# zhenyuw16/Uni3DETR

Hardware: AMD Instinct MI355X
Metric: scenes/sec (fwd+bwd) SUN-RGB-D 20k pts, 300 queries (higher is better)
Workload: dtype bf16

## Files before the change

### include/u3d_hip.h

```cpp
#ifndef U3D_HIP_H_
#define U3D_HIP_H_

#include <stddef.h>
#include <stdint.h>

#ifdef __cplusplus
extern "C" {
#endif

typedef struct ihipStream_t* u3d_stream;

enum {
  U3D_OK = 0,
  U3D_ERR_ARG = -1,
  U3D_ERR_UNSUPPORTED = -2,
  U3D_ERR_LAUNCH = -3,
  U3D_ERR_WORKSPACE = -4
};

enum { U3D_F32 = 0, U3D_BF16 = 1 };

int32_t u3d_version(void);
const char* u3d_strerror(int32_t code);

// ... 388 lines not shown
  U3D_DL_IOU0, U3D_DL_IOU1, U3D_DL_IOU2,
  U3D_DL_NLIN
};
enum { U3D_DLN_1, U3D_DLN_2, U3D_DLN_3, U3D_DLN_PE0, U3D_DLN_PE1, U3D_DLN_C1, U3D_DLN_C2, U3D_DL_NLN };
typedef struct u3d_declayer_params {
  const void* w[U3D_DL_NLIN];
  const void* wt[U3D_DL_NLIN];
  const float* b[U3D_DL_NLIN];
  const float* ln_g[U3D_DL_NLN];
  const float* ln_b[U3D_DL_NLN];
  const float* attw_w; const float* attw_b;
  const float* pe0_w;  const float* pe0_b;
  const float* dim_t;
} u3d_declayer_params;
typedef struct u3d_declayer_dims {
  int32_t m;
  int32_t nq;
  int32_t qps;
  int32_t batch, dz, dy, dx;
  int32_t ncls, code;
  int32_t has_qs;
  int32_t need_dref;
  int32_t layer;
  float p_attn, p_drop;
  float ln_eps;
  int32_t dtype;
  int32_t reserved;
} u3d_declayer_dims;
enum {
  U3D_DS_SINE, U3D_DS_RPH1, U3D_DS_RPH2, U3D_DS_RAW, U3D_DS_QS1, U3D_DS_QS2, U3D_DS_QS, U3D_DS_POS, U3D_DS_QKIN,
  U3D_DS_QK, U3D_DS_V, U3D_DS_LSE, U3D_DS_O, U3D_DS_U1, U3D_DS_MR, U3D_DS_QP, U3D_DS_SAMP, U3D_DS_GATED, U3D_DS_PEH0,
  U3D_DS_UPE1, U3D_DS_U2, U3D_DS_X2C, U3D_DS_FFH, U3D_DS_U3, U3D_DS_R1, U3D_DS_R2, U3D_DS_I1, U3D_DS_I2, U3D_DS_UC1,
  U3D_DS_C1, U3D_DS_UC2, U3D_DS_C2,
  U3D_DS_AMASK,
  U3D_DS_COUNT
};
enum {
  U3D_DG_CLSO, U3D_DG_C2U, U3D_DG_C1U, U3D_DG_IOUO, U3D_DG_I2, U3D_DG_I1, U3D_DG_REGO, U3D_DG_R2, U3D_DG_R1, U3D_DG_F,
  U3D_DG_FFH, U3D_DG_OUT, U3D_DG_UPE1, U3D_DG_P0, U3D_DG_WL, U3D_DG_O2, U3D_DG_DO, U3D_DG_DQK, U3D_DG_DV, U3D_DG_QS,
  U3D_DG_QS2, U3D_DG_QS1, U3D_DG_RAW, U3D_DG_RPH2, U3D_DG_RPH1, U3D_DG_LNP, U3D_DG_DU1, U3D_DG_DPOSA, U3D_DG_SINE,
  U3D_DG_COUNT
};
int32_t u3d_decoder_layer_slots(int32_t m, int32_t ncls, int32_t code, int64_t* save_off, int64_t* grad_off);
int32_t u3d_decoder_layer_slots_dt(int32_t m, int32_t ncls, int32_t code, int32_t dtype, int64_t* save_off, int64_t* grad_off);
int32_t u3d_decoder_layer_blocks(int32_t m);
int32_t u3d_decoder_layer_blocks_dt(int32_t m, int32_t dtype);
int32_t u3d_decoder_layer_fwd(const u3d_declayer_params* p, const u3d_declayer_dims* d, const float* x, const void* xc,
                              const float* ref, const void* value, const uint64_t* rng, float* x_out, void* xc_out,
                              float* reg_out, float* cls_out, float* iou_out, void* save, int64_t save_bytes, u3d_stream s);
int32_t u3d_decoder_layer_bwd(const u3d_declayer_params* p, const u3d_declayer_dims* d, const float* x, const void* xc,
                              const float* ref, const void* value, const uint64_t* rng, const void* xc_out, const void* save,
                              const float* dx_out, const float* dreg, const float* dcls, const float* diou, float* dx,
                              void* vrec, float* dref, void* grad, int64_t grad_bytes, u3d_stream s);
int64_t u3d_value_records_bytes(int32_t m);
int64_t u3d_value_scatter_workspace(int32_t n_cells);
int32_t u3d_value_scatter(const void* records, int32_t m, int32_t n_cells, void* dvalue, int32_t dvalue_bf16, void* work,
                          int64_t work_bytes, u3d_stream s);
int32_t u3d_mha_fwd(const void* qk, const void* v, int32_t m, int32_t nq, float p_attn, int32_t layer, const uint64_t* rng, void* o,
                    float* lse, u3d_stream s);
int32_t u3d_mha_bwd(const void* qk, const void* v, const void* o, const void* d_o, const float* lse, int32_t m, int32_t nq,
                    float p_attn, int32_t layer, const uint64_t* rng, void* dqk, void* dv, u3d_stream s);
int32_t u3d_mha_fwd_dt(const void* qk, const void* v, int32_t m, int32_t nq, float p_attn, int32_t layer, const uint64_t* rng, void* o,
                       float* lse, int32_t dtype, u3d_stream s);
int32_t u3d_mha_bwd_dt(const void* qk, const void* v, const void* o, const void* d_o, const float* lse, int32_t m, int32_t nq,
                       float p_attn, int32_t layer, const uint64_t* rng, void* dqk, void* dv, int32_t dtype, u3d_stream s);
typedef struct u3d_wpack_desc {
  const float* src; void* dst; void* dst_t;
  int32_t n, k, n_pad, n_pad_t;
  int32_t t_plain;
  int32_t reserved;
} u3d_wpack_desc;
int32_t u3d_wpack_bf16(const u3d_wpack_desc* descs_dev, int32_t count, int32_t max_elems, u3d_stream s);
int32_t u3d_wpack(const u3d_wpack_desc* descs_dev, int32_t count, int32_t max_elems, int32_t dtype, u3d_stream s);
int32_t u3d_dropout_mask(const uint64_t* rng, int32_t layer, int32_t site, int64_t n, float p, int32_t cols, uint8_t* keep, u3d_stream s);

#define U3D_AUG_NPARAM 9
int32_t u3d_points_augment(float* points, const int32_t* scene_off, int32_t batch, int32_t n_total, int32_t feat, const float* params,
                           int32_t coord, int32_t height_dim, u3d_stream s);
int32_t u3d_boxes_augment(float* boxes, const int32_t* gt_off, int32_t batch, int32_t n, int32_t box_dim, const float* params, int32_t coord,
                          u3d_stream s);
int32_t u3d_points_range_filter(const float* points, const int32_t* scene_off, int32_t batch, int32_t feat, const float* range6, float* out,
                                int32_t* count, u3d_stream s);
int32_t u3d_point_sample(const float* points, const int32_t* scene_off, const int32_t* count, int32_t batch, int32_t feat, int32_t num_points,
                         const uint64_t* seed, float* out, int32_t* idx_out, u3d_stream s);

int32_t u3d_boxes_range_filter(float* boxes, int32_t* labels, const int32_t* gt_off, int32_t batch, int32_t box_dim,
                               const float* bev_range4, int32_t* count, u3d_stream s);
int32_t u3d_point_shuffle(const float* points, const int32_t* scene_off, const int32_t* count, int32_t batch, int32_t n_total, int32_t feat,
                          const uint64_t* seed, float* out, u3d_stream s);
int32_t u3d_boxes_label_filter(float* boxes, int32_t* labels, const int32_t* gt_off, const int32_t* gt_count, int32_t batch, int32_t box_dim,
                               int32_t num_classes, int32_t* count, u3d_stream s);

int32_t u3d_batch_ingest(const float* points, int32_t n_src, int32_t feat, const int32_t* scene_off, const int32_t* count, int32_t batch,
                         int32_t point_cap, const float* gt, int32_t g_src, int32_t box_dim, const int32_t* gt_labels, const int32_t* gt_off,
                         const int32_t* gt_count, int32_t gt_cap, int32_t gt_dim, float* cat, int32_t* dst_off, float* gt_out,
                         int32_t* labels_out, int32_t* gt_off_out, float* flag, int32_t* overflow, u3d_stream s);

int32_t u3d_objaug_stats(const int32_t* scene_off, const int32_t* count, const int32_t* gt_off, const int32_t* gt_count,
                         const int32_t* labels, int32_t batch, int32_t ncls, int32_t* stats, u3d_stream s);
int32_t u3d_objaug_accept(const float* gt, const int32_t* gt_off, const int32_t* g_live, int32_t box_dim, const float* db_boxes,
                          const int32_t* cand_ids, const int32_t* cand_off, const int32_t* cand_grp, int32_t batch, int32_t words,
                          int32_t* hit_ws, uint32_t* cc_ws, int32_t* acc, u3d_stream s);
int32_t u3d_points_in_boxes(const float* points, const int32_t* scene_off, const int32_t* n_live, int32_t batch, int32_t feat,
                            int32_t tiles, const float* boxes, const int32_t* box_off, const int32_t* box_live, const int32_t* box_active,
                            int32_t box_dim, int32_t words, int32_t* first, uint32_t* bits, int32_t* tile_free, u3d_stream s);
int32_t u3d_objaug_paste(const float* points, const int32_t* scene_off, const int32_t* n_live, int32_t feat, const int32_t* first,
// ... 42 lines not shown
```

### uni3detr_amd/csrc/decoder.hip

```cpp
#include "decoder_common.h"

#ifdef DC_PHASE_TIMING
__device__ unsigned long long dc_dbg_fwd[64];
#define DC_MARK(id) do { if (blockIdx.x == 7 && threadIdx.x == 0) dc_dbg_fwd[id] = __builtin_readcyclecounter(); } while (0)
extern "C" int32_t u3d_debug_fwd_times(uint64_t* out) { return hipMemcpyFromSymbol(out, HIP_SYMBOL(dc_dbg_fwd), 64 * 8) == hipSuccess ? 0 : -1; }
#define MP_MARK(id) do { if (blockIdx.x == 7 && threadIdx.x == 0) dc_dbg_fwd[32 + (id)] = __builtin_readcyclecounter(); } while (0)
#else
#define DC_MARK(id)
#define MP_MARK(id)
#endif

template <typename E>
struct DcPtrs {
  typedef typename E::T T;
  T *sine, *rph1, *rph2, *raw, *qs1, *qs2, *qs, *pos, *qkin, *qk, *v;
  float* lse;
  T* o;
  float *u1, *mr;
  T *qp, *samp, *gated, *peh0, *upe1;
  float* u2;
  T *x2c, *ffh;
  float* u3;
  T *r1, *r2, *i1, *i2, *uc1, *c1, *uc2, *c2;
  unsigned* amask;
// ... 80 lines not shown
  for (int i = blockIdx.x * 256 + threadIdx.x; i < total; i += gridDim.x * 256) {
    const int e = i % E::CH, l = (i / E::CH) & 63, blk = i / WBLK, ks = blk % KS, tile = blk / KS;
    const int n = tile * 16 + (l & 15), k = ks * E::KSTEP + (l >> 4) * E::CH + e;
    ((T*)d.dst)[i] = n < d.n ? E::from_f(d.src[(size_t)n * d.k + k]) : E::from_f(0.f);
  }
  if (d.dst_t) {
    const int tt = d.k * d.n_pad_t;
    if (d.t_plain) {
      for (int i = blockIdx.x * 256 + threadIdx.x; i < tt; i += gridDim.x * 256) {
        const int k = i / d.n_pad_t, n = i % d.n_pad_t;
        ((T*)d.dst_t)[i] = n < d.n ? E::from_f(d.src[(size_t)n * d.k + k]) : E::from_f(0.f);
      }
    } else {
      const int KST = d.n_pad_t / E::KSTEP;
      for (int i = blockIdx.x * 256 + threadIdx.x; i < tt; i += gridDim.x * 256) {
        const int e = i % E::CH, l = (i / E::CH) & 63, blk = i / WBLK, ks = blk % KST, tile = blk / KST;
        const int k = tile * 16 + (l & 15), n = ks * E::KSTEP + (l >> 4) * E::CH + e;
        ((T*)d.dst_t)[i] = n < d.n ? E::from_f(d.src[(size_t)n * d.k + k]) : E::from_f(0.f);
      }
    }
  }
}
extern "C" int32_t u3d_wpack(const u3d_wpack_desc* descs_dev, int32_t count, int32_t max_elems, int32_t dtype, u3d_stream s) {
  U3D_REQUIRE(descs_dev && count >= 0 && max_elems > 0 && (dtype == U3D_BF16 || dtype == U3D_F32), U3D_ERR_ARG);
  if (count == 0) return U3D_OK;
  int gx = u3d_cdiv(max_elems, 256 * 4);
  if (gx > 64) gx = 64;
  if (dtype == U3D_BF16) hipLaunchKernelGGL(k_wpack<EB>, dim3(gx, count), dim3(256), 0, s, descs_dev);
  else hipLaunchKernelGGL(k_wpack<EF>, dim3(gx, count), dim3(256), 0, s, descs_dev);
  U3D_CHECK_LAUNCH();
  return U3D_OK;
}
extern "C" int32_t u3d_wpack_bf16(const u3d_wpack_desc* descs_dev, int32_t count, int32_t max_elems, u3d_stream s) {
  return u3d_wpack(descs_dev, count, max_elems, U3D_BF16, s);
}

__global__ void k_dropout_mask(const unsigned long long* rng, int layer, int site, long long n, unsigned thresh, int cols, unsigned char* keep) {
  const long long i = (long long)blockIdx.x * blockDim.x + threadIdx.x;
  if (i >= n) return;
  const unsigned idx = cols > 0 ? dc_att_idx((unsigned)(i / cols), (unsigned)(i % cols), (unsigned)(cols + 1) & ~1u) : (unsigned)i;
  keep[i] = thresh == 0u ? 1 : (dc_keep(dc_rng_load(rng), dc_site_key(layer, site), idx, thresh) ? 1 : 0);
}
extern "C" int32_t u3d_dropout_mask(const uint64_t* rng, int32_t layer, int32_t site, int64_t n, float p, int32_t cols, uint8_t* keep,
                                    u3d_stream s) {
  U3D_REQUIRE(rng && keep && n >= 0 && p >= 0.f && p < 1.f && cols >= 0, U3D_ERR_ARG);
  if (n == 0) return U3D_OK;
  hipLaunchKernelGGL(k_dropout_mask, dim3((unsigned)((n + 255) / 256)), dim3(256), 0, s, (const unsigned long long*)rng, layer, site,
                     (long long)n, dc_thresh(p), (int)cols, keep);
  U3D_CHECK_LAUNCH();
  return U3D_OK;
}

template <typename E>
__global__ __launch_bounds__(DC_THREADS) void k_dec_pre(u3d_declayer_params P, u3d_declayer_dims dm, const typename E::T* __restrict__ xc,
                                                        const float* __restrict__ ref, DcPtrs<E> S, int skip_inproj) {
  typedef typename E::T T;
  typedef typename E::V4 V4;
  typedef typename E::VC VC;
  typedef DcLds<E> L;
  constexpr int BM = E::BM;
  extern __shared__ __attribute__((aligned(16))) unsigned char lds[];
  T* A0 = (T*)(lds + L::A0);
  T* A1 = (T*)(lds + L::A1);
  T* A2 = (T*)(lds + L::A2);
  const int tid = threadIdx.x, lane = tid & 63, wave = dc_wave_id();
  const int wv = (wave + (int)(blockIdx.x >> 3)) & 3;
  const int row0 = blockIdx.x * BM, M = dm.m;
  dc_poison_lds<E>(lds, tid);
  constexpr int SCH = 384 / E::CH;
  DC_FOR_TID(c, BM * SCH) {
    const int row = c / SCH, ch = c % SCH, col0 = ch * E::CH, coord = col0 >> 7, f0 = col0 & 127;
    const float pos = E::sigmoid(ref[(size_t)min(row0 + row, M - 1) * 3 + coord]);
    VC v;
#pragma unroll
    for (int e = 0; e < E::CH; ++e) {
      const float sarg = pos * 6.283185307179586f / P.dim_t[f0 + e];
      v[e] = E::from_f((e & 1) ? cosf(sarg) : sinf(sarg));
    }
    *(VC*)(A0 + dc_aoff<E>(row, col0, 384)) = v;
    *(VC*)(S.sine + (size_t)(row0 + row) * 384 + col0) = v;
  }
  __syncthreads();
  auto relu_to = [&](T* dst, const float* bias) {
    return [=](int row, int col, f32x4 v) {
      *(V4*)(dst + dc_aoff<E>(row, col, DC_C)) = E::pack4(dc_relu4(v + dc_bias4(bias, col)));
    };
  };
  auto lin_to = [&](T* dst, const float* bias) {
    return [=](int row, int col, f32x4 v) { *(V4*)(dst + dc_aoff<E>(row, col, DC_C)) = E::pack4(v + dc_bias4(bias, col)); };
  };
  T* A1b = A1 + BM * DC_C;
  dc_linear<E, 384, 4>(A0, (const T*)P.w[U3D_DL_RPH0], wv * 64, lane, relu_to(A1, P.b[U3D_DL_RPH0]));
  __syncthreads();
  dc_store_a<E, 256>(A1, S.rph1, DC_C, row0, tid);
  dc_linear<E, 256, 4>(A1, (const T*)P.w[U3D_DL_RPH1], wv * 64, lane, relu_to(A0, P.b[U3D_DL_RPH1]));
  __syncthreads();
  dc_store_a<E, 256>(A0, S.rph2, DC_C, row0, tid);
  dc_linear<E, 256, 4>(A0, (const T*)P.w[U3D_DL_RPH2], wv * 64, lane, lin_to(A2, P.b[U3D_DL_RPH2]));
  __syncthreads();
  dc_store_a<E, 256>(A2, dm.has_qs ? S.raw : S.pos, DC_C, row0, tid);
  dc_load_a<E, 256, true>(A0, xc, DC_C, row0, M, tid);
  __syncthreads();
  if (dm.has_qs) {
    dc_linear<E, 256, 4>(A0, (const T*)P.w[U3D_DL_QS0], wv * 64, lane, relu_to(A1, P.b[U3D_DL_QS0]));
    __syncthreads();
    dc_store_a<E, 256>(A1, S.qs1, DC_C, row0, tid);
    dc_linear<E, 256, 4>(A1, (const T*)P.w[U3D_DL_QS1], wv * 64, lane, relu_to(A1b, P.b[U3D_DL_QS1]));
    __syncthreads();
    dc_store_a<E, 256>(A1b, S.qs2, DC_C, row0, tid);
    const float* bias = P.b[U3D_DL_QS2];
    dc_linear<E, 256, 4>(A1b, (const T*)P.w[U3D_DL_QS2], wv * 64, lane, [=](int row, int col, f32x4 v) {
      const V4 q = E::pack4(v + dc_bias4(bias, col));
      const int ao = dc_aoff<E>(row, col, DC_C);
      const f32x4 raw = E::unpack4(*(const V4*)(A2 + ao));
      *(V4*)(A2 + ao) = E::pack4(E::unpack4(q) * raw);
      *(V4*)(A1 + ao) = q;
    });
    __syncthreads();
    dc_store_a<E, 256>(A1, S.qs, DC_C, row0, tid);
    dc_store_a<E, 256>(A2, S.pos, DC_C, row0, tid);
  }
  DC_FOR_TID(c, BM * (DC_C / E::CH)) {
    const int off = c * E::CH;
    const VC a = *(const VC*)(A0 + off), p = *(const VC*)(A2 + off);
    VC r;
#pragma unroll
    for (int e = 0; e < E::CH; ++e) r[e] = E::from_f(E::to_f(a[e]) + E::to_f(p[e]));
    *(VC*)(A1b + off) = r;
  }
  __syncthreads();
  dc_store_a<E, 256>(A1b, S.qkin, DC_C, row0, tid);
  if (skip_inproj) return;
  dc_linear<E, 256, 4>(A1b, (const T*)P.w[U3D_DL_INQK], wv * 64, lane, lin_to(A1, P.b[U3D_DL_INQK]));
  {
    const float* bias = P.b[U3D_DL_INQK];
    dc_linear<E, 256, 4>(A1b, (const T*)P.w[U3D_DL_INQK], 256 + wv * 64, lane, [=](int row, int col, f32x4 v) {
      *(V4*)(A2 + dc_aoff<E>(row, col - 256, DC_C)) = E::pack4(v + dc_bias4(bias, col));
    });
  }
  __syncthreads();
  dc_store_a<E, 256>(A1, S.qk, 512, row0, tid);
  dc_store_a<E, 256>(A2, S.qk + 256, 512, row0, tid);
  dc_linear<E, 256, 4>(A0, (const T*)P.w[U3D_DL_INV], wv * 64, lane, lin_to(A1b, P.b[U3D_DL_INV]));
  __syncthreads();
  dc_store_a<E, 256>(A1b, S.v, DC_C, row0, tid);
}

template <typename E>
__device__ __forceinline__ void mha_chunk(const typename E::T* Ks, const typename E::T* Vs, const typename E::T* Vt, int kc0, int nkeys,
                                          const typename Mha<E>::RowFrag& qf, unsigned row, unsigned nq_pad, DcRng rg, unsigned key_site,
                                          unsigned thresh, float inv_keep, float scale_log2, int r16, int kq, float& m_run, float& l_run,
                                          f32x4 (&oacc)[2], const unsigned* __restrict__ keep_bits = nullptr) {
  typedef Mha<E> H;
  constexpr int KC = H::KC;
  const int ntile = (nkeys + 15) >> 4;
  f32x4 s[KC / 16];
  float mx = -INFINITY;
#pragma unroll
  for (int t = 0; t < KC / 16; ++t) {
    s[t] = (f32x4){-INFINITY, -INFINITY, -INFINITY, -INFINITY};
    if (t < ntile) {
      f32x4 a = H::scores(Ks, t * 16, r16, kq, qf);
      if (t == ntile - 1) {
#pragma unroll
        for (int r = 0; r < 4; ++r) a[r] = t * 16 + kq * 4 + r < nkeys ? a[r] : -INFINITY;
      }
      mx = fmaxf(fmaxf(mx, fmaxf(a[0], a[1])), fmaxf(a[2], a[3]));
      s[t] = a;
    }
  }
  mx = fmaxf(mx, __shfl_xor(mx, 16, 64));
  mx = fmaxf(mx, __shfl_xor(mx, 32, 64));
  const float m_new = fmaxf(m_run, mx);
  const float corr = E::exp2((m_run - m_new) * scale_log2);
  const float neg_m = -m_new * scale_log2;
  l_run *= corr;
  oacc[0] *= corr; oacc[1] *= corr;
  m_run = m_new;
#pragma unroll
  for (int tp = 0; tp < KC / 32; ++tp) {
    if (tp * 2 < ntile) {
      f32x4 p0, p1;
#pragma unroll
      for (int r = 0; r < 4; ++r) {
        p0[r] = E::exp2(fmaf(s[2 * tp][r], scale_log2, neg_m));
        p1[r] = E::exp2(fmaf(s[2 * tp + 1][r], scale_log2, neg_m));
        l_run += p0[r] + p1[r];
      }
      if (thresh && keep_bits) {
        const int w = (int)keep_bits[tp];
#pragma unroll
        for (int r = 0; r < 4; ++r) {
          p0[r] = __int_as_float(__float_as_int(p0[r] * inv_keep) & __builtin_amdgcn_sbfe(w, kq * 4 + r, 1));
          p1[r] = __int_as_float(__float_as_int(p1[r] * inv_keep) & __builtin_amdgcn_sbfe(w, 16 + kq * 4 + r, 1));
        }
      } else if (thresh) {
// ... 200 lines not shown
        *(V4*)(img + row * RS + (t & 1) * 16 + kq * 4) = valid ? pk : (V4){0, 0, 0, 0};
      }
    }
  }
  MP_MARK(3);
  __syncthreads();
  MP_MARK(4);
  {
    const int per = nq * 4, total = 3 * per, iters = (total + MHA_PROJ_THREADS - 1) / MHA_PROJ_THREADS;
    for (int it = 0; it < iters; ++it) {
      const int c = it * MHA_PROJ_THREADS + tid;
      if (c < total) {
        const int which = c / per, rem = c - which * per, row = rem >> 2, part = rem & 3;
        const VC v = *(const VC*)((which == 0 ? Qs : (which == 1 ? Ks : Vs)) + row * RS + part * 8);
        u16* dst = which == 2 ? v_out + (base + row) * DC_C + h * DC_HD + part * 8
                              : qk_out + (base + row) * 512 + which * 256 + h * DC_HD + part * 8;
        *(VC*)dst = v;
      }
    }
    if (thresh) {
      const int words = nq * MhaProjLds::MW, wit = (words + MHA_PROJ_THREADS - 1) / MHA_PROJ_THREADS;
      for (int it = 0; it < wit; ++it) {
        const int wd = it * MHA_PROJ_THREADS + tid;
        if (wd < words) amask[(size_t)bh * words + wd] = Ms[wd];
      }
    }
  }
  MP_MARK(5);
  for (int qb = wave; qb < nrb; qb += NW) {
    const int q = qb * 16 + r16;
    H::RowFrag qf;
    qf.c[0] = *(const VC*)(Qs + q * RS + kq * 8);
    f32x4 oacc[2] = {{0.f, 0.f, 0.f, 0.f}, {0.f, 0.f, 0.f, 0.f}};
    float m_run = -INFINITY, l_run = 0.f;
    const unsigned row = (unsigned)(bh * nq + q);
    unsigned kb[MhaProjLds::MW];
#pragma unroll
    for (int j = 0; j < MhaProjLds::MW; ++j) kb[j] = Ms[q * MhaProjLds::MW + j];
    mha_chunk<EB>(Ks, Vs, nullptr, 0, nq, qf, row, nq_pad, rg, key_site, thresh, inv_keep, scale_log2, r16, kq, m_run, l_run, oacc, kb);
    l_run += __shfl_xor(l_run, 16, 64);
    l_run += __shfl_xor(l_run, 32, 64);
    if (q < nq) {
      const float inv = 1.f / l_run;
#pragma unroll
      for (int dt = 0; dt < 2; ++dt) *(V4*)(o + (base + q) * DC_C + h * DC_HD + dt * 16 + kq * 4) = EB::pack4(oacc[dt] * inv);
      if (kq == 0) lse[(base + q) * DC_NHEAD + h] = m_run * scale_log2 + log2f(l_run);
    }
    MP_MARK(6 + (qb >> 3));
  }
  MP_MARK(9);
}

template <typename E>
__global__ __launch_bounds__(DC_THREADS) void k_dec_post(u3d_declayer_params P, u3d_declayer_dims dm, const float* __restrict__ x,
                                                         const float* __restrict__ ref, const typename E::T* __restrict__ value,
                                                         const unsigned long long* __restrict__ rng, DcPtrs<E> S, float* __restrict__ x_out,
                                                         typename E::T* __restrict__ xc_out, float* __restrict__ reg_out,
                                                         float* __restrict__ cls_out, float* __restrict__ iou_out) {
  typedef typename E::T T;
  typedef typename E::V4 V4;
  typedef DcLds<E> L;
  constexpr int BM = E::BM, RPW = E::BM / 4;
  extern __shared__ __attribute__((aligned(16))) unsigned char lds[];
  T* A0 = (T*)(lds + L::A0);
  T* A1 = (T*)(lds + L::A1);
  T* A2 = (T*)(lds + L::A2);
  float* F = (float*)(lds + L::F);
  float* G = (float*)(lds + L::G);
  float* misc = (float*)(lds + L::MISC);
  const int tid = threadIdx.x, lane = tid & 63, wave = dc_wave_id();
  const int wv = (wave + (int)(blockIdx.x >> 3)) & 3;
  const int row0 = blockIdx.x * BM, M = dm.m;
  dc_poison_lds<E>(lds, tid);
  DcDrop drop = {dc_rng_load(rng), dc_thresh(dm.p_drop), dc_inv_keep(dm.p_drop), dm.layer};

  DC_MARK(0);
  dc_load_a<E, 256, true>(A0, S.o, DC_C, row0, M, tid);
  dc_load_f<E, false>(F, x, row0, M, tid);
  dc_load_a<E, 256, false>(A2, S.pos, DC_C, row0, M, tid);
  {
    const int row = (tid >> 3) & (BM - 1), j = tid & 7;
    misc[row * DC_MISC_LD + j] = ref[(size_t)min(row0 + row, M - 1) * 3 + min(j, 2)];
  }
  __syncthreads();
  auto add_to_F = [&](const float* bias, int site) {
    return [=](int row, int col, f32x4 v) {
      v = E::round4(v + dc_bias4(bias, col));
      v = drop.apply(v, site, (unsigned)((row0 + row) * DC_C + col));
      float* fp = F + row * DC_TS + col;
      *(f32x4*)fp = *(const f32x4*)fp + v;
    };
  };
  DC_MARK(1);
  dc_linear<E, 256, 4>(A0, (const T*)P.w[U3D_DL_OUTP], wv * 64, lane, add_to_F(P.b[U3D_DL_OUTP], 0));
  __syncthreads();
  DC_MARK(2);
  {
    DcLnOut<E> o = {F, A0, DC_C, nullptr, nullptr, S.mr, U3D_DLN_1, false, S.u1, nullptr};
    dc_layernorm<E>(F, P.ln_g[U3D_DLN_1], P.ln_b[U3D_DLN_1], dm.ln_eps, false, o, row0, wave, lane);
  }
  __syncthreads();
  DC_MARK(3);
  {
    const f32x4 aw = *(const f32x4*)(P.attw_w + lane * 4);
    const float ab = P.attw_b[0];
    constexpr int GRP = 4;
    static_assert(RPW % GRP == 0, "rows per wave must split into gather groups");
#pragma unroll 1
    for (int r0g = 0; r0g < RPW; r0g += GRP) {
      V4 cv[GRP][8];
      float cw[GRP][8];
#ifndef DC_ABL_NOGATHER
#pragma unroll
      for (int g = 0; g < GRP; ++g) {
        const int row = wave * RPW + r0g + g;
        DcCorners tc;
        dc_corners<E>(misc + row * DC_MISC_LD, min(row0 + row, M - 1) / dm.qps, dm.dz, dm.dy, dm.dx, tc);
#pragma unroll
        for (int c = 0; c < 8; ++c) {
          const int vr = max(tc.row[c], 0);
          cw[g][c] = tc.row[c] >= 0 ? tc.w[c] : 0.f;
          cv[g][c] = *(const V4*)(value + (size_t)vr * DC_C + lane * 4);
        }
      }
#endif
#pragma unroll
      for (int g = 0; g < GRP; ++g) {
        const int row = wave * RPW + r0g + g;
        const size_t gr = (size_t)(row0 + row);
        const int ao = dc_aoff<E>(row, lane * 4, DC_C);
        const f32x4 x1 = E::unpack4(*(const V4*)(A0 + ao)), pp = E::unpack4(*(const V4*)(A2 + ao));
        const V4 qpb = E::pack4(x1 + pp);
        const f32x4 qp = E::unpack4(qpb);
        *(V4*)(S.qp + gr * DC_C + lane * 4) = qpb;
        const float wl = E::round(dc_wave_sum(qp[0] * aw[0] + qp[1] * aw[1] + qp[2] * aw[2] + qp[3] * aw[3]) + ab);
        const float gate = E::round(E::sigmoid(wl));
        S.mr[gr * 16 + 14] = wl;
        f32x4 acc = {0.f, 0.f, 0.f, 0.f};
#ifndef DC_ABL_NOGATHER
#pragma unroll
        for (int c = 0; c < 8; ++c) acc += cw[g][c] * E::unpack4(cv[g][c]);
#endif
        const V4 sb = E::pack4(acc);
        const V4 gb = E::pack4(E::unpack4(sb) * gate);
        *(V4*)(A1 + ao) = gb;
        *(V4*)(S.samp + gr * DC_C + lane * 4) = sb;
        *(V4*)(S.gated + gr * DC_C + lane * 4) = gb;
      }
    }
  }
  DC_MARK(4);
  {
    const int col = tid;
    const float w0 = E::round(P.pe0_w[col * 3 + 0]), w1 = E::round(P.pe0_w[col * 3 + 1]), w2 = E::round(P.pe0_w[col * 3 + 2]);
    const float b = P.pe0_b[col];
    for (int row = 0; row < BM; ++row) {
      const float* r3 = misc + row * DC_MISC_LD;
      G[row * DC_TS + col] = E::round(E::round(r3[0]) * w0 + E::round(r3[1]) * w1 + E::round(r3[2]) * w2 + b);
    }
  }
  __syncthreads();
  DC_MARK(5);
  dc_linear<E, 256, 4>(A1, (const T*)P.w[U3D_DL_OPROJ], wv * 64, lane, add_to_F(P.b[U3D_DL_OPROJ], 1));
  {
    DcLnOut<E> o = {nullptr, A0, DC_C, nullptr, S.peh0, S.mr, U3D_DLN_PE0, false, nullptr, nullptr};
    dc_layernorm<E>(G, P.ln_g[U3D_DLN_PE0], P.ln_b[U3D_DLN_PE0], dm.ln_eps, true, o, row0, wave, lane);
  }
  __syncthreads();
  DC_MARK(6);
  {
    const float* bias = P.b[U3D_DL_PE1];
    dc_linear<E, 256, 4>(A0, (const T*)P.w[U3D_DL_PE1], wv * 64, lane, [=](int row, int col, f32x4 v) {
      *(f32x4*)(G + row * DC_TS + col) = E::round4(v + dc_bias4(bias, col));
    });
  }
  __syncthreads();
  DC_MARK(7);
  {
    DcLnOut<E> o = {G, nullptr, 0, nullptr, nullptr, S.mr, U3D_DLN_PE1, true, nullptr, S.upe1};
    dc_layernorm<E>(G, P.ln_g[U3D_DLN_PE1], P.ln_b[U3D_DLN_PE1], dm.ln_eps, true, o, row0, wave, lane);
  }
  __syncthreads();
  DC_FOR_TID(c, BM * 64) {
    const int o = (c >> 6) * DC_TS + (c & 63) * 4;
    *(f32x4*)(F + o) = *(const f32x4*)(F + o) + *(const f32x4*)(G + o);
  }
  __syncthreads();
  DC_MARK(8);
  {
    DcLnOut<E> o = {F, A0, DC_C, nullptr, S.x2c, S.mr, U3D_DLN_2, false, S.u2, nullptr};
    dc_layernorm<E>(F, P.ln_g[U3D_DLN_2], P.ln_b[U3D_DLN_2], dm.ln_eps, false, o, row0, wave, lane);
  }
  __syncthreads();
  DC_MARK(9);
  {
    const float* bias = P.b[U3D_DL_FFN0];
    auto ffh = [=](int row, int col, f32x4 v) {
      v = E::round4(dc_relu4(v + dc_bias4(bias, col)));
      const V4 hb = E::pack4(drop.apply(v, 2, (unsigned)((row0 + row) * DC_FF + col)));
      *(V4*)(A1 + dc_aoff<E>(row, col, DC_FF)) = hb;
    };
    dc_linear<E, 256, 4>(A0, (const T*)P.w[U3D_DL_FFN0], wv * 64, lane, ffh);
    dc_linear<E, 256, 4>(A0, (const T*)P.w[U3D_DL_FFN0], 256 + wv * 64, lane, ffh);
  }
  __syncthreads();
  DC_MARK(10);
  dc_store_a<E, 512>(A1, S.ffh, DC_FF, row0, tid);
  dc_linear<E, 512, 4>(A1, (const T*)P.w[U3D_DL_FFN1], wv * 64, lane, add_to_F(P.b[U3D_DL_FFN1], 3));
  __syncthreads();
  DC_MARK(11);
  {
    DcLnOut<E> o = {nullptr, A2, DC_C, x_out, xc_out, S.mr, U3D_DLN_3, false, S.u3, nullptr};
    dc_layernorm<E>(F, P.ln_g[U3D_DLN_3], P.ln_b[U3D_DLN_3], dm.ln_eps, false, o, row0, wave, lane);
  }
  __syncthreads();
  DC_MARK(12);
  auto relu_to = [&](T* dst, const float* bias) {
    return [=](int row, int col, f32x4 v) {
      *(V4*)(dst + dc_aoff<E>(row, col, DC_C)) = E::pack4(dc_relu4(v + dc_bias4(bias, col)));
    };
  };
  auto narrow_out = [&](float* dst, int n, const float* bias) {
    return [=](int row, int col, f32x4 v) {
#pragma unroll
      for (int r = 0; r < 4; ++r)
        if (col + r < n) dst[(size_t)(row0 + row) * n + col + r] = E::round(v[r] + bias[col + r]);
    };
  };
  T* A1b = A1 + BM * DC_C;
#ifdef DC_PHASE_TIMING
  {
    DC_MARK(20);
    f32x4 acc[E::MT][4];
#pragma unroll
    for (int mt = 0; mt < E::MT; ++mt)
#pragma unroll
      for (int nt = 0; nt < 4; ++nt) acc[mt][nt] = (f32x4){0.f, 0.f, 0.f, 0.f};
    dc_gemm<E, 256, 4>(A2, (const T*)P.w[U3D_DL_REG0] + (size_t)(wv * 64) * 256, acc, lane);
    __builtin_amdgcn_sched_barrier(0);
    DC_MARK(21);
    auto epi = relu_to(A0, P.b[U3D_DL_REG0]);
#pragma unroll
    for (int mt = 0; mt < E::MT; ++mt)
#pragma unroll
      for (int nt = 0; nt < 4; ++nt) epi(mt * 16 + (lane & 15), wv * 64 + nt * 16 + (lane >> 4) * 4, acc[mt][nt]);
    __builtin_amdgcn_sched_barrier(0);
    DC_MARK(22);
    __syncthreads();
    DC_MARK(23);
  }
#else
  dc_linear<E, 256, 4>(A2, (const T*)P.w[U3D_DL_REG0], wv * 64, lane, relu_to(A0, P.b[U3D_DL_REG0]));
  __syncthreads();
#endif
  dc_store_a<E, 256>(A0, S.r1, DC_C, row0, tid);
  dc_linear<E, 256, 4>(A0, (const T*)P.w[U3D_DL_REG1], wv * 64, lane, relu_to(A1, P.b[U3D_DL_REG1]));
  __syncthreads();
  dc_store_a<E, 256>(A1, S.r2, DC_C, row0, tid);
  dc_linear<E, 256, 1>(A1, (const T*)P.w[U3D_DL_REG2], wv * 16, lane, narrow_out(reg_out, dm.code, P.b[U3D_DL_REG2]));
  dc_linear<E, 256, 4>(A2, (const T*)P.w[U3D_DL_IOU0], wv * 64, lane, relu_to(A0, P.b[U3D_DL_IOU0]));
  __syncthreads();
  dc_store_a<E, 256>(A0, S.i1, DC_C, row0, tid);
  dc_linear<E, 256, 4>(A0, (const T*)P.w[U3D_DL_IOU1], wv * 64, lane, relu_to(A1b, P.b[U3D_DL_IOU1]));
  __syncthreads();
  dc_store_a<E, 256>(A1b, S.i2, DC_C, row0, tid);
  dc_linear<E, 256, 1>(A1b, (const T*)P.w[U3D_DL_IOU2], wv * 16, lane, narrow_out(iou_out, 1, P.b[U3D_DL_IOU2]));
  auto to_G = [&](const float* bias) {
    return [=](int row, int col, f32x4 v) { *(f32x4*)(G + row * DC_TS + col) = E::round4(v + dc_bias4(bias, col)); };
  };
  dc_linear<E, 256, 4>(A2, (const T*)P.w[U3D_DL_CLS0], wv * 64, lane, to_G(P.b[U3D_DL_CLS0]));
  __syncthreads();
  {
    DcLnOut<E> o = {nullptr, A0, DC_C, nullptr, S.c1, S.mr, U3D_DLN_C1, false, nullptr, S.uc1};
    dc_layernorm<E>(G, P.ln_g[U3D_DLN_C1], P.ln_b[U3D_DLN_C1], dm.ln_eps, true, o, row0, wave, lane);
  }
  __syncthreads();
  dc_linear<E, 256, 4>(A0, (const T*)P.w[U3D_DL_CLS1], wv * 64, lane, to_G(P.b[U3D_DL_CLS1]));
  __syncthreads();
  {
    DcLnOut<E> o = {nullptr, A1, DC_C, nullptr, S.c2, S.mr, U3D_DLN_C2, false, nullptr, S.uc2};
    dc_layernorm<E>(G, P.ln_g[U3D_DLN_C2], P.ln_b[U3D_DLN_C2], dm.ln_eps, true, o, row0, wave, lane);
  }
  __syncthreads();
  dc_linear<E, 256, 1>(A1, (const T*)P.w[U3D_DL_CLS2], wv * 16, lane, narrow_out(cls_out, dm.ncls, P.b[U3D_DL_CLS2]));
  DC_MARK(14);
}

static int32_t dc_check(const u3d_declayer_params* p, const u3d_declayer_dims* d) {
  U3D_REQUIRE(p && d, U3D_ERR_ARG);
  U3D_REQUIRE(d->m > 0 && d->nq > 0 && d->qps > 0 && d->qps % d->nq == 0 && d->m % d->qps == 0 && d->batch == d->m / d->qps, U3D_ERR_ARG);
  U3D_REQUIRE(d->ncls > 0 && d->ncls <= 32 && d->code > 0 && d->code <= 32, U3D_ERR_UNSUPPORTED);
  U3D_REQUIRE(d->p_attn >= 0.f && d->p_attn < 1.f && d->p_drop >= 0.f && d->p_drop < 1.f, U3D_ERR_ARG);
  U3D_REQUIRE(d->dtype == U3D_BF16 || d->dtype == U3D_F32, U3D_ERR_ARG);
  U3D_REQUIRE((long long)d->m * DC_FF < (1ll << 32), U3D_ERR_UNSUPPORTED);
  for (int i = 0; i < U3D_DL_NLIN; ++i) {
    if (!d->has_qs && (i == U3D_DL_QS0 || i == U3D_DL_QS1 || i == U3D_DL_QS2)) continue;
    U3D_REQUIRE(p->w[i] && p->b[i], U3D_ERR_ARG);
  }
  for (int i = 0; i < U3D_DL_NLN; ++i) U3D_REQUIRE(p->ln_g[i] && p->ln_b[i], U3D_ERR_ARG);
  U3D_REQUIRE(p->attw_w && p->attw_b && p->pe0_w && p->pe0_b && p->dim_t, U3D_ERR_ARG);
  return U3D_OK;
}

template <typename E>
static int32_t dc_layer_fwd(const u3d_declayer_params* p, const u3d_declayer_dims* d, const float* x, const void* xc, const float* ref,
                            const void* value, const uint64_t* rng, float* x_out, void* xc_out, float* reg_out, float* cls_out,
                            float* iou_out, void* save, u3d_stream s) {
  typedef typename E::T T;
  const DcPtrs<E> S = dc_resolve<E>(save, d->m);
  const int nb = u3d_decoder_layer_blocks_dt(d->m, E::DT);
  U3D_ALLOW_LDS(k_dec_pre<E>, DcLds<E>::BYTES);
  U3D_ALLOW_LDS(k_dec_post<E>, DcLds<E>::BYTES);
  const bool fused = mha_fused_inproj(E::DT, d->nq);
  hipLaunchKernelGGL(k_dec_pre<E>, dim3(nb), dim3(DC_THREADS), DcLds<E>::BYTES, s, *p, *d, (const T*)xc, ref, S, fused ? 1 : 0);
  if (fused) {
    U3D_ALLOW_LDS(k_mha_proj_fwd, MhaProjLds::BYTES);
    const float scale_log2 = 1.4426950408889634f / sqrtf((float)DC_HD);
    hipLaunchKernelGGL(k_mha_proj_fwd, dim3((d->m / d->nq) * DC_NHEAD), dim3(MHA_PROJ_THREADS), MhaProjLds::BYTES, s, (const u16*)S.qkin,
                       (const u16*)xc, (const u16*)p->w[U3D_DL_INQK], p->b[U3D_DL_INQK], (const u16*)p->w[U3D_DL_INV], p->b[U3D_DL_INV],
                       d->nq, scale_log2, dc_thresh(d->p_attn), dc_inv_keep(d->p_attn), d->layer, (const unsigned long long*)rng,
                       (u16*)S.qk, (u16*)S.v, (u16*)S.o, S.lse, S.amask);
  } else {
    int32_t rc = u3d_mha_fwd_dt(S.qk, S.v, d->m, d->nq, d->p_attn, d->layer, rng, S.o, S.lse, E::DT, s);
    if (rc != U3D_OK) return rc;
  }
  hipLaunchKernelGGL(k_dec_post<E>, dim3(nb), dim3(DC_THREADS), DcLds<E>::BYTES, s, *p, *d, x, ref, (const T*)value,
                     (const unsigned long long*)rng, S, x_out, (T*)xc_out, reg_out, cls_out, iou_out);
  U3D_CHECK_LAUNCH();
  return U3D_OK;
}

extern "C" int32_t u3d_decoder_layer_fwd(const u3d_declayer_params* p, const u3d_declayer_dims* d, const float* x, const void* xc,
                                         const float* ref, const void* value, const uint64_t* rng, float* x_out, void* xc_out,
                                         float* reg_out, float* cls_out, float* iou_out, void* save, int64_t save_bytes, u3d_stream s) {
  int32_t rc = dc_check(p, d);
  if (rc != U3D_OK) return rc;
  U3D_REQUIRE(x && xc && ref && value && x_out && xc_out && reg_out && cls_out && iou_out && save, U3D_ERR_ARG);
  U3D_REQUIRE((d->p_attn == 0.f && d->p_drop == 0.f) || rng, U3D_ERR_ARG);
  int64_t off[U3D_DS_COUNT + 1];
  u3d_decoder_layer_slots_dt(d->m, d->ncls, d->code, d->dtype, off, nullptr);
  U3D_REQUIRE(save_bytes >= off[U3D_DS_COUNT], U3D_ERR_WORKSPACE);
  if (d->dtype == U3D_BF16) return dc_layer_fwd<EB>(p, d, x, xc, ref, value, rng, x_out, xc_out, reg_out, cls_out, iou_out, save, s);
  return dc_layer_fwd<EF>(p, d, x, xc, ref, value, rng, x_out, xc_out, reg_out, cls_out, iou_out, save, s);
}
```

### uni3detr_amd/csrc/decoder_bwd.hip

```cpp
#define DC_PF 4
#include "decoder_common.h"

#ifdef DC_PHASE_TIMING
__device__ unsigned long long dc_dbg_bwd[64];
#define DC_MARK(id) do { if (blockIdx.x == 7 && threadIdx.x == 0) dc_dbg_bwd[id] = __builtin_readcyclecounter(); } while (0)
extern "C" int32_t u3d_debug_bwd_times(uint64_t* out) { return hipMemcpyFromSymbol(out, HIP_SYMBOL(dc_dbg_bwd), 64 * 8) == hipSuccess ? 0 : -1; }
#else
#define DC_MARK(id)
#endif

template <typename E>
struct DcSave {
  typedef typename E::T T;
  const T *sine, *rph1, *rph2, *raw, *qs1, *qs2, *qs, *pos, *qkin, *qk, *v;
  const float* lse;
  const T* o;
  const float *u1, *mr;
  const T *qp, *samp, *gated, *peh0, *upe1;
  const float* u2;
  const T *x2c, *ffh;
  const float* u3;
  const T *r1, *r2, *i1, *i2, *uc1, *c1, *uc2, *c2;
  const unsigned* amask;
};
// ... 11 lines not shown
extern "C" int32_t u3d_decoder_layer_blocks_dt(int32_t m, int32_t dtype);

template <typename E>
static DcSave<E> dcb_resolve_save(const void* save, int m) {
  typedef typename E::T T;
  int64_t off[U3D_DS_COUNT + 1];
  u3d_decoder_layer_slots_dt(m, 1, 1, E::DT, off, nullptr);
  const char* b = (const char*)save;
  DcSave<E> p;
  p.sine = (const T*)(b + off[U3D_DS_SINE]); p.rph1 = (const T*)(b + off[U3D_DS_RPH1]); p.rph2 = (const T*)(b + off[U3D_DS_RPH2]);
  p.raw = (const T*)(b + off[U3D_DS_RAW]); p.qs1 = (const T*)(b + off[U3D_DS_QS1]); p.qs2 = (const T*)(b + off[U3D_DS_QS2]);
  p.qs = (const T*)(b + off[U3D_DS_QS]); p.pos = (const T*)(b + off[U3D_DS_POS]); p.qkin = (const T*)(b + off[U3D_DS_QKIN]);
  p.qk = (const T*)(b + off[U3D_DS_QK]); p.v = (const T*)(b + off[U3D_DS_V]); p.lse = (const float*)(b + off[U3D_DS_LSE]);
  p.o = (const T*)(b + off[U3D_DS_O]); p.u1 = (const float*)(b + off[U3D_DS_U1]); p.mr = (const float*)(b + off[U3D_DS_MR]);
  p.qp = (const T*)(b + off[U3D_DS_QP]); p.samp = (const T*)(b + off[U3D_DS_SAMP]); p.gated = (const T*)(b + off[U3D_DS_GATED]);
  p.peh0 = (const T*)(b + off[U3D_DS_PEH0]); p.upe1 = (const T*)(b + off[U3D_DS_UPE1]); p.u2 = (const float*)(b + off[U3D_DS_U2]);
  p.x2c = (const T*)(b + off[U3D_DS_X2C]); p.ffh = (const T*)(b + off[U3D_DS_FFH]); p.u3 = (const float*)(b + off[U3D_DS_U3]);
  p.r1 = (const T*)(b + off[U3D_DS_R1]); p.r2 = (const T*)(b + off[U3D_DS_R2]); p.i1 = (const T*)(b + off[U3D_DS_I1]);
  p.i2 = (const T*)(b + off[U3D_DS_I2]); p.uc1 = (const T*)(b + off[U3D_DS_UC1]); p.c1 = (const T*)(b + off[U3D_DS_C1]);
  p.uc2 = (const T*)(b + off[U3D_DS_UC2]); p.c2 = (const T*)(b + off[U3D_DS_C2]);
  p.amask = (const unsigned*)(b + off[U3D_DS_AMASK]);
  return p;
}
template <typename E>
static DcGrad<E> dcb_resolve_grad(void* grad, int m, int ncls, int code, int64_t* total) {
  typedef typename E::T T;
  int64_t off[U3D_DG_COUNT + 1];
  u3d_decoder_layer_slots_dt(m, ncls, code, E::DT, nullptr, off);
  char* b = (char*)grad;
  DcGrad<E> g;
  g.clso = (T*)(b + off[U3D_DG_CLSO]); g.c2u = (T*)(b + off[U3D_DG_C2U]); g.c1u = (T*)(b + off[U3D_DG_C1U]);
  g.iouo = (T*)(b + off[U3D_DG_IOUO]); g.i2 = (T*)(b + off[U3D_DG_I2]); g.i1 = (T*)(b + off[U3D_DG_I1]);
  g.rego = (T*)(b + off[U3D_DG_REGO]); g.r2 = (T*)(b + off[U3D_DG_R2]); g.r1 = (T*)(b + off[U3D_DG_R1]);
  g.f = (T*)(b + off[U3D_DG_F]); g.ffh = (T*)(b + off[U3D_DG_FFH]); g.out = (T*)(b + off[U3D_DG_OUT]);
  g.upe1 = (T*)(b + off[U3D_DG_UPE1]); g.p0 = (T*)(b + off[U3D_DG_P0]); g.wl = (T*)(b + off[U3D_DG_WL]);
  g.o2 = (T*)(b + off[U3D_DG_O2]); g.d_o = (T*)(b + off[U3D_DG_DO]); g.dqk = (T*)(b + off[U3D_DG_DQK]);
  g.dv = (T*)(b + off[U3D_DG_DV]); g.qs = (T*)(b + off[U3D_DG_QS]); g.qs2 = (T*)(b + off[U3D_DG_QS2]);
  g.qs1 = (T*)(b + off[U3D_DG_QS1]); g.raw = (T*)(b + off[U3D_DG_RAW]); g.rph2 = (T*)(b + off[U3D_DG_RPH2]);
  g.rph1 = (T*)(b + off[U3D_DG_RPH1]); g.lnp = (float*)(b + off[U3D_DG_LNP]); g.du1 = (float*)(b + off[U3D_DG_DU1]);
  g.dposa = (T*)(b + off[U3D_DG_DPOSA]); g.sine = (T*)(b + off[U3D_DG_SINE]);
  g.nb = u3d_decoder_layer_blocks_dt(m, E::DT);
  if (total) *total = off[U3D_DG_COUNT];
  return g;
}

template <typename E>
struct DcLnBwdOut { float* tile; typename E::T* a; typename E::T* g16; };
template <typename E, typename LoadU>
__device__ __forceinline__ void dc_layernorm_bwd(const float* T, LoadU load_u, const float* __restrict__ mr, int mr_idx,
                                                 const float* __restrict__ gamma, const float* __restrict__ beta, bool relu,
                                                 const DcLnBwdOut<E>& o, float* __restrict__ lnp, int ln, int nb, float* red ,
                                                 int row0, int wave, int lane, int tid) {
  typedef typename E::V4 V4;
  constexpr int RPW = E::BM / 4;
  const f32x4 ga = *(const f32x4*)(gamma + lane * 4), be = *(const f32x4*)(beta + lane * 4);
  f32x4 dg = {0.f, 0.f, 0.f, 0.f}, db = {0.f, 0.f, 0.f, 0.f};
#pragma unroll 2
  for (int rr = 0; rr < RPW; ++rr) {
    const int row = wave * RPW + rr;
    const int gr = row0 + row;
    const float mu = mr[(size_t)gr * 16 + 2 * mr_idx], rs = mr[(size_t)gr * 16 + 2 * mr_idx + 1];
    const f32x4 u = load_u(row, gr);
    f32x4 dy = *(const f32x4*)(T + row * DC_TS + lane * 4);
    f32x4 xh, dxh;
    float s1 = 0.f, s2 = 0.f;
#pragma unroll
    for (int j = 0; j < 4; ++j) {
      xh[j] = (u[j] - mu) * rs;
      if (relu && !(xh[j] * ga[j] + be[j] > 0.f)) dy[j] = 0.f;
      dxh[j] = dy[j] * ga[j];
      s1 += dxh[j];
      s2 += dxh[j] * xh[j];
      dg[j] += dy[j] * xh[j];
      db[j] += dy[j];
    }
    s1 = dc_wave_sum(s1) * (1.f / DC_C);
    s2 = dc_wave_sum(s2) * (1.f / DC_C);
    f32x4 du;
#pragma unroll
    for (int j = 0; j < 4; ++j) du[j] = rs * (dxh[j] - s1 - xh[j] * s2);
    if (o.tile) *(f32x4*)(o.tile + row * DC_TS + lane * 4) = du;
    const V4 dub = E::pack4(du);
    if (o.a) *(V4*)(o.a + dc_aoff<E>(row, lane * 4, DC_C)) = dub;
    if (o.g16) *(V4*)(o.g16 + (size_t)gr * DC_C + lane * 4) = dub;
  }
  *(f32x4*)(red + (wave * 2 + 0) * DC_C + lane * 4) = dg;
  *(f32x4*)(red + (wave * 2 + 1) * DC_C + lane * 4) = db;
  __syncthreads();
  DC_FOR_TID(i, 2 * DC_C) {
    const int which = i >> 8, col = i & 255;
    const float v = red[(0 * 2 + which) * DC_C + col] + red[(1 * 2 + which) * DC_C + col] + red[(2 * 2 + which) * DC_C + col] +
                    red[(3 * 2 + which) * DC_C + col];
    lnp[((size_t)(ln * 2 + which) * nb + blockIdx.x) * DC_C + col] = v;
  }
  __syncthreads();
}

template <typename E>
__global__ __launch_bounds__(DC_THREADS) void k_dec_post_bwd(u3d_declayer_params P, u3d_declayer_dims dm, const float* __restrict__ ref,
                                                             const typename E::T* __restrict__ value,
                                                             const unsigned long long* __restrict__ rng, DcSave<E> S, DcGrad<E> Gd,
                                                             const float* __restrict__ dx_out, const float* __restrict__ dreg,
                                                             const float* __restrict__ dcls, const float* __restrict__ diou,
                                                             void* __restrict__ vrec, float* __restrict__ dref) {
  float* const rec_ds = (float*)vrec;
  int* const rec_cell = (int*)(rec_ds + (size_t)dm.m * DC_C);
  float* const rec_w = (float*)(rec_cell + (size_t)dm.m * 8);
  typedef typename E::T T;
  typedef typename E::V4 V4;
  typedef DcLds<E> L;
  constexpr int BM = E::BM, RPW = E::BM / 4;
  extern __shared__ __attribute__((aligned(16))) unsigned char lds[];
  T* A0 = (T*)(lds + L::A0);
  T* A1 = (T*)(lds + L::A1);
  T* A2 = (T*)(lds + L::A2);
  float* F = (float*)(lds + L::F);
  float* G = (float*)(lds + L::G);
  float* misc = (float*)(lds + L::MISC);
  float* red = (float*)(A1 + BM * DC_C);
  static_assert(BM * DC_C * sizeof(T) >= 4 * 2 * DC_C * 4, "LayerNorm reduce scratch must fit the second half of A1");
  constexpr int NLD = 40;
  T* Dn = A2;
  static_assert(BM * NLD <= BM * DC_C, "narrow-gradient tile must fit the A2 region");
  const int tid = threadIdx.x, lane = tid & 63, wave = dc_wave_id();
  const int wv = (wave + (int)(blockIdx.x >> 3)) & 3;
  const int row0 = blockIdx.x * BM, M = dm.m, nb = Gd.nb;
  dc_poison_lds<E>(lds, tid);
  DcDrop drop = {dc_rng_load(rng), dc_thresh(dm.p_drop), dc_inv_keep(dm.p_drop), dm.layer};

  DC_MARK(0);
  dc_load_f<E, true>(F, dx_out, row0, M, tid);
  {
    const int row = (tid >> 3) & (BM - 1), j = tid & 7;
    misc[row * DC_MISC_LD + j] = ref[(size_t)min(row0 + row, M - 1) * 3 + min(j, 2)];
  }
  auto load_narrow = [&](const float* src, int n, T* gcopy) {
    DC_FOR_TID(i, BM * 32) {
      const int row = i >> 5, j = i & 31;
      const float raw = src[(size_t)min(row0 + row, M - 1) * n + min(j, n - 1)];
      const float vr = row0 + row < M ? raw : 0.f;
      gcopy[(size_t)(row0 + row) * n + min(j, n - 1)] = E::from_f(vr);
      Dn[row * NLD + j] = E::from_f(j < n ? vr : 0.f);
    }
  };
  auto narrow_dgrad = [&](const T* wt, const T* mask_src, T* dst) {
    typedef typename E::VC VC;
    constexpr int KSN = 32 / E::KSTEP, WBLK = 64 * E::CH;
    const int r16 = lane & 15, kq = lane >> 4;
    f32x4 acc[E::MT][4];
#pragma unroll
    for (int mt = 0; mt < E::MT; ++mt)
#pragma unroll
      for (int nt = 0; nt < 4; ++nt) acc[mt][nt] = (f32x4){0.f, 0.f, 0.f, 0.f};
#pragma unroll
    for (int ks = 0; ks < KSN; ++ks) {
      VC a[E::MT];
#pragma unroll
      for (int mt = 0; mt < E::MT; ++mt) a[mt] = *(const VC*)(Dn + (mt * 16 + r16) * NLD + (ks * 4 + kq) * E::CH);
#pragma unroll
      for (int nt = 0; nt < 4; ++nt) {
        const VC wf = *(const VC*)(wt + (size_t)((wv * 4 + nt) * KSN + ks) * WBLK + lane * E::CH);
#pragma unroll
        for (int mt = 0; mt < E::MT; ++mt) E::mma(wf, a[mt], acc[mt][nt]);
      }
    }
#pragma unroll
    for (int mt = 0; mt < E::MT; ++mt)
#pragma unroll
      for (int nt = 0; nt < 4; ++nt) {
        const int row = mt * 16 + r16, col = wv * 64 + nt * 16 + kq * 4;
        f32x4 v = acc[mt][nt];
        if (mask_src) {
          const V4 y = *(const V4*)(mask_src + (size_t)(row0 + row) * DC_C + col);
#pragma unroll
          for (int r = 0; r < 4; ++r) v[r] = E::to_f(y[r]) > 0.f ? v[r] : 0.f;
        }
        if (dst) *(V4*)(dst + dc_aoff<E>(row, col, DC_C)) = E::pack4(v);
        else *(f32x4*)(G + row * DC_TS + col) = E::round4(v);
      }
  };
  auto masked_to = [&](T* dst, const T* mask_src) {
    return [=](int row, int col, f32x4 v) {
      const V4 y = *(const V4*)(mask_src + (size_t)(row0 + row) * DC_C + col);
#pragma unroll
      for (int r = 0; r < 4; ++r) v[r] = E::to_f(y[r]) > 0.f ? v[r] : 0.f;
      *(V4*)(dst + dc_aoff<E>(row, col, DC_C)) = E::pack4(v);
    };
  };
  auto acc_to_F = [&]() {
    return [=](int row, int col, f32x4 v) {
      float* fp = F + row * DC_TS + col;
      *(f32x4*)fp = *(const f32x4*)fp + E::round4(v);
    };
  };
  auto to_G = [&]() {
    return [=](int row, int col, f32x4 v) { *(f32x4*)(G + row * DC_TS + col) = E::round4(v); };
  };
  auto u_elem = [&](const T* src) {
    return [=](int row, int gr) { return E::unpack4(*(const V4*)(src + (size_t)gr * DC_C + lane * 4)); };
  };
  auto u_f32 = [&](const float* src) {
    return [=](int row, int gr) { return *(const f32x4*)(src + (size_t)gr * DC_C + lane * 4); };
  };

  DC_MARK(1);
  load_narrow(dcls, dm.ncls, Gd.clso);
  __syncthreads();
  narrow_dgrad((const T*)P.wt[U3D_DL_CLS2], nullptr, nullptr);
  __syncthreads();
  {
    DcLnBwdOut<E> o = {nullptr, A0, Gd.c2u};
    dc_layernorm_bwd<E>(G, u_elem(S.uc2), S.mr, U3D_DLN_C2, P.ln_g[U3D_DLN_C2], P.ln_b[U3D_DLN_C2], true, o, Gd.lnp, U3D_DLN_C2, nb, red, row0,
                        wave, lane, tid);
  }
  dc_linear<E, 256, 4>(A0, (const T*)P.wt[U3D_DL_CLS1], wv * 64, lane, to_G());
  __syncthreads();
  {
    DcLnBwdOut<E> o = {nullptr, A0, Gd.c1u};
    dc_layernorm_bwd<E>(G, u_elem(S.uc1), S.mr, U3D_DLN_C1, P.ln_g[U3D_DLN_C1], P.ln_b[U3D_DLN_C1], true, o, Gd.lnp, U3D_DLN_C1, nb, red, row0,
                        wave, lane, tid);
  }
  dc_linear<E, 256, 4>(A0, (const T*)P.wt[U3D_DL_CLS0], wv * 64, lane, acc_to_F());
  __syncthreads();
  DC_MARK(2);
  load_narrow(diou, 1, Gd.iouo);
  __syncthreads();
  narrow_dgrad((const T*)P.wt[U3D_DL_IOU2], S.i2, A0);
  __syncthreads();
  dc_store_a<E, 256>(A0, Gd.i2, DC_C, row0, tid);
  dc_linear<E, 256, 4>(A0, (const T*)P.wt[U3D_DL_IOU1], wv * 64, lane, masked_to(A1, S.i1));
  __syncthreads();
  dc_store_a<E, 256>(A1, Gd.i1, DC_C, row0, tid);
  dc_linear<E, 256, 4>(A1, (const T*)P.wt[U3D_DL_IOU0], wv * 64, lane, acc_to_F());
  __syncthreads();
  DC_MARK(3);
  load_narrow(dreg, dm.code, Gd.rego);
  __syncthreads();
  narrow_dgrad((const T*)P.wt[U3D_DL_REG2], S.r2, A0);
  __syncthreads();
  dc_store_a<E, 256>(A0, Gd.r2, DC_C, row0, tid);
  dc_linear<E, 256, 4>(A0, (const T*)P.wt[U3D_DL_REG1], wv * 64, lane, masked_to(A1, S.r1));
  __syncthreads();
  dc_store_a<E, 256>(A1, Gd.r1, DC_C, row0, tid);
  dc_linear<E, 256, 4>(A1, (const T*)P.wt[U3D_DL_REG0], wv * 64, lane, acc_to_F());
  __syncthreads();
  DC_MARK(4);
  {
    DcLnBwdOut<E> o = {F, nullptr, nullptr};
    dc_layernorm_bwd<E>(F, u_f32(S.u3), S.mr, U3D_DLN_3, P.ln_g[U3D_DLN_3], P.ln_b[U3D_DLN_3], false, o, Gd.lnp, U3D_DLN_3, nb, red, row0,
                        wave, lane, tid);
  }
  DC_MARK(5);
  auto branch_grad = [&](int site, T* dst, T* gslot) {
    DC_FOR_TID(c, BM * 64) {
      const int row = c >> 6, col = (c & 63) * 4;
      f32x4 v = *(const f32x4*)(F + row * DC_TS + col);
      v = drop.apply(v, site, (unsigned)((row0 + row) * DC_C + col));
      const V4 o = E::pack4(v);
      *(V4*)(dst + dc_aoff<E>(row, col, DC_C)) = o;
      *(V4*)(gslot + (size_t)(row0 + row) * DC_C + col) = o;
    }
  };
  branch_grad(3, A0, Gd.f);
  __syncthreads();
  {
    const float ik = drop.inv_keep;
    auto dh = [=](int row, int col, f32x4 v) {
      const V4 y = *(const V4*)(S.ffh + (size_t)(row0 + row) * DC_FF + col);
#pragma unroll
      for (int r = 0; r < 4; ++r) v[r] = E::to_f(y[r]) > 0.f ? E::round(v[r]) * ik : 0.f;
      const V4 o = E::pack4(v);
      *(V4*)(A1 + dc_aoff<E>(row, col, DC_FF)) = o;
    };
    dc_linear<E, 256, 4>(A0, (const T*)P.wt[U3D_DL_FFN1], wv * 64, lane, dh);
    dc_linear<E, 256, 4>(A0, (const T*)P.wt[U3D_DL_FFN1], 256 + wv * 64, lane, dh);
  }
  __syncthreads();
  dc_store_a<E, 512>(A1, Gd.ffh, DC_FF, row0, tid);
  dc_linear<E, 512, 4>(A1, (const T*)P.wt[U3D_DL_FFN0], wv * 64, lane, acc_to_F());
  __syncthreads();
  DC_MARK(6);
  {
    DcLnBwdOut<E> o = {F, nullptr, nullptr};
    dc_layernorm_bwd<E>(F, u_f32(S.u2), S.mr, U3D_DLN_2, P.ln_g[U3D_DLN_2], P.ln_b[U3D_DLN_2], false, o, Gd.lnp, U3D_DLN_2, nb, red, row0,
                        wave, lane, tid);
  }
  DC_MARK(7);
  DC_FOR_TID(c, BM * 64) {
    const int o = (c >> 6) * DC_TS + (c & 63) * 4;
    *(f32x4*)(G + o) = E::round4(*(const f32x4*)(F + o));
  }
  __syncthreads();
  {
    DcLnBwdOut<E> o = {nullptr, A0, Gd.upe1};
    dc_layernorm_bwd<E>(G, u_elem(S.upe1), S.mr, U3D_DLN_PE1, P.ln_g[U3D_DLN_PE1], P.ln_b[U3D_DLN_PE1], true, o, Gd.lnp, U3D_DLN_PE1, nb, red,
                        row0, wave, lane, tid);
  }
  dc_linear<E, 256, 4>(A0, (const T*)P.wt[U3D_DL_PE1], wv * 64, lane, to_G());
  __syncthreads();
  {
    const f32x4 b4 = *(const f32x4*)(P.pe0_b + lane * 4);
    float w[4][3];
#pragma unroll
    for (int j = 0; j < 4; ++j)
#pragma unroll
      for (int k = 0; k < 3; ++k) w[j][k] = E::round(P.pe0_w[(lane * 4 + j) * 3 + k]);
    auto u_pe0 = [=](int row, int gr) {
      const float* r3 = misc + row * DC_MISC_LD;
      const float a = E::round(r3[0]), b = E::round(r3[1]), c = E::round(r3[2]);
      f32x4 u;
#pragma unroll
      for (int j = 0; j < 4; ++j) u[j] = E::round(a * w[j][0] + b * w[j][1] + c * w[j][2] + b4[j]);
      return u;
    };
    DcLnBwdOut<E> o = {G, nullptr, Gd.p0};
    dc_layernorm_bwd<E>(G, u_pe0, S.mr, U3D_DLN_PE0, P.ln_g[U3D_DLN_PE0], P.ln_b[U3D_DLN_PE0], true, o, Gd.lnp, U3D_DLN_PE0, nb, red, row0,
                        wave, lane, tid);
    if (dm.need_dref) {
      for (int rr = 0; rr < RPW; ++rr) {
        const int row = wave * RPW + rr;
        const f32x4 d = E::round4(*(const f32x4*)(G + row * DC_TS + lane * 4));
        float g3[3];
#pragma unroll
        for (int k = 0; k < 3; ++k) g3[k] = dc_wave_sum(d[0] * w[0][k] + d[1] * w[1][k] + d[2] * w[2][k] + d[3] * w[3][k]);
        misc[row * DC_MISC_LD + 8 + (lane & 3)] = (lane & 3) == 0 ? g3[0] : ((lane & 3) == 1 ? g3[1] : g3[2]);
      }
    }
  }
  __syncthreads();
  DC_MARK(8);
  branch_grad(1, A0, Gd.out);
  __syncthreads();
  dc_linear<E, 256, 4>(A0, (const T*)P.wt[U3D_DL_OPROJ], wv * 64, lane, to_G());
  __syncthreads();
  DC_MARK(9);
  {
    const f32x4 aw = *(const f32x4*)(P.attw_w + lane * 4);
#pragma unroll 2
    for (int rr = 0; rr < RPW; ++rr) {
      const int row = wave * RPW + rr, gr = row0 + row;
      const bool ok = gr < M;
      const f32x4 dgt = *(const f32x4*)(G + row * DC_TS + lane * 4);
      const f32x4 samp = E::unpack4(*(const V4*)(S.samp + (size_t)gr * DC_C + lane * 4));
      const float wl = S.mr[(size_t)gr * 16 + 14];
      const float gate = E::round(E::sigmoid(wl));
      float dw = dc_wave_sum(dgt[0] * samp[0] + dgt[1] * samp[1] + dgt[2] * samp[2] + dgt[3] * samp[3]);
      const float sg = E::sigmoid(wl);
      const float dwl = E::round(E::round(dw) * sg * (1.f - sg));
      Gd.wl[gr] = E::from_f(dwl);
      f32x4 dqp;
#pragma unroll
      for (int j = 0; j < 4; ++j) dqp[j] = E::round(dwl * E::round(aw[j]));
      float* fp = F + row * DC_TS + lane * 4;
      *(f32x4*)fp = *(const f32x4*)fp + dqp;
      *(V4*)(Gd.dposa + (size_t)gr * DC_C + lane * 4) = E::pack4(dqp);
      f32x4 ds;
#pragma unroll
      for (int j = 0; j < 4; ++j) ds[j] = E::round(dgt[j] * gate);
      float dsc[4];
#pragma unroll
      for (int j = 0; j < 4; ++j) dsc[j] = E::round(G[row * DC_TS + j * 64 + lane] * gate);
      DcCorners tc;
      dc_corners<E>(misc + row * DC_MISC_LD, min(gr, M - 1) / dm.qps, dm.dz, dm.dy, dm.dx, tc);
      if (ok) {
        float* rds = rec_ds + (size_t)gr * DC_C + lane;
#pragma unroll
        for (int j = 0; j < 4; ++j) rds[j * 64] = dsc[j];
        if (lane == 0) {
#pragma unroll
          for (int c = 0; c < 8; ++c) { rec_cell[(size_t)gr * 8 + c] = tc.row[c]; rec_w[(size_t)gr * 8 + c] = tc.w[c]; }
        }
      }
      float gx = 0.f, gy = 0.f, gz = 0.f;
#ifndef DC_ABL_NOGATHER
      if (ok && dm.need_dref) {
#pragma unroll
        for (int c = 0; c < 8; ++c)
          if (tc.row[c] >= 0) {
            const f32x4 val = E::unpack4(*(const V4*)(value + (size_t)tc.row[c] * DC_C + lane * 4));
            const float dot = val[0] * ds[0] + val[1] * ds[1] + val[2] * ds[2] + val[3] * ds[3];
            gx += tc.dwx[c] * dot; gy += tc.dwy[c] * dot; gz += tc.dwz[c] * dot;
          }
      }
#endif
      if (dm.need_dref) {
        gx = dc_wave_sum(gx); gy = dc_wave_sum(gy); gz = dc_wave_sum(gz);
        {
          const float* r3 = misc + row * DC_MISC_LD;
          const int k = lane % 3;
          const float gk = k == 0 ? gx * dm.dx * 0.5f : (k == 1 ? gy * dm.dy * 0.5f : gz * dm.dz * 0.5f);
          const float sk = E::sigmoid(r3[k]);
          dref[(size_t)gr * 3 + k] = r3[8 + k] + gk * 2.f * sk * (1.f - sk);
        }
      }
    }
  }
  __syncthreads();
  DC_MARK(10);
  {
    DcLnBwdOut<E> o = {F, nullptr, nullptr};
    dc_layernorm_bwd<E>(F, u_f32(S.u1), S.mr, U3D_DLN_1, P.ln_g[U3D_DLN_1], P.ln_b[U3D_DLN_1], false, o, Gd.lnp, U3D_DLN_1, nb, red, row0,
                        wave, lane, tid);
  }
  dc_store_f<E>(F, Gd.du1, row0, tid);
  branch_grad(0, A0, Gd.o2);
  __syncthreads();
  dc_linear<E, 256, 4>(A0, (const T*)P.wt[U3D_DL_OUTP], wv * 64, lane, [=](int row, int col, f32x4 v) {
    *(V4*)(A1 + dc_aoff<E>(row, col, DC_C)) = E::pack4(v);
  });
  __syncthreads();
  dc_store_a<E, 256>(A1, Gd.d_o, DC_C, row0, tid);
  DC_MARK(11);
}

template <typename E>
__global__ __launch_bounds__(256, 2) void k_mha_bwd_dq(const typename E::T* __restrict__ qk, const typename E::T* __restrict__ vv,
                                                       const typename E::T* __restrict__ o, const typename E::T* __restrict__ d_o,
                                                       const float* __restrict__ lse, int nq, int qt_per_wg, float scale_log2, float scale,
                                                       unsigned thresh, float inv_keep, int layer, const unsigned long long* __restrict__ rng,
                                                       typename E::T* __restrict__ dqk, const unsigned* __restrict__ amask) {
  typedef typename E::T T;
  typedef typename E::V4 V4;
  typedef Mha<E> H;
  constexpr int KC = H::KC, MW = KC / 32;
  __shared__ __attribute__((aligned(16))) T Ks[H::RM_ELEMS];
  __shared__ __attribute__((aligned(16))) T Vs[H::RM_ELEMS];
  __shared__ __attribute__((aligned(16))) T Kt[H::TP_ELEMS];
  const int tid = threadIdx.x, lane = tid & 63, wave = tid >> 6, r16 = lane & 15, kq = lane >> 4;
  const int bh = blockIdx.y, g = bh >> 3, h = bh & 7;
  const long long base = (long long)g * nq;
  const unsigned nq_pad = (unsigned)(nq + 1) & ~1u;
  const DcRng rg = dc_rng_load(rng);
  const unsigned key_site = dc_site_key(layer, 4);
  const bool one_chunk = nq <= KC;
  for (int qt = 0; qt < qt_per_wg; ++qt) {
    const int q0 = (blockIdx.x * qt_per_wg + qt) * 64;
    if (q0 >= nq) break;
    const int q = q0 + wave * 16 + r16;
    const bool qok = q < nq;
    typename H::RowFrag qf = H::zero_frag(), dof = H::zero_frag();
    float Dq = 0.f, lq = INFINITY;
    if (qok) {
      qf = H::load_frag(qk + (base + q) * 512 + h * DC_HD, kq);
      dof = H::load_frag(d_o + (base + q) * DC_C + h * DC_HD, kq);
      Dq = H::dot(dof, H::load_frag(o + (base + q) * DC_C + h * DC_HD, kq));
      lq = lse[(base + q) * DC_NHEAD + h];
    }
    Dq += __shfl_xor(Dq, 16, 64);
    Dq += __shfl_xor(Dq, 32, 64);
    f32x4 dq[2] = {{0.f, 0.f, 0.f, 0.f}, {0.f, 0.f, 0.f, 0.f}};
    const unsigned row = (unsigned)(bh * nq + q);
    unsigned kb[MW];
#pragma unroll
    for (int j = 0; j < MW; ++j) kb[j] = (amask && qok) ? amask[(size_t)row * MW + j] : 0u;
    for (int kc0 = 0; kc0 < nq; kc0 += KC) {
      if (qt == 0 || !one_chunk) {
        __syncthreads();
        H::stage(qk + 256 + h * DC_HD, 512, base, kc0, nq, Ks, Kt, tid);
        H::stage(vv + h * DC_HD, 256, base, kc0, nq, Vs, nullptr, tid);
        __syncthreads();
// ... 31 lines not shown
          }
          H::pv(Ks, Kt, tp, r16, kq, dsv[0], dsv[1], dq);
        }
      }
    }
    if (qok) {
#pragma unroll
      for (int dt = 0; dt < 2; ++dt) *(V4*)(dqk + (base + q) * 512 + h * DC_HD + dt * 16 + kq * 4) = E::pack4(dq[dt]);
    }
  }
}

template <typename E>
__global__ __launch_bounds__(256, 2) void k_mha_bwd_dkv(const typename E::T* __restrict__ qk, const typename E::T* __restrict__ vv,
                                                        const typename E::T* __restrict__ o, const typename E::T* __restrict__ d_o,
                                                        const float* __restrict__ lse, int nq, int kt_per_wg, float scale_log2, float scale,
                                                        unsigned thresh, float inv_keep, int layer, const unsigned long long* __restrict__ rng,
                                                        typename E::T* __restrict__ dqk, typename E::T* __restrict__ dv,
                                                        const unsigned* __restrict__ amask) {
  typedef typename E::T T;
  typedef typename E::V4 V4;
  typedef typename E::VC VC;
  typedef Mha<E> H;
  constexpr int KC = H::KC, NP = H::NP, MW = KC / 32;
  __shared__ unsigned Ms[H::TR ? KC * MW : 4];
  __shared__ __attribute__((aligned(16))) T Qs[H::RM_ELEMS];
  __shared__ __attribute__((aligned(16))) T Os[H::RM_ELEMS];
  __shared__ __attribute__((aligned(16))) T Qt[H::TP_ELEMS];
  __shared__ __attribute__((aligned(16))) T Ot[H::TP_ELEMS];
  __shared__ float lse_s[KC], D_s[KC];
  const int tid = threadIdx.x, lane = tid & 63, wave = tid >> 6, r16 = lane & 15, kq = lane >> 4;
  const int bh = blockIdx.y, g = bh >> 3, h = bh & 7;
  const long long base = (long long)g * nq;
  const unsigned nq_pad = (unsigned)(nq + 1) & ~1u;
  const DcRng rg = dc_rng_load(rng);
  const unsigned key_site = dc_site_key(layer, 4);
  const bool one_chunk = nq <= KC;
  for (int kt = 0; kt < kt_per_wg; ++kt) {
    const int k0 = (blockIdx.x * kt_per_wg + kt) * 64;
    if (k0 >= nq) break;
    const int key = k0 + wave * 16 + r16;
    const bool kok = key < nq;
    typename H::RowFrag kf = H::zero_frag(), vf = H::zero_frag();
    if (kok) {
      kf = H::load_frag(qk + (base + key) * 512 + 256 + h * DC_HD, kq);
      vf = H::load_frag(vv + (base + key) * DC_C + h * DC_HD, kq);
    }
    f32x4 dk[2] = {{0.f, 0.f, 0.f, 0.f}, {0.f, 0.f, 0.f, 0.f}}, dvv[2] = {{0.f, 0.f, 0.f, 0.f}, {0.f, 0.f, 0.f, 0.f}};
    for (int qc0 = 0; qc0 < nq; qc0 += KC) {
      if (kt == 0 || !one_chunk) {
        __syncthreads();
        H::stage(qk + h * DC_HD, 512, base, qc0, nq, Qs, Qt, tid);
        H::stage(d_o + h * DC_HD, 256, base, qc0, nq, Os, Ot, tid);
        DC_FOR_TID(c, KC * NP) {
          const int qq = c / NP, part = c % NP;
          float d = 0.f;
          if (qc0 + qq < nq) {
            const VC a = *(const VC*)(d_o + (base + qc0 + qq) * DC_C + h * DC_HD + part * E::CH);
            const VC b = *(const VC*)(o + (base + qc0 + qq) * DC_C + h * DC_HD + part * E::CH);
#pragma unroll
            for (int e = 0; e < E::CH; ++e) d += E::chunk_elem(a, e) * E::chunk_elem(b, e);
          }
#pragma unroll
          for (int sh = 1; sh < NP; sh <<= 1) d += __shfl_xor(d, sh, 64);
          if (part == 0) {
            D_s[qq] = d;
            lse_s[qq] = qc0 + qq < nq ? lse[(base + qc0 + qq) * DC_NHEAD + h] : INFINITY;
          }
        }
        if constexpr (H::TR) {
          if (amask) {
            DC_FOR_TID(c, KC * MW) Ms[c] = c < nq * MW ? amask[(size_t)bh * nq * MW + c] : 0u;
          }
        }
        __syncthreads();
      }
      const int nqs = min(KC, nq - qc0);
      const int ntile = (nqs + 15) >> 4;
#pragma unroll 2
      for (int tp = 0; tp < KC / 32; ++tp) {
        if (tp * 2 < ntile) {
          f32x4 pd[2], dsv[2];
#pragma unroll
          for (int u = 0; u < 2; ++u) {
            const int t = tp * 2 + u;
            const f32x4 s = H::scores(Qs, t * 16, r16, kq, kf);
            const f32x4 dp = H::scores(Os, t * 16, r16, kq, vf);
            const f32x4 l4 = *(const f32x4*)(lse_s + t * 16 + kq * 4), D4 = *(const f32x4*)(D_s + t * 16 + kq * 4);
#pragma unroll
            for (int r = 0; r < 4; ++r) {
              const float p = E::exp2(fmaf(s[r], scale_log2, -l4[r]));
              float keepf = 1.f;
              if (H::TR && thresh && amask)
                keepf = __int_as_float(__float_as_int(inv_keep) & __builtin_amdgcn_sbfe((int)Ms[(t * 16 + kq * 4 + r) * MW + (key >> 5)], key & 31, 1));
              else if (thresh) keepf = dc_keep(rg, key_site, dc_att_idx((unsigned)(bh * nq + qc0 + t * 16 + kq * 4 + r), (unsigned)key, nq_pad), thresh) ? inv_keep : 0.f;
              pd[u][r] = p * keepf;
              dsv[u][r] = p * (dp[r] * keepf - D4[r]) * scale;
            }
          }
          H::pv(Os, Ot, tp, r16, kq, pd[0], pd[1], dvv);
          H::pv(Qs, Qt, tp, r16, kq, dsv[0], dsv[1], dk);
        }
      }
    }
    if (kok) {
#pragma unroll
      for (int dt = 0; dt < 2; ++dt) {
        *(V4*)(dqk + (base + key) * 512 + 256 + h * DC_HD + dt * 16 + kq * 4) = E::pack4(dk[dt]);
        *(V4*)(dv + (base + key) * DC_C + h * DC_HD + dt * 16 + kq * 4) = E::pack4(dvv[dt]);
      }
    }
  }
}

template <typename E>
static void mha_bwd_launch(const void* qk, const void* v, const void* o, const void* d_o, const float* lse, int32_t m, int32_t nq,
                           float p_attn, int32_t layer, const uint64_t* rng, void* dqk, void* dv, u3d_stream s, const unsigned* amask = nullptr) {
  typedef typename E::T T;
  if (nq > Mha<E>::KC || E::DT != U3D_BF16) amask = nullptr;
  const float scale = 1.f / sqrtf((float)DC_HD), scale_log2 = 1.4426950408889634f * scale;
  const int qt = mha_tiles_per_wg<E>(nq);
  const dim3 grid(u3d_cdiv(nq, 64 * qt), (m / nq) * DC_NHEAD);
  hipLaunchKernelGGL(k_mha_bwd_dq<E>, grid, dim3(256), 0, s, (const T*)qk, (const T*)v, (const T*)o, (const T*)d_o, lse, nq, qt, scale_log2,
                     scale, dc_thresh(p_attn), dc_inv_keep(p_attn), layer, (const unsigned long long*)rng, (T*)dqk, amask);
  hipLaunchKernelGGL(k_mha_bwd_dkv<E>, grid, dim3(256), 0, s, (const T*)qk, (const T*)v, (const T*)o, (const T*)d_o, lse, nq, qt, scale_log2,
                     scale, dc_thresh(p_attn), dc_inv_keep(p_attn), layer, (const unsigned long long*)rng, (T*)dqk, (T*)dv, amask);
}
extern "C" int32_t u3d_mha_bwd_dt(const void* qk, const void* v, const void* o, const void* d_o, const float* lse, int32_t m, int32_t nq,
                                  float p_attn, int32_t layer, const uint64_t* rng, void* dqk, void* dv, int32_t dtype, u3d_stream s) {
  U3D_REQUIRE(qk && v && o && d_o && lse && dqk && dv && m > 0 && nq > 0 && m % nq == 0 && p_attn >= 0.f && p_attn < 1.f, U3D_ERR_ARG);
  U3D_REQUIRE(p_attn == 0.f || rng, U3D_ERR_ARG);
  U3D_REQUIRE(dtype == U3D_BF16 || dtype == U3D_F32, U3D_ERR_ARG);
  U3D_REQUIRE((long long)(m / nq) * DC_NHEAD * nq * (nq + 1) < (1ll << 32), U3D_ERR_UNSUPPORTED);
  if (dtype == U3D_BF16) mha_bwd_launch<EB>(qk, v, o, d_o, lse, m, nq, p_attn, layer, rng, dqk, dv, s);
  else mha_bwd_launch<EF>(qk, v, o, d_o, lse, m, nq, p_attn, layer, rng, dqk, dv, s);
  U3D_CHECK_LAUNCH();
  return U3D_OK;
}
extern "C" int32_t u3d_mha_bwd(const void* qk, const void* v, const void* o, const void* d_o, const float* lse, int32_t m, int32_t nq,
                               float p_attn, int32_t layer, const uint64_t* rng, void* dqk, void* dv, u3d_stream s) {
  return u3d_mha_bwd_dt(qk, v, o, d_o, lse, m, nq, p_attn, layer, rng, dqk, dv, U3D_BF16, s);
}

template <typename E>
__global__ __launch_bounds__(DC_THREADS) void k_dec_pre_bwd(u3d_declayer_params P, u3d_declayer_dims dm, DcSave<E> S, DcGrad<E> Gd,
                                                            float* __restrict__ dx) {
  typedef typename E::T T;
  typedef typename E::V4 V4;
  typedef DcLds<E> L;
  constexpr int BM = E::BM;
  extern __shared__ __attribute__((aligned(16))) unsigned char lds[];
  T* A0 = (T*)(lds + L::A0);
  T* A1 = (T*)(lds + L::A1);
  T* A2 = (T*)(lds + L::A2);
  float* F = (float*)(lds + L::F);
  float* G = (float*)(lds + L::G);
  const int tid = threadIdx.x, lane = tid & 63, wave = dc_wave_id();
  const int wv = (wave + (int)(blockIdx.x >> 3)) & 3;
  const int row0 = blockIdx.x * BM, M = dm.m;
  dc_poison_lds<E>(lds, tid);

  dc_load_a<E, 512, true>(A1, Gd.dqk, 512, row0, M, tid);
  dc_load_a<E, 256, true>(A0, Gd.dv, DC_C, row0, M, tid);
  dc_load_f_rows<E>(F, Gd.du1, row0, tid);
  __syncthreads();
  auto acc_to_F = [&]() {
    return [=](int row, int col, f32x4 v) {
      float* fp = F + row * DC_TS + col;
      *(f32x4*)fp = *(const f32x4*)fp + E::round4(v);
    };
  };
  auto masked_to = [&](T* dst, const T* mask_src) {
    return [=](int row, int col, f32x4 v) {
      const V4 y = *(const V4*)(mask_src + (size_t)(row0 + row) * DC_C + col);
#pragma unroll
      for (int r = 0; r < 4; ++r) v[r] = E::to_f(y[r]) > 0.f ? v[r] : 0.f;
      *(V4*)(dst + dc_aoff<E>(row, col, DC_C)) = E::pack4(v);
    };
  };
  dc_linear<E, 512, 4>(A1, (const T*)P.wt[U3D_DL_INQK], wv * 64, lane,
                       [=](int row, int col, f32x4 v) { *(f32x4*)(G + row * DC_TS + col) = E::round4(v); });
  dc_linear<E, 256, 4>(A0, (const T*)P.wt[U3D_DL_INV], wv * 64, lane, acc_to_F());
  __syncthreads();
  DC_FOR_TID(c, BM * 64) {
    const int row = c >> 6, col = (c & 63) * 4;
    const size_t go = (size_t)(row0 + row) * DC_C + col;
    const f32x4 dqk = *(const f32x4*)(G + row * DC_TS + col);
    float* fp = F + row * DC_TS + col;
    *(f32x4*)fp = *(const f32x4*)fp + dqk;
    const f32x4 dpos = E::round4(dqk + E::unpack4(*(const V4*)(Gd.dposa + go)));
    const int ao = dc_aoff<E>(row, col, DC_C);
    if (dm.has_qs) {
      const f32x4 raw = E::unpack4(*(const V4*)(S.raw + go)), qs = E::unpack4(*(const V4*)(S.qs + go));
      const V4 dqs = E::pack4(dpos * raw), draw = E::pack4(dpos * qs);
      *(V4*)(A0 + ao) = dqs;
      *(V4*)(A2 + ao) = draw;
      *(V4*)(Gd.qs + go) = dqs;
      *(V4*)(Gd.raw + go) = draw;
    } else {
      const V4 draw = E::pack4(dpos);
      *(V4*)(A2 + ao) = draw;
      *(V4*)(Gd.raw + go) = draw;
    }
  }
  __syncthreads();
  T* A1b = A1 + BM * DC_C;
  if (dm.has_qs) {
    dc_linear<E, 256, 4>(A0, (const T*)P.wt[U3D_DL_QS2], wv * 64, lane, masked_to(A1, S.qs2));
    __syncthreads();
    dc_store_a<E, 256>(A1, Gd.qs2, DC_C, row0, tid);
    dc_linear<E, 256, 4>(A1, (const T*)P.wt[U3D_DL_QS1], wv * 64, lane, masked_to(A1b, S.qs1));
    __syncthreads();
    dc_store_a<E, 256>(A1b, Gd.qs1, DC_C, row0, tid);
    dc_linear<E, 256, 4>(A1b, (const T*)P.wt[U3D_DL_QS0], wv * 64, lane, acc_to_F());
    __syncthreads();
  }
  dc_linear<E, 256, 4>(A2, (const T*)P.wt[U3D_DL_RPH2], wv * 64, lane, masked_to(A0, S.rph2));
  __syncthreads();
  dc_store_a<E, 256>(A0, Gd.rph2, DC_C, row0, tid);
  dc_linear<E, 256, 4>(A0, (const T*)P.wt[U3D_DL_RPH1], wv * 64, lane, masked_to(A1, S.rph1));
  __syncthreads();
  dc_store_a<E, 256>(A1, Gd.rph1, DC_C, row0, tid);
  if (dm.need_dref) {
    auto to_sine = [=](int row, int col, f32x4 v) { *(V4*)(Gd.sine + (size_t)(row0 + row) * 384 + col) = E::pack4(v); };
    dc_linear<E, 256, 4>(A1, (const T*)P.wt[U3D_DL_RPH0], wv * 64, lane, to_sine);
    dc_linear<E, 256, 2>(A1, (const T*)P.wt[U3D_DL_RPH0], 256 + wv * 32, lane, to_sine);
  }
  dc_store_f<E>(F, dx, row0, tid);
}

static int32_t dcb_check(const u3d_declayer_params* p, const u3d_declayer_dims* d) {
  U3D_REQUIRE(p && d, U3D_ERR_ARG);
  U3D_REQUIRE(d->m > 0 && d->nq > 0 && d->qps > 0 && d->qps % d->nq == 0 && d->m % d->qps == 0 && d->batch == d->m / d->qps, U3D_ERR_ARG);
  U3D_REQUIRE(d->ncls > 0 && d->ncls <= 32 && d->code > 0 && d->code <= 32, U3D_ERR_UNSUPPORTED);
  U3D_REQUIRE(d->dtype == U3D_BF16 || d->dtype == U3D_F32, U3D_ERR_ARG);
  for (int i = 0; i < U3D_DL_NLIN; ++i) {
    if (!d->has_qs && (i == U3D_DL_QS0 || i == U3D_DL_QS1 || i == U3D_DL_QS2)) continue;
    U3D_REQUIRE(p->w[i], U3D_ERR_ARG);
    U3D_REQUIRE(p->wt[i], U3D_ERR_ARG);
  }
  for (int i = 0; i < U3D_DL_NLN; ++i) U3D_REQUIRE(p->ln_g[i] && p->ln_b[i], U3D_ERR_ARG);
  U3D_REQUIRE(p->attw_w && p->pe0_w && p->pe0_b && p->dim_t, U3D_ERR_ARG);
  return U3D_OK;
}

template <typename E>
static int32_t dcb_layer_bwd(const u3d_declayer_params* p, const u3d_declayer_dims* d, const float* ref, const void* value,
                             const uint64_t* rng, const void* save, const float* dx_out, const float* dreg, const float* dcls,
                             const float* diou, float* dx, void* dvalue, float* dref, void* grad, int64_t grad_bytes, u3d_stream s) {
  typedef typename E::T T;
  int64_t total = 0;
  const DcGrad<E> G = dcb_resolve_grad<E>(grad, d->m, d->ncls, d->code, &total);
  U3D_REQUIRE(grad_bytes >= total, U3D_ERR_WORKSPACE);
  const DcSave<E> S = dcb_resolve_save<E>(save, d->m);
  U3D_ALLOW_LDS(k_dec_post_bwd<E>, DcLds<E>::BYTES);
  U3D_ALLOW_LDS(k_dec_pre_bwd<E>, DcLds<E>::BYTES);
  hipLaunchKernelGGL(k_dec_post_bwd<E>, dim3(G.nb), dim3(DC_THREADS), DcLds<E>::BYTES, s, *p, *d, ref, (const T*)value,
                     (const unsigned long long*)rng, S, G, dx_out, dreg, dcls, diou, dvalue, dref);
  if (mha_fused_inproj(E::DT, d->nq) && d->p_attn > 0.f) {
    U3D_REQUIRE((long long)(d->m / d->nq) * DC_NHEAD * d->nq * (d->nq + 1) < (1ll << 32), U3D_ERR_UNSUPPORTED);
    mha_bwd_launch<E>(S.qk, S.v, S.o, G.d_o, S.lse, d->m, d->nq, d->p_attn, d->layer, rng, G.dqk, G.dv, s, S.amask);
  } else {
    int32_t rc = u3d_mha_bwd_dt(S.qk, S.v, S.o, G.d_o, S.lse, d->m, d->nq, d->p_attn, d->layer, rng, G.dqk, G.dv, E::DT, s);
    if (rc != U3D_OK) return rc;
  }
  hipLaunchKernelGGL(k_dec_pre_bwd<E>, dim3(G.nb), dim3(DC_THREADS), DcLds<E>::BYTES, s, *p, *d, S, G, dx);
  U3D_CHECK_LAUNCH();
  return U3D_OK;
}

extern "C" int32_t u3d_decoder_layer_bwd(const u3d_declayer_params* p, const u3d_declayer_dims* d, const float* x, const void* xc,
                                         const float* ref, const void* value, const uint64_t* rng, const void* xc_out, const void* save,
                                         const float* dx_out, const float* dreg, const float* dcls, const float* diou, float* dx,
                                         void* dvalue, float* dref, void* grad, int64_t grad_bytes, u3d_stream s) {
  (void)x; (void)xc; (void)xc_out;
  int32_t rc = dcb_check(p, d);
  if (rc != U3D_OK) return rc;
  U3D_REQUIRE(ref && value && save && dreg && dcls && diou && dx && dvalue && grad, U3D_ERR_ARG);
  U3D_REQUIRE(d->reserved == 0, U3D_ERR_ARG);
  U3D_REQUIRE(!d->need_dref || dref, U3D_ERR_ARG);
  U3D_REQUIRE((d->p_attn == 0.f && d->p_drop == 0.f) || rng, U3D_ERR_ARG);
  if (d->dtype == U3D_BF16)
    return dcb_layer_bwd<EB>(p, d, ref, value, rng, save, dx_out, dreg, dcls, diou, dx, dvalue, dref, grad, grad_bytes, s);
  return dcb_layer_bwd<EF>(p, d, ref, value, rng, save, dx_out, dreg, dcls, diou, dx, dvalue, dref, grad, grad_bytes, s);
}

#define VS_K 64
#define VS_NONE 0x7fffffff

__global__ void k_vs_init(int* __restrict__ cnt, int* __restrict__ owner, int n_cells) {
  const long long i = (long long)blockIdx.x * blockDim.x + threadIdx.x;
  if (i < n_cells) { cnt[i] = 0; owner[i] = VS_NONE; }
}

__global__ void k_vs_register(const int* __restrict__ cell, int n_entries, int n_cells, int* __restrict__ cnt, int* __restrict__ owner,
                              int* __restrict__ list) {
  const int e = blockIdx.x * blockDim.x + threadIdx.x;
  if (e >= n_entries) return;
  const int c = cell[e];
  if (c < 0 || c >= n_cells) return;
  atomicMin(&owner[c], e);
  const int slot = atomicAdd(&cnt[c], 1);
  if (slot < VS_K) list[(size_t)c * VS_K + slot] = e;
}

__device__ __forceinline__ unsigned short vs_bf16_rne(float f) {
  const unsigned int u = __float_as_uint(f);
  if ((u & 0x7fffffffu) > 0x7f800000u) return (unsigned short)((u >> 16) | 0x40u);
  return (unsigned short)((u + 0x7fffu + ((u >> 16) & 1u)) >> 16);
}

__device__ __forceinline__ void vs_add_entry(const float* __restrict__ ds, const float* __restrict__ w, int id, int lane, float* acc) {
  const float wt = w[id];
  const float* src = ds + (size_t)(id >> 3) * 256 + lane;
#pragma unroll
  for (int j = 0; j < 4; ++j) acc[j] += wt * src[j * 64];
}

__global__ __launch_bounds__(256) void k_vs_reduce(const float* __restrict__ ds, const int* __restrict__ cell, const float* __restrict__ w,
                                                   int n_entries, int n_cells, int* __restrict__ cnt, int* __restrict__ owner,
                                                   const int* __restrict__ list, void* __restrict__ dvalue, int dvalue_bf16) {
  const int lane = threadIdx.x & 63, wave = threadIdx.x >> 6;
  const int e = blockIdx.x * 4 + wave;
  if (e >= n_entries) return;
  const int c = cell[e];
  if (c < 0 || c >= n_cells || owner[c] != e) return;
  const int n = cnt[c];
  float acc[4] = {0.f, 0.f, 0.f, 0.f};
  if (n <= VS_K) {
    const int mine = lane < n ? list[(size_t)c * VS_K + lane] : VS_NONE;
    int rank = 0;
    for (int k = 0; k < n; ++k) rank += __shfl(mine, k) < mine;
    for (int k = 0; k < n; ++k)
      vs_add_entry(ds, w, __shfl(mine, __builtin_ctzll(__ballot(lane < n && rank == k))), lane, acc);
  } else {
    for (int base = 0; base < n_entries; base += 256) {
      int cc[4];
// ... 47 lines not shown
```

### uni3detr_amd/csrc/decoder_common.h

```cpp
#pragma once
#include "common.h"

typedef float f32x4 __attribute__((ext_vector_type(4)));
typedef __bf16 bf16x8 __attribute__((ext_vector_type(8)));
typedef __bf16 bf16x4 __attribute__((ext_vector_type(4)));
typedef unsigned short u16;
typedef unsigned short u16x4 __attribute__((ext_vector_type(4)));
typedef unsigned short u16x8 __attribute__((ext_vector_type(8)));

#define DC_THREADS 256
#define DC_C 256
#define DC_FF 512
#define DC_TS 260
#define DC_NHEAD 8
#define DC_HD 32
#define DC_MISC_LD 48

__device__ __forceinline__ float dc_bf2f(u16 v) { return __uint_as_float((unsigned)v << 16); }
__device__ __forceinline__ u16 dc_f2bf(float f) {
  __bf16 h = (__bf16)f;
  return __builtin_bit_cast(u16, h);
}
__device__ __forceinline__ float dc_sigmoid(float x) { return 1.f / (1.f + __expf(-x)); }

template <int CTRL, int ROW_MASK>
__device__ __forceinline__ float dc_dpp(float v) {
  return __builtin_bit_cast(float, __builtin_amdgcn_update_dpp(0, __builtin_bit_cast(int, v), CTRL, ROW_MASK, 0xF, true));
}
__device__ __forceinline__ float dc_wave_sum(float v) {
  v += dc_dpp<0xB1, 0xF>(v);
  v += dc_dpp<0x4E, 0xF>(v);
  v += dc_dpp<0x141, 0xF>(v);
  v += dc_dpp<0x140, 0xF>(v);
  v += dc_dpp<0x142, 0xA>(v);
  v += dc_dpp<0x143, 0xC>(v);
  return __builtin_bit_cast(float, __builtin_amdgcn_readlane(__builtin_bit_cast(int, v), 63));
}

struct EB {
  typedef u16 T;
  typedef u16x4 V4;
  typedef u16x8 VC;
  static constexpr int CH = 8;
  static constexpr int BM = 32;
  static constexpr int MT = 2;
  static constexpr int KSTEP = 32;
  static constexpr int DT = U3D_BF16;
  static constexpr int MHA_KC = 320;
  __device__ static __forceinline__ float to_f(T v) { return dc_bf2f(v); }
  __device__ static __forceinline__ T from_f(float f) { return dc_f2bf(f); }
  __device__ static __forceinline__ float round(float f) { return dc_bf2f(dc_f2bf(f)); }
  __device__ static __forceinline__ V4 pack4(f32x4 v) { return __builtin_bit_cast(u16x4, __builtin_convertvector(v, bf16x4)); }
  __device__ static __forceinline__ f32x4 unpack4(V4 v) {
    f32x4 r = {dc_bf2f(v[0]), dc_bf2f(v[1]), dc_bf2f(v[2]), dc_bf2f(v[3])};
    return r;
  }
  __device__ static __forceinline__ f32x4 round4(f32x4 v) { return unpack4(pack4(v)); }
  __device__ static __forceinline__ float exp2(float x) { return __builtin_amdgcn_exp2f(x); }
  __device__ static __forceinline__ float sigmoid(float x) { return 1.f / (1.f + __expf(-x)); }
  __device__ static __forceinline__ float rsqrt(float x) { return rsqrtf(x); }
  __device__ static __forceinline__ VC zero_chunk() { return (VC){0, 0, 0, 0, 0, 0, 0, 0}; }
  __device__ static __forceinline__ float chunk_elem(const VC& v, int e) { return dc_bf2f(v[e]); }
  __device__ static __forceinline__ void mma(const VC& w, const VC& a, f32x4& acc) {
    acc = __builtin_amdgcn_mfma_f32_16x16x32_bf16(__builtin_bit_cast(bf16x8, w), __builtin_bit_cast(bf16x8, a), acc, 0, 0, 0);
  }
};
struct EF {
  typedef float T;
  typedef f32x4 V4;
  typedef f32x4 VC;
  static constexpr int CH = 4;
  static constexpr int BM = 16;
  static constexpr int MT = 1;
  static constexpr int KSTEP = 16;
  static constexpr int DT = U3D_F32;
  static constexpr int MHA_KC = 64;
  __device__ static __forceinline__ float to_f(T v) { return v; }
  __device__ static __forceinline__ T from_f(float f) { return f; }
  __device__ static __forceinline__ float round(float f) { return f; }
  __device__ static __forceinline__ V4 pack4(f32x4 v) { return v; }
  __device__ static __forceinline__ f32x4 unpack4(V4 v) { return v; }
  __device__ static __forceinline__ f32x4 round4(f32x4 v) { return v; }
  __device__ static __forceinline__ float exp2(float x) { return exp2f(x); }
  __device__ static __forceinline__ float sigmoid(float x) { return 1.f / (1.f + expf(-x)); }
  __device__ static __forceinline__ float rsqrt(float x) { return 1.f / sqrtf(x); }
  __device__ static __forceinline__ VC zero_chunk() { return (VC){0.f, 0.f, 0.f, 0.f}; }
  __device__ static __forceinline__ float chunk_elem(const VC& v, int e) { return v[e]; }
  __device__ static __forceinline__ void mma(const VC& w, const VC& a, f32x4& acc) {
#pragma unroll
    for (int j = 0; j < 4; ++j) acc = __builtin_amdgcn_mfma_f32_16x16x4f32(w[j], a[j], acc, 0, 0, 0);
  }
};

template <typename E>
struct DcLds {
  static constexpr int ES = (int)sizeof(typename E::T);
  static constexpr int A0 = 0;
  static constexpr int A1 = A0 + E::BM * 512 * ES;
  static constexpr int A2 = A1 + E::BM * 512 * ES;
  static constexpr int F = A2 + E::BM * 256 * ES;
  static constexpr int G = F + E::BM * DC_TS * 4;
  static constexpr int MISC = G + E::BM * DC_TS * 4;
  static constexpr int BYTES = MISC + E::BM * DC_MISC_LD * 4;
};
static_assert(DcLds<EB>::BYTES <= 160 * 1024 && DcLds<EF>::BYTES <= 160 * 1024, "row-chain tiles must fit the CU's LDS");

template <typename E>
__device__ __forceinline__ int dc_aoff(int row, int col, int ldk) {
  return row * ldk + ((((col / E::CH) ^ (row & 15)) * E::CH) | (col % E::CH));
}

struct DcRng { unsigned lo, hi; };
__device__ __forceinline__ DcRng dc_rng_load(const unsigned long long* p) {
  const unsigned long long v = p ? *p : 0ull;
  DcRng r = {(unsigned)v, (unsigned)(v >> 32)};
  return r;
}
__device__ __forceinline__ unsigned dc_site_key(int layer, int site) { return (unsigned)(layer * 8 + site + 1) * 0x85EBCA77u; }
__device__ __forceinline__ unsigned dc_hash_pair(DcRng g, unsigned site_key, unsigned pair) {
  unsigned h = pair * 0x9E3779B1u + (g.lo ^ site_key);
  h ^= h >> 15; h *= 0x85EBCA77u; h ^= h >> 13; h ^= g.hi; h *= 0xC2B2AE3Du; h ^= h >> 16;
  return h;
}
__device__ __forceinline__ bool dc_keep_half(unsigned word, unsigned odd, unsigned thresh) { return ((word >> (odd * 16u)) & 0xFFFFu) >= thresh; }
__device__ __forceinline__ bool dc_keep(DcRng g, unsigned site_key, unsigned idx, unsigned thresh) {
  return dc_keep_half(dc_hash_pair(g, site_key, idx >> 1), idx & 1u, thresh);
}
__device__ __forceinline__ void dc_keep4(DcRng g, unsigned site_key, unsigned idx0, unsigned thresh, bool (&k)[4]) {
  const unsigned w0 = dc_hash_pair(g, site_key, idx0 >> 1), w1 = dc_hash_pair(g, site_key, (idx0 >> 1) + 1u);
  k[0] = dc_keep_half(w0, 0u, thresh); k[1] = dc_keep_half(w0, 1u, thresh);
  k[2] = dc_keep_half(w1, 0u, thresh); k[3] = dc_keep_half(w1, 1u, thresh);
}
__device__ __forceinline__ unsigned dc_att_idx(unsigned row, unsigned key, unsigned nq_pad) { return row * nq_pad + key; }
__host__ __device__ static inline unsigned dc_thresh(float p) { return p <= 0.f ? 0u : (unsigned)(p * 65536.0f); }
__host__ __device__ static inline float dc_inv_keep(float p) { return p <= 0.f ? 1.f : 1.f / (1.f - p); }

struct DcDrop {
  DcRng rng; unsigned thresh; float inv_keep; int layer;
  __device__ __forceinline__ f32x4 apply(f32x4 v, int site, unsigned idx0) const {
    if (thresh == 0u) return v;
    bool k[4];
    dc_keep4(rng, dc_site_key(layer, site), idx0, thresh, k);
#pragma unroll
    for (int r = 0; r < 4; ++r) v[r] = k[r] ? v[r] * inv_keep : 0.f;
    return v;
  }
};

#ifndef DC_PF
#define DC_PF 8
#endif
constexpr int dc_burst(int ks, int want) {
  int b = 1;
  for (int d = 1; d <= want && d <= ks; ++d)
    if (ks % d == 0) b = d;
  return b;
}
template <typename E, int K, int NT>
__device__ __forceinline__ void dc_gemm(const typename E::T* A, const typename E::T* __restrict__ W, f32x4 (&acc)[E::MT][NT], int lane) {
  typedef typename E::T T;
  typedef typename E::VC VC;
  constexpr int KS = K / E::KSTEP;
  constexpr int PF = dc_burst(KS, DC_PF);
  static_assert((K / E::CH) % 16 == 0, "the chunk swizzle permutes aligned groups of 16 chunks");
#ifdef DC_ABL_NOGEMM
  return;
#endif
  const int r16 = lane & 15, kq = lane >> 4;
  constexpr int WBLK = 64 * E::CH;
  const T* wp[NT];
#pragma unroll
  for (int nt = 0; nt < NT; ++nt) wp[nt] = W + (size_t)nt * KS * WBLK + lane * E::CH;
  const T* ap[E::MT];
#pragma unroll
  for (int mt = 0; mt < E::MT; ++mt) ap[mt] = A + (mt * 16 + r16) * K;
#ifndef DC_NO_KROT
  const int rot = (int)(blockIdx.x % KS);
#else
  const int rot = 0;
#endif
#pragma unroll
  for (int kb = 0; kb < KS; kb += PF) {
    VC wf[PF][NT];
    int kk[PF];
#pragma unroll
    for (int p = 0; p < PF; ++p) {
      kk[p] = kb + p + rot;
      kk[p] = kk[p] >= KS ? kk[p] - KS : kk[p];
    }
#pragma unroll
    for (int p = 0; p < PF; ++p)
#pragma unroll
      for (int nt = 0; nt < NT; ++nt) wf[p][nt] = *(const VC*)(wp[nt] + kk[p] * WBLK);
    __builtin_amdgcn_sched_barrier(0);
#pragma unroll
    for (int p = 0; p < PF; ++p) {
      const int ch = ((kk[p] * 4 + kq) ^ r16) * E::CH;
      VC a[E::MT];
#pragma unroll
      for (int mt = 0; mt < E::MT; ++mt) a[mt] = *(const VC*)(ap[mt] + ch);
#pragma unroll
      for (int nt = 0; nt < NT; ++nt)
#pragma unroll
        for (int mt = 0; mt < E::MT; ++mt) E::mma(wf[p][nt], a[mt], acc[mt][nt]);
    }
    __builtin_amdgcn_sched_barrier(0);
  }
}

template <typename E, int K, int NT, typename Epi>
__device__ __forceinline__ void dc_linear(const typename E::T* A, const typename E::T* __restrict__ W, int ncol0, int lane, Epi epi) {
  f32x4 acc[E::MT][NT];
#pragma unroll
  for (int mt = 0; mt < E::MT; ++mt)
#pragma unroll
    for (int nt = 0; nt < NT; ++nt) acc[mt][nt] = (f32x4){0.f, 0.f, 0.f, 0.f};
  dc_gemm<E, K, NT>(A, W + (size_t)ncol0 * K, acc, lane);
  const int r16 = lane & 15, kq = lane >> 4;
#pragma unroll
  for (int mt = 0; mt < E::MT; ++mt)
#pragma unroll
    for (int nt = 0; nt < NT; ++nt) epi(mt * 16 + r16, ncol0 + nt * 16 + kq * 4, acc[mt][nt]);
}

__device__ __forceinline__ f32x4 dc_ld4(const float* p) { return *(const f32x4*)p; }
__device__ __forceinline__ f32x4 dc_bias4(const float* b, int col) {
  return b ? *(const f32x4*)(b + col) : (f32x4){0.f, 0.f, 0.f, 0.f};
}
__device__ __forceinline__ f32x4 dc_relu4(f32x4 v) {
  f32x4 r = {fmaxf(v[0], 0.f), fmaxf(v[1], 0.f), fmaxf(v[2], 0.f), fmaxf(v[3], 0.f)};
  return r;
}

#define DC_FOR_TID(c, N) _Pragma("unroll") for (int it_ = 0, c = tid; it_ < (N) / DC_THREADS; ++it_, c += DC_THREADS)
__device__ __forceinline__ int dc_wave_id() { return __builtin_amdgcn_readfirstlane((int)(threadIdx.x >> 6)); }

template <typename E, int K, bool CLAMP>
__device__ __forceinline__ void dc_load_a(typename E::T* A, const typename E::T* __restrict__ src, int ld, int row0, int M, int tid) {
  typedef typename E::VC VC;
  constexpr int CPR = K / E::CH;
  static_assert((E::BM * CPR) % DC_THREADS == 0, "tile chunks must split evenly over the workgroup");
  DC_FOR_TID(c, E::BM * CPR) {
    const int row = c / CPR, ch = c % CPR;
    const int gr = CLAMP ? min(row0 + row, M - 1) : row0 + row;
    *(VC*)(A + dc_aoff<E>(row, ch * E::CH, K)) = *(const VC*)(src + (size_t)gr * ld + ch * E::CH);
  }
}
template <typename E, int K>
__device__ __forceinline__ void dc_store_a(const typename E::T* A, typename E::T* __restrict__ dst, int ld, int row0, int tid) {
  typedef typename E::VC VC;
  constexpr int CPR = K / E::CH;
  DC_FOR_TID(c, E::BM * CPR) {
    const int row = c / CPR, ch = c % CPR;
    *(VC*)(dst + (size_t)(row0 + row) * ld + ch * E::CH) = *(const VC*)(A + dc_aoff<E>(row, ch * E::CH, K));
  }
}
template <typename E, bool ZERO_TAIL>
__device__ __forceinline__ void dc_load_f(float* T, const float* __restrict__ src, int row0, int M, int tid) {
  if (src == nullptr) {
    DC_FOR_TID(c, E::BM * 64) *(f32x4*)(T + (c >> 6) * DC_TS + (c & 63) * 4) = (f32x4){0.f, 0.f, 0.f, 0.f};
    return;
  }
  DC_FOR_TID(c, E::BM * 64) {
    const int row = c >> 6, q = c & 63;
    f32x4 v = *(const f32x4*)(src + (size_t)min(row0 + row, M - 1) * DC_C + q * 4);
    if (ZERO_TAIL) {
      const float keep = row0 + row < M ? 1.f : 0.f;
      v *= keep;
    }
    *(f32x4*)(T + row * DC_TS + q * 4) = v;
  }
}
template <typename E>
__device__ __forceinline__ void dc_load_f_rows(float* T, const float* __restrict__ src, int row0, int tid) {
  DC_FOR_TID(c, E::BM * 64) *(f32x4*)(T + (c >> 6) * DC_TS + (c & 63) * 4) = *(const f32x4*)(src + (size_t)(row0 + (c >> 6)) * DC_C + (c & 63) * 4);
}
template <typename E>
__device__ __forceinline__ void dc_store_f(const float* T, float* __restrict__ dst, int row0, int tid) {
  DC_FOR_TID(c, E::BM * 64) *(f32x4*)(dst + (size_t)(row0 + (c >> 6)) * DC_C + (c & 63) * 4) = *(const f32x4*)(T + (c >> 6) * DC_TS + (c & 63) * 4);
}

template <typename E>
struct DcLnOut {
  float* tile;
  typename E::T* a; int a_ldk;
  float* g32;
  typename E::T* g16;
  float* mr;
  int mr_idx;
  bool round_out;
  float* gpre;
  typename E::T* gpre16;
};
template <typename E>
__device__ __forceinline__ void dc_layernorm(const float* T, const float* __restrict__ gamma, const float* __restrict__ beta, float eps,
                                             bool relu, const DcLnOut<E>& o, int row0, int wave, int lane) {
  typedef typename E::V4 V4;
  constexpr int RPW = E::BM / 4;
  const f32x4 ga = *(const f32x4*)(gamma + lane * 4), be = *(const f32x4*)(beta + lane * 4);
#pragma unroll 2
  for (int rr = 0; rr < RPW; ++rr) {
    const int row = wave * RPW + rr;
    const f32x4 v = *(const f32x4*)(T + row * DC_TS + lane * 4);
    const float mu = dc_wave_sum(v[0] + v[1] + v[2] + v[3]) * (1.f / DC_C);
    const f32x4 d = {v[0] - mu, v[1] - mu, v[2] - mu, v[3] - mu};
    const float rs = E::rsqrt(dc_wave_sum(d[0] * d[0] + d[1] * d[1] + d[2] * d[2] + d[3] * d[3]) * (1.f / DC_C) + eps);
    f32x4 y;
#pragma unroll
    for (int j = 0; j < 4; ++j) {
      y[j] = d[j] * rs * ga[j] + be[j];
      if (relu) y[j] = fmaxf(y[j], 0.f);
    }
    const V4 yb = E::pack4(y);
    if (o.round_out) y = E::unpack4(yb);
    const size_t grow = (size_t)(row0 + row);
    if (o.gpre) *(f32x4*)(o.gpre + grow * DC_C + lane * 4) = v;
    if (o.gpre16) *(V4*)(o.gpre16 + grow * DC_C + lane * 4) = E::pack4(v);
    if (o.tile) *(f32x4*)(o.tile + row * DC_TS + lane * 4) = y;
    if (o.a) *(V4*)(o.a + dc_aoff<E>(row, lane * 4, o.a_ldk)) = yb;
    if (o.g32) *(f32x4*)(o.g32 + grow * DC_C + lane * 4) = y;
    if (o.g16) *(V4*)(o.g16 + grow * DC_C + lane * 4) = yb;
    if (o.mr) {
      o.mr[grow * 16 + 2 * o.mr_idx] = mu;
      o.mr[grow * 16 + 2 * o.mr_idx + 1] = rs;
    }
  }
}

struct DcCorners { int row[8]; float w[8], dwx[8], dwy[8], dwz[8]; };
template <typename E>
__device__ __forceinline__ void dc_corners(const float* ref3, int b, int D, int H, int W, DcCorners& tc) {
  const float gx = (E::sigmoid(ref3[0]) - 0.5f) * 2.f, gy = (E::sigmoid(ref3[1]) - 0.5f) * 2.f, gz = (E::sigmoid(ref3[2]) - 0.5f) * 2.f;
  const float ix = ((gx + 1.f) * W - 1.f) * 0.5f, iy = ((gy + 1.f) * H - 1.f) * 0.5f, iz = ((gz + 1.f) * D - 1.f) * 0.5f;
  const float fx = floorf(ix), fy = floorf(iy), fz = floorf(iz);
  const int x0 = (int)fx, y0 = (int)fy, z0 = (int)fz;
  const float tx = ix - fx, ty = iy - fy, tz = iz - fz;
#pragma unroll
  for (int c = 0; c < 8; ++c) {
    const int dx = c & 1, dy = (c >> 1) & 1, dz = c >> 2;
    const int x = x0 + dx, y = y0 + dy, z = z0 + dz;
    const float wx = dx ? tx : 1.f - tx, wy = dy ? ty : 1.f - ty, wz = dz ? tz : 1.f - tz;
    const bool ok = (unsigned)x < (unsigned)W && (unsigned)y < (unsigned)H && (unsigned)z < (unsigned)D;
    tc.row[c] = __builtin_amdgcn_readfirstlane(ok ? ((b * D + z) * H + y) * W + x : -1);
    tc.w[c] = wx * wy * wz;
    tc.dwx[c] = (dx ? 1.f : -1.f) * wy * wz;
    tc.dwy[c] = (dy ? 1.f : -1.f) * wx * wz;
    tc.dwz[c] = (dz ? 1.f : -1.f) * wx * wy;
  }
}

#ifndef DC_POISON_LDS
#define DC_POISON_LDS 0
#endif
template <typename E>
__device__ __forceinline__ void dc_poison_lds(unsigned char* lds, int tid) {
#if DC_POISON_LDS == 1
  for (int i = tid; i < DcLds<E>::BYTES / 4; i += DC_THREADS) ((unsigned*)lds)[i] = 0xFFFFFFFFu;
  __syncthreads();
#elif DC_POISON_LDS == 2
  __syncthreads();
#elif DC_POISON_LDS == 3
  for (int i = tid; i < DcLds<E>::BYTES / 4; i += DC_THREADS) ((unsigned*)lds)[i] = 0xFFFFFFFFu;
#endif
}

#ifdef DC_ABL_NOFRAGSTORE
#define DC_FRAG_STORE(stmt)
#else
#define DC_FRAG_STORE(stmt) stmt
#endif

__host__ static inline int dc_esize(int dtype) { return dtype == U3D_BF16 ? 2 : 4; }
__host__ static inline int dc_bm(int dtype) { return dtype == U3D_BF16 ? EB::BM : EF::BM; }

typedef short s16x4 __attribute__((ext_vector_type(4)));
typedef short s16x8 __attribute__((ext_vector_type(8)));
template <typename E>
struct Mha {
  typedef typename E::T T;
  typedef typename E::VC VC;
  static constexpr bool TR = E::CH == 8;
  static constexpr int KC = E::MHA_KC;
  static constexpr int NP = DC_HD / E::CH;
  static constexpr int RS = TR ? 48 : 32;
  static constexpr int TLD = KC + 8;
  static constexpr int RM_ELEMS = KC * RS;
  static constexpr int TP_ELEMS = TR ? 8 : 32 * TLD;
  __device__ static __forceinline__ int roff(int row, int part) {
    if constexpr (TR) return row * RS + part * 8;
    else return row * 32 + (((part ^ row) & 7) << 2);
  }
  __device__ static __forceinline__ void stage(const T* __restrict__ src, int ld, long long base_row, int first, int nvalid, T* rowmajor,
                                               T* transposed, int tid) {
    DC_FOR_TID(c, KC * NP) {
      const int key = c / NP, part = c % NP;
      VC v = E::zero_chunk();
      if (first + key < nvalid) v = *(const VC*)(src + (base_row + first + key) * ld + part * E::CH);
      if (rowmajor) *(VC*)(rowmajor + roff(key, part)) = v;
      if constexpr (!TR) {
        if (transposed) {
#pragma unroll
          for (int e = 0; e < E::CH; ++e) transposed[(part * E::CH + e) * TLD + key] = v[e];
        }
      }
    }
  }
  struct RowFrag { VC c[NP / 4]; };
  __device__ static __forceinline__ RowFrag zero_frag() {
    RowFrag f;
#pragma unroll
    for (int j = 0; j < NP / 4; ++j) f.c[j] = E::zero_chunk();
    return f;
  }
  __device__ static __forceinline__ RowFrag load_frag(const T* __restrict__ row32, int kq) {
    RowFrag f;
#pragma unroll
    for (int j = 0; j < NP / 4; ++j) f.c[j] = *(const VC*)(row32 + (j * 4 + kq) * E::CH);
    return f;
  }
  __device__ static __forceinline__ float dot(const RowFrag& a, const RowFrag& b) {
    float d = 0.f;
#pragma unroll
    for (int j = 0; j < NP / 4; ++j)
#pragma unroll
      for (int e = 0; e < E::CH; ++e) d += E::chunk_elem(a.c[j], e) * E::chunk_elem(b.c[j], e);
    return d;
  }
  __device__ static __forceinline__ f32x4 scores(const T* rowmajor, int row0, int r16, int kq, const RowFrag& f) {
    f32x4 acc = {0.f, 0.f, 0.f, 0.f};
#pragma unroll
    for (int j = 0; j < NP / 4; ++j) E::mma(*(const VC*)(rowmajor + roff(row0 + r16, j * 4 + kq)), f.c[j], acc);
    return acc;
  }
  __device__ static __forceinline__ void pv(const T* rowmajor, const T* transposed, int tp, int r16, int kq, f32x4 p0, f32x4 p1,
                                            f32x4 (&acc)[2]) {
    if constexpr (TR) {
      (void)transposed;
      const u16x4 a4 = EB::pack4(p0), b4 = EB::pack4(p1);
      const u16x8 pb = {a4[0], a4[1], a4[2], a4[3], b4[0], b4[1], b4[2], b4[3]};
      const int j = r16 >> 2, q = r16 & 3;
      const u16* p0a = (const u16*)rowmajor + (tp * 32 + 4 * kq + j) * RS + 4 * q;
#pragma unroll
      for (int dt = 0; dt < 2; ++dt) {
        typedef s16x4 __attribute__((address_space(3))) * lds_s16x4;
        const s16x4 x0 = __builtin_amdgcn_ds_read_tr16_b64_v4i16((lds_s16x4)(p0a + dt * 16));
        const s16x4 x1 = __builtin_amdgcn_ds_read_tr16_b64_v4i16((lds_s16x4)(p0a + dt * 16 + 16 * RS));
        const s16x8 vb = {x0[0], x0[1], x0[2], x0[3], x1[0], x1[1], x1[2], x1[3]};
// ... 26 lines not shown
```

### uni3detr_amd/native.py

```python
import ctypes as C
import os

import numpy as np
import torch

from . import abi

_HERE = os.path.dirname(os.path.abspath(__file__))
LIB_PATH = os.environ.get("U3D_LIB_PATH") or os.path.join(_HERE, "libu3d_hip.so")

_ABI = abi.load()
_K = _ABI.constants


def _struct(c_name, py_name):
    return abi.structure(_ABI.structs[c_name], py_name)


def _slot_names(prefix):
    names = sorted((v, n[len(prefix):]) for n, v in _K.items() if n.startswith(prefix))
    assert [v for v, _ in names] == list(range(len(names))) and names[-1][1] == "COUNT" and _K[prefix + "COUNT"] == len(names) - 1
    return [n for _, n in names[:-1]]


# ... 1551 lines not shown
    n, nc = logits.shape
    F_ = dim_t.numel()
    out = torch.empty((n, nc * F_), dtype=out_dtype, device=logits.device)
    _check(lib().u3d_sine_embed_fwd(_ptr(logits), _ptr(dim_t), n, nc, F_, dtype_code(out), _ptr(out), _stream()), "sine_embed_fwd")
    return out


def sine_embed_bwd(logits, dim_t, dout):
    n, nc = logits.shape
    dl = torch.empty((n, nc), dtype=torch.float32, device=logits.device)
    _check(lib().u3d_sine_embed_bwd(_ptr(logits), _ptr(dim_t), _ptr(dout), dtype_code(dout), n, nc, dim_t.numel(), _ptr(dl), _stream()),
           "sine_embed_bwd")
    return dl


_SLOT_CACHE = {}
DT_F32, DT_BF16 = F32, BF16


def dt_code(dtype):
    if dtype == torch.bfloat16:
        return DT_BF16
    if dtype == torch.float32:
        return DT_F32
    raise U3DError(f"fused decoder: unsupported element type {dtype}")


def decoder_layer_slots(m, ncls, code, dtype=torch.bfloat16):
    key = (m, ncls, code, dtype)
    r = _SLOT_CACHE.get(key)
    if r is None:
        so = (C.c_int64 * (len(DS_NAMES) + 1))()
        go = (C.c_int64 * (len(DG_NAMES) + 1))()
        _check(lib().u3d_decoder_layer_slots_dt(m, ncls, code, dt_code(dtype), so, go), "decoder_layer_slots")
        r = ({**{n: int(so[i]) for i, n in enumerate(DS_NAMES)}, "_total": int(so[len(DS_NAMES)])},
             {**{n: int(go[i]) for i, n in enumerate(DG_NAMES)}, "_total": int(go[len(DG_NAMES)])})
        _SLOT_CACHE[key] = r
    return r


def slot_view(buf, off, rows, cols, dtype):
    nbytes = rows * cols * torch.empty((), dtype=dtype).element_size()
    return buf[off:off + nbytes].view(dtype).view(rows, cols)


def decoder_blocks(m, dtype=torch.bfloat16):
    return int(lib().u3d_decoder_layer_blocks_dt(m, dt_code(dtype)))


def decoder_rows(m, dtype=torch.bfloat16):
    return decoder_blocks(m, dtype) * (32 if dtype == torch.bfloat16 else 16)


def decoder_layer_fwd(params, dims, x, xc, ref, value_rows, rng, save):
    m, code, ncls = dims.m, dims.code, dims.ncls
    et = torch.bfloat16 if dims.dtype == DT_BF16 else torch.float32
    assert xc.dtype == et and value_rows.dtype == et and x.dtype == torch.float32
    mp = decoder_rows(m, et)
    dev = x.device
    x_out = torch.empty((mp, 256), dtype=torch.float32, device=dev)
    xc_out = torch.empty((mp, 256), dtype=torch.bfloat16, device=dev) if et == torch.bfloat16 else x_out
    reg = torch.empty((mp, code), dtype=torch.float32, device=dev)
    cls = torch.empty((mp, ncls), dtype=torch.float32, device=dev)
    iou = torch.empty((mp,), dtype=torch.float32, device=dev)
    _check(lib().u3d_decoder_layer_fwd(C.byref(params), C.byref(dims), _ptr(x), _ptr(xc), _ptr(ref), _ptr(value_rows), _ptr(rng),
                                       _ptr(x_out), _ptr(xc_out), _ptr(reg), _ptr(cls), _ptr(iou), _ptr(save), save.numel(), _stream()),
           "decoder_layer_fwd")
    return x_out[:m], xc_out[:m], reg[:m], cls[:m], iou[:m]


def decoder_layer_bwd(params, dims, x, xc, ref, value_rows, rng, xc_out, save, dx_out, dreg, dcls, diou, dvalue, grad):
    m = dims.m
    dims.reserved = 0
    assert dvalue.dtype == torch.float32 or dims.dtype == DT_BF16
    rec = torch.empty(int(lib().u3d_value_records_bytes(m)), dtype=torch.uint8, device=ref.device)
    mp = decoder_rows(m, torch.bfloat16 if dims.dtype == DT_BF16 else torch.float32)
    dx = torch.empty((mp, 256), dtype=torch.float32, device=ref.device)
    dref = torch.empty((mp, 3), dtype=torch.float32, device=ref.device) if dims.need_dref else None
    _check(lib().u3d_decoder_layer_bwd(C.byref(params), C.byref(dims), _ptr(x), _ptr(xc), _ptr(ref), _ptr(value_rows), _ptr(rng),
                                       _ptr(xc_out), _ptr(save), _ptr(dx_out), _ptr(dreg), _ptr(dcls), _ptr(diou), _ptr(dx),
                                       _ptr(rec), _ptr(dref), _ptr(grad), grad.numel(), _stream()), "decoder_layer_bwd")
    value_scatter(rec, m, dvalue)
    return dx[:m], (None if dref is None else dref[:m])


def value_scatter(records, m, dvalue):
    assert dvalue.is_contiguous() and dvalue.shape[1] == 256 and dvalue.dtype in (torch.float32, torch.bfloat16)
    n = dvalue.shape[0]
    work = torch.empty(int(lib().u3d_value_scatter_workspace(n)), dtype=torch.uint8, device=dvalue.device)
    _check(lib().u3d_value_scatter(_ptr(records), m, n, _ptr(dvalue), int(dvalue.dtype == torch.bfloat16), _ptr(work), work.numel(),
                                   _stream()), "value_scatter")


def mha_fwd(qk, v, nq, p_attn=0.0, layer=0, rng=None):
    m = qk.shape[0]
    assert qk.dtype == v.dtype and qk.is_contiguous() and v.is_contiguous()
    o = torch.empty((m, 256), dtype=qk.dtype, device=qk.device)
    lse = torch.empty((m, 8), dtype=torch.float32, device=qk.device)
    _check(lib().u3d_mha_fwd_dt(_ptr(qk), _ptr(v), m, nq, p_attn, layer, _ptr(rng), _ptr(o), _ptr(lse), dt_code(qk.dtype), _stream()),
           "mha_fwd")
    return o, lse


def mha_bwd(qk, v, o, d_o, lse, nq, p_attn=0.0, layer=0, rng=None):
    m = qk.shape[0]
    assert qk.dtype == v.dtype == o.dtype == d_o.dtype
    dqk, dv = torch.empty_like(qk), torch.empty_like(v)
    _check(lib().u3d_mha_bwd_dt(_ptr(qk), _ptr(v), _ptr(o), _ptr(d_o), _ptr(lse), m, nq, p_attn, layer, _ptr(rng), _ptr(dqk), _ptr(dv),
                                dt_code(qk.dtype), _stream()), "mha_bwd")
    return dqk, dv


def wpack(descs_dev, count, max_elems, dtype=torch.bfloat16):
    _check(lib().u3d_wpack(_ptr(descs_dev), count, max_elems, dt_code(dtype), _stream()), "wpack")


def wpack_bf16(descs_dev, count, max_elems):
    wpack(descs_dev, count, max_elems, torch.bfloat16)


def dropout_mask(rng, layer, site, n, p, cols=0):
    keep = torch.empty((n,), dtype=torch.uint8, device=rng.device)
    _check(lib().u3d_dropout_mask(_ptr(rng), layer, site, n, p, int(cols), _ptr(keep), _stream()), "dropout_mask")
    return keep


AUG_NPARAM = _K["U3D_AUG_NPARAM"]


def points_augment(points, scene_off, params, coord, height_dim=-1):
    assert points.dtype == torch.float32 and points.is_contiguous() and params.dtype == torch.float32 and params.shape[1] == AUG_NPARAM
    batch = scene_off.numel() - 1
    _check(lib().u3d_points_augment(_ptr(points), _ptr(scene_off), batch, points.shape[0], points.shape[1], _ptr(params.contiguous()),
                                    int(coord), int(height_dim), _stream()), "points_augment")
# ... 334 lines not shown
```

### uni3detr_amd/plugin/fused_decoder.py

```python
import os

import torch
from torch import nn

from .. import native as nv

ENABLED = True
SHARED_DEFER = True
PK_SCATTER = os.environ.get("U3D_PK_SCATTER", "0") == "1"
POISON = os.environ.get("U3D_DEC_POISON", "0") == "1"
DEBUG_KEEP = None

_WIDE = [nv.DL_RPH0, nv.DL_RPH1, nv.DL_RPH2, nv.DL_QS0, nv.DL_QS1, nv.DL_QS2, nv.DL_INQK, nv.DL_INV, nv.DL_OUTP, nv.DL_OPROJ, nv.DL_PE1,
         nv.DL_FFN0, nv.DL_FFN1, nv.DL_REG0, nv.DL_REG1, nv.DL_CLS0, nv.DL_CLS1, nv.DL_IOU0, nv.DL_IOU1]
_NARROW = [nv.DL_REG2, nv.DL_CLS2, nv.DL_IOU2]


def _is_seq(seq, kinds):
    return isinstance(seq, nn.Sequential) and len(seq) == len(kinds) and all(isinstance(m, k) for m, k in zip(seq, kinds))


class LayerSpec:

    def __init__(self, decoder, lid, reg_branch, cls_branch, iou_branch):
        from .transformer import FFN, MultiheadAttention, UniCrossAtten
        layer = decoder.layers[lid]
        if layer.operation_order != ("self_attn", "norm", "cross_attn", "norm", "ffn", "norm"):
            raise ValueError("operation order")
        sa, ca, ffn = layer.attentions[0], layer.attentions[1], layer.ffns[0]
        if not (isinstance(sa, MultiheadAttention) and isinstance(ca, UniCrossAtten) and isinstance(ffn, FFN)):
            raise ValueError("layer members")
        if sa.embed_dims != 256 or sa.num_heads != 8 or ca.num_points != 1 or not ffn.add_identity:
            raise ValueError("dims")
        if not (_is_seq(ffn.layers, (nn.Sequential, nn.Linear, nn.Dropout)) and _is_seq(ffn.layers[0], (nn.Linear, nn.ReLU, nn.Dropout))):
            raise ValueError("ffn layout")
        f0, f1 = ffn.layers[0][0], ffn.layers[1]
        if f0.out_features != 512 or f1.in_features != 512:
            raise ValueError("ffn width")
        pe = ca.position_encoder
        if not _is_seq(pe, (nn.Linear, nn.LayerNorm, nn.ReLU, nn.Linear, nn.LayerNorm, nn.ReLU)):
            raise ValueError("position encoder")
        if not (_is_seq(reg_branch, (nn.Linear, nn.ReLU, nn.Linear, nn.ReLU, nn.Linear))
                and _is_seq(iou_branch, (nn.Linear, nn.ReLU, nn.Linear, nn.ReLU, nn.Linear))
                and _is_seq(cls_branch, (nn.Linear, nn.LayerNorm, nn.ReLU, nn.Linear, nn.LayerNorm, nn.ReLU, nn.Linear))):
            raise ValueError("branch layout")
        rph, qs = decoder.ref_point_head.layers, decoder.query_scale.layers
        if len(rph) != 3 or len(qs) != 3 or rph[0].in_features != 384:
            raise ValueError("mlp layout")
        ipw, ipb = sa.attn.in_proj_weight, sa.attn.in_proj_bias
        if ipw is None or ipb is None or sa.attn.out_proj.bias is None:
            raise ValueError("in_proj")
        L = lambda m: (m.weight, 0, m.weight.shape[0], m.bias)
        self.lin = [None] * nv.DL_NLIN
        for i, m in zip((nv.DL_RPH0, nv.DL_RPH1, nv.DL_RPH2), rph):
            self.lin[i] = L(m)
        for i, m in zip((nv.DL_QS0, nv.DL_QS1, nv.DL_QS2), qs):
            self.lin[i] = L(m)
        self.lin[nv.DL_INQK] = (ipw, 0, 512, ipb)
        self.lin[nv.DL_INV] = (ipw, 512, 256, ipb)
        self.lin[nv.DL_OUTP] = L(sa.attn.out_proj)
        self.lin[nv.DL_OPROJ] = L(ca.output_proj)
        self.lin[nv.DL_PE1] = L(pe[3])
        self.lin[nv.DL_FFN0], self.lin[nv.DL_FFN1] = L(f0), L(f1)
        self.lin[nv.DL_REG0], self.lin[nv.DL_REG1], self.lin[nv.DL_REG2] = L(reg_branch[0]), L(reg_branch[2]), L(reg_branch[4])
# ... 102 lines not shown
            st = self._states[et] = self._build(dev, et)
            st.key = key
        self.params = st.params
        nv.wpack(st.descs_dev, st.ndesc, st.max_elems, et)
        return st


class _State:
    key = None


def element_type(decoder, query, value, reg_branches, head_branches):
    if not (ENABLED and query.is_cuda):
        return None
    if reg_branches is None or head_branches is None or value.dim() != 5 or value.shape[1] != 256 or query.shape[-1] != 256:
        return None
    if len(reg_branches) != decoder.num_layers or len({id(m) for m in reg_branches}) != decoder.num_layers:
        return None
    if torch.is_autocast_enabled():
        return torch.bfloat16 if torch.get_autocast_dtype("cuda") == torch.bfloat16 else None
    return torch.float32 if (query.dtype == torch.float32 and value.dtype == torch.float32) else None


def eligible(decoder, query, value, reg_branches, head_branches):
    return element_type(decoder, query, value, reg_branches, head_branches) is not None


class FusedLayerFn(torch.autograd.Function):

    @staticmethod
    def forward(ctx, x, xc, ref, rows, meta, *ptensors):
        fd, lid, dims_t, accum = meta[:4]
        et = meta[4] if len(meta) > 4 else torch.bfloat16
        sp = fd.specs[lid]
        B, qps, nq, D, H, W = dims_t
        M = x.shape[0]
        x = x.contiguous()
        xc = x if et == torch.float32 else (x.to(et) if xc is None else xc)
        ref = ref.contiguous().float()
        assert rows.dtype == et and rows.is_contiguous()
        d = nv.DecLayerDims()
        d.m, d.nq, d.qps, d.batch, d.dz, d.dy, d.dx = M, nq, qps, B, D, H, W
        d.ncls, d.code, d.has_qs, d.need_dref, d.layer = sp.ncls, sp.code, int(lid > 0), 0, lid
        d.dtype = nv.dt_code(et)
        train = fd.decoder.training
        d.p_attn = sp.p_attn if train else 0.0
        d.p_drop = sp.p_drop if train else 0.0
        d.ln_eps = float(sp.ln[0].eps)
        so, go = nv.decoder_layer_slots(M, sp.ncls, sp.code, et)
        save = torch.empty(so["_total"], dtype=torch.uint8, device=x.device)
        if POISON:
            save.fill_(255)
        params = fd._states[et].params[lid]
        x_out, xc_out, reg, cls, iou = nv.decoder_layer_fwd(params, d, x, xc, ref, rows, fd.rng, save)
        ctx.save_for_backward(x, xc, ref, rows, xc_out, save)
        ctx.meta, ctx.dims, ctx.et, ctx.params = meta, d, et, params
        ctx.wids = []
        from .transformer import _Deferred
        for w, r0, rows_, b in sp.lin:
            if r0 == 0:
                _Deferred.uses[id(w)] = _Deferred.uses.get(id(w), 0) + 1
                _Deferred.fused_uses[id(w)] = _Deferred.fused_uses.get(id(w), 0) + 1
                _Deferred.params[id(w)] = (w, b)
        for t in (sp.attw.weight, sp.pe0.weight):
            _Deferred.uses[id(t)] = _Deferred.uses.get(id(t), 0) + 1
        for n in sp.ln:
            _Deferred.uses[id(n.weight)] = _Deferred.uses.get(id(n.weight), 0) + 1
        xc_ret = xc_out if et == torch.bfloat16 else x_out.new_empty(0)
        ctx.mark_non_differentiable(xc_ret)
        return x_out, xc_ret, reg, cls, iou

    @staticmethod
    def backward(ctx, dx_out, _dxc, dreg, dcls, diou):
        from .transformer import _Deferred
        x, xc, ref, rows, xc_out, save = ctx.saved_tensors
        fd, lid, dims_t, accum = ctx.meta[:4]
        et = ctx.et
        sp, d = fd.specs[lid], ctx.dims
        M = x.shape[0]
        dev = x.device
        d.need_dref = int(ctx.needs_input_grad[2])
        so, go = nv.decoder_layer_slots(M, sp.ncls, sp.code, et)
        grad = torch.empty(go["_total"], dtype=torch.uint8, device=dev)
        if POISON:
            grad.fill_(255)
        z = lambda t, shape: torch.zeros(shape, dtype=torch.float32, device=dev) if t is None else t.contiguous().float()
        dreg, dcls, diou = z(dreg, (M, sp.code)), z(dcls, (M, sp.ncls)), z(diou, (M,))
        dx_out = None if dx_out is None else dx_out.contiguous().float()
        want_dv = ctx.needs_input_grad[3]
        acc_dt = torch.bfloat16 if (PK_SCATTER and rows.dtype == torch.bfloat16) else torch.float32
        if accum is not None:
            if accum.buf is None:
                accum.buf = torch.zeros(rows.shape, dtype=acc_dt, device=dev)
            dvalue = accum.buf
        else:
            dvalue = torch.zeros(rows.shape, dtype=acc_dt, device=dev)
        dx, dref = nv.decoder_layer_bwd(ctx.params, d, x, xc, ref, rows, fd.rng, xc_out, save, dx_out, dreg, dcls, diou, dvalue, grad)
        if DEBUG_KEEP is not None:
            DEBUG_KEEP.append(grad)
        drows = None
        if accum is not None:
            accum.remaining -= 1
            if accum.remaining == 0:
                drows = accum.buf.to(rows.dtype) if want_dv else None
                accum.buf = None
        elif want_dv:
            drows = dvalue.to(rows.dtype)
        f32 = torch.float32
        S = lambda name, cols, dt=et: nv.slot_view(save, so[name], M, cols, dt)
        Gv = lambda name, cols, dt=et: nv.slot_view(grad, go[name], M, cols, dt)
        if d.need_dref:
            dref = dref + nv.sine_embed_bwd(ref, fd._dim_t, Gv("SINE", 384))
        pairs = {
            nv.DL_RPH0: (Gv("RPH1", 256), S("SINE", 384)), nv.DL_RPH1: (Gv("RPH2", 256), S("RPH1", 256)),
            nv.DL_RPH2: (Gv("RAW", 256), S("RPH2", 256)),
            nv.DL_INQK: (Gv("DQK", 512), S("QKIN", 256)), nv.DL_INV: (Gv("DV", 256), xc),
            nv.DL_OUTP: (Gv("O2", 256), S("O", 256)), nv.DL_OPROJ: (Gv("OUT", 256), S("GATED", 256)),
            nv.DL_PE1: (Gv("UPE1", 256), S("PEH0", 256)), nv.DL_FFN0: (Gv("FFH", 512), S("X2C", 256)),
            nv.DL_FFN1: (Gv("F", 256), S("FFH", 512)), nv.DL_REG0: (Gv("R1", 256), xc_out), nv.DL_REG1: (Gv("R2", 256), S("R1", 256)),
            nv.DL_REG2: (Gv("REGO", sp.code), S("R2", 256)), nv.DL_CLS0: (Gv("C1U", 256), xc_out),
            nv.DL_CLS1: (Gv("C2U", 256), S("C1", 256)), nv.DL_CLS2: (Gv("CLSO", sp.ncls), S("C2", 256)),
            nv.DL_IOU0: (Gv("I1", 256), xc_out), nv.DL_IOU1: (Gv("I2", 256), S("I1", 256)), nv.DL_IOU2: (Gv("IOUO", 1), S("I2", 256)),
        }
        if lid > 0:
            pairs.update({nv.DL_QS0: (Gv("QS1", 256), xc), nv.DL_QS1: (Gv("QS2", 256), S("QS1", 256)), nv.DL_QS2: (Gv("QS", 256), S("QS2", 256))})
        deferred_ok = _Deferred.active and et == torch.bfloat16
        split_wg = et == torch.float32 and getattr(fd.decoder, "split_f32_wgrad", False)
        planes = {}
        to_split = []
        ok = lambda t: t.dim() == 2 and t.stride(1) == 1 and t.stride(0) % 4 == 0 and t.shape[1] % 4 == 0 and t.data_ptr() % 16 == 0

        def hi_lo(t):
            key = id(t)
            if key not in planes:
                t2 = t if ok(t) else t.contiguous()
                pl = torch.empty((2 * t2.shape[0], t2.shape[1]), dtype=torch.bfloat16, device=dev)
                to_split.append((t2, pl))
                planes[key] = (t, pl[:t2.shape[0]], pl[t2.shape[0]:])
            return planes[key][1], planes[key][2]
        grads = []
        wgrad_now = {}
        sums_now = []
        new = lambda *shape: torch.empty(shape, dtype=f32, device=dev)

        def slot(param, deferred):
            v = getattr(param, "_u3d_grad_view", None) if deferred else None
            return v.view(v.shape) if (v is not None and v.dtype == f32 and v.is_contiguous()) else new(*param.shape)

        def skinny_now(dy, xin, dw):
            if et == torch.bfloat16:
# ... 176 lines not shown
```

Baseline: 435.5.

## Run fused decoder layer kernels with eight waves per workgroup for bf16

Parameterizes the fused decoder pre/post (and backward) kernels on a wave count NW, so each wave covers a narrower slice of output columns (NTW tiles) and bf16 workgroups launch 512 threads instead of 256. The Python side selects eight waves by default for bf16 and keeps four for fp32, with a new _nw entry point that takes the wave count. The aim is more latency hiding and MFMA parallelism per block on the row-tile GEMM chain. In exchange each wave reuses the A tile over fewer columns, the narrow heads run only on the first four waves, and there is extra register and barrier pressure.

```diff
diff --git a/include/u3d_hip.h b/include/u3d_hip.h
--- a/include/u3d_hip.h
+++ b/include/u3d_hip.h
@@ -464,6 +464,14 @@
                               const float* ref, const void* value, const uint64_t* rng, const void* xc_out, const void* save,
                               const float* dx_out, const float* dreg, const float* dcls, const float* diou, float* dx,
                               void* vrec, float* dref, void* grad, int64_t grad_bytes, u3d_stream s);
+int32_t u3d_decoder_layer_fwd_nw(const u3d_declayer_params* p, const u3d_declayer_dims* d, const float* x, const void* xc,
+                                 const float* ref, const void* value, const uint64_t* rng, float* x_out, void* xc_out,
+                                 float* reg_out, float* cls_out, float* iou_out, void* save, int64_t save_bytes, int32_t row_waves,
+                                 u3d_stream s);
+int32_t u3d_decoder_layer_bwd_nw(const u3d_declayer_params* p, const u3d_declayer_dims* d, const float* x, const void* xc,
+                                 const float* ref, const void* value, const uint64_t* rng, const void* xc_out, const void* save,
+                                 const float* dx_out, const float* dreg, const float* dcls, const float* diou, float* dx,
+                                 void* vrec, float* dref, void* grad, int64_t grad_bytes, int32_t row_waves, u3d_stream s);
 int64_t u3d_value_records_bytes(int32_t m);
 int64_t u3d_value_scatter_workspace(int32_t n_cells);
 int32_t u3d_value_scatter(const void* records, int32_t m, int32_t n_cells, void* dvalue, int32_t dvalue_bf16, void* work,
diff --git a/uni3detr_amd/csrc/decoder.hip b/uni3detr_amd/csrc/decoder.hip
--- a/uni3detr_amd/csrc/decoder.hip
+++ b/uni3detr_amd/csrc/decoder.hip
@@ -156,7 +156,7 @@
 }
 
 template <typename E>
-__global__ __launch_bounds__(DC_THREADS) void k_dec_pre(u3d_declayer_params P, u3d_declayer_dims dm, const typename E::T* __restrict__ xc,
+__global__ __launch_bounds__(E::NW * 64) void k_dec_pre(u3d_declayer_params P, u3d_declayer_dims dm, const typename E::T* __restrict__ xc,
                                                         const float* __restrict__ ref, DcPtrs<E> S, int skip_inproj) {
   typedef typename E::T T;
   typedef typename E::V4 V4;
@@ -168,7 +168,8 @@
   T* A1 = (T*)(lds + L::A1);
   T* A2 = (T*)(lds + L::A2);
   const int tid = threadIdx.x, lane = tid & 63, wave = dc_wave_id();
-  const int wv = (wave + (int)(blockIdx.x >> 3)) & 3;
+  constexpr int NTW = 16 / E::NW, WC = NTW * 16;
+  const int wv = (wave + (int)(blockIdx.x >> 3)) & (E::NW - 1);
   const int row0 = blockIdx.x * BM, M = dm.m;
   dc_poison_lds<E>(lds, tid);
   constexpr int SCH = 384 / E::CH;
@@ -194,26 +195,26 @@
     return [=](int row, int col, f32x4 v) { *(V4*)(dst + dc_aoff<E>(row, col, DC_C)) = E::pack4(v + dc_bias4(bias, col)); };
   };
   T* A1b = A1 + BM * DC_C;
-  dc_linear<E, 384, 4>(A0, (const T*)P.w[U3D_DL_RPH0], wv * 64, lane, relu_to(A1, P.b[U3D_DL_RPH0]));
+  dc_linear<E, 384, NTW>(A0, (const T*)P.w[U3D_DL_RPH0], wv * WC, lane, relu_to(A1, P.b[U3D_DL_RPH0]));
   __syncthreads();
   dc_store_a<E, 256>(A1, S.rph1, DC_C, row0, tid);
-  dc_linear<E, 256, 4>(A1, (const T*)P.w[U3D_DL_RPH1], wv * 64, lane, relu_to(A0, P.b[U3D_DL_RPH1]));
+  dc_linear<E, 256, NTW>(A1, (const T*)P.w[U3D_DL_RPH1], wv * WC, lane, relu_to(A0, P.b[U3D_DL_RPH1]));
   __syncthreads();
   dc_store_a<E, 256>(A0, S.rph2, DC_C, row0, tid);
-  dc_linear<E, 256, 4>(A0, (const T*)P.w[U3D_DL_RPH2], wv * 64, lane, lin_to(A2, P.b[U3D_DL_RPH2]));
+  dc_linear<E, 256, NTW>(A0, (const T*)P.w[U3D_DL_RPH2], wv * WC, lane, lin_to(A2, P.b[U3D_DL_RPH2]));
   __syncthreads();
   dc_store_a<E, 256>(A2, dm.has_qs ? S.raw : S.pos, DC_C, row0, tid);
   dc_load_a<E, 256, true>(A0, xc, DC_C, row0, M, tid);
   __syncthreads();
   if (dm.has_qs) {
-    dc_linear<E, 256, 4>(A0, (const T*)P.w[U3D_DL_QS0], wv * 64, lane, relu_to(A1, P.b[U3D_DL_QS0]));
+    dc_linear<E, 256, NTW>(A0, (const T*)P.w[U3D_DL_QS0], wv * WC, lane, relu_to(A1, P.b[U3D_DL_QS0]));
     __syncthreads();
     dc_store_a<E, 256>(A1, S.qs1, DC_C, row0, tid);
-    dc_linear<E, 256, 4>(A1, (const T*)P.w[U3D_DL_QS1], wv * 64, lane, relu_to(A1b, P.b[U3D_DL_QS1]));
+    dc_linear<E, 256, NTW>(A1, (const T*)P.w[U3D_DL_QS1], wv * WC, lane, relu_to(A1b, P.b[U3D_DL_QS1]));
     __syncthreads();
     dc_store_a<E, 256>(A1b, S.qs2, DC_C, row0, tid);
     const float* bias = P.b[U3D_DL_QS2];
-    dc_linear<E, 256, 4>(A1b, (const T*)P.w[U3D_DL_QS2], wv * 64, lane, [=](int row, int col, f32x4 v) {
+    dc_linear<E, 256, NTW>(A1b, (const T*)P.w[U3D_DL_QS2], wv * WC, lane, [=](int row, int col, f32x4 v) {
       const V4 q = E::pack4(v + dc_bias4(bias, col));
       const int ao = dc_aoff<E>(row, col, DC_C);
       const f32x4 raw = E::unpack4(*(const V4*)(A2 + ao));
@@ -235,17 +236,17 @@
   __syncthreads();
   dc_store_a<E, 256>(A1b, S.qkin, DC_C, row0, tid);
   if (skip_inproj) return;
-  dc_linear<E, 256, 4>(A1b, (const T*)P.w[U3D_DL_INQK], wv * 64, lane, lin_to(A1, P.b[U3D_DL_INQK]));
+  dc_linear<E, 256, NTW>(A1b, (const T*)P.w[U3D_DL_INQK], wv * WC, lane, lin_to(A1, P.b[U3D_DL_INQK]));
   {
     const float* bias = P.b[U3D_DL_INQK];
-    dc_linear<E, 256, 4>(A1b, (const T*)P.w[U3D_DL_INQK], 256 + wv * 64, lane, [=](int row, int col, f32x4 v) {
+    dc_linear<E, 256, NTW>(A1b, (const T*)P.w[U3D_DL_INQK], 256 + wv * WC, lane, [=](int row, int col, f32x4 v) {
       *(V4*)(A2 + dc_aoff<E>(row, col - 256, DC_C)) = E::pack4(v + dc_bias4(bias, col));
     });
   }
   __syncthreads();
   dc_store_a<E, 256>(A1, S.qk, 512, row0, tid);
   dc_store_a<E, 256>(A2, S.qk + 256, 512, row0, tid);
-  dc_linear<E, 256, 4>(A0, (const T*)P.w[U3D_DL_INV], wv * 64, lane, lin_to(A1b, P.b[U3D_DL_INV]));
+  dc_linear<E, 256, NTW>(A0, (const T*)P.w[U3D_DL_INV], wv * WC, lane, lin_to(A1b, P.b[U3D_DL_INV]));
   __syncthreads();
   dc_store_a<E, 256>(A1b, S.v, DC_C, row0, tid);
 }
@@ -552,7 +553,7 @@
 }
 
 template <typename E>
-__global__ __launch_bounds__(DC_THREADS) void k_dec_post(u3d_declayer_params P, u3d_declayer_dims dm, const float* __restrict__ x,
+__global__ __launch_bounds__(E::NW * 64) void k_dec_post(u3d_declayer_params P, u3d_declayer_dims dm, const float* __restrict__ x,
                                                          const float* __restrict__ ref, const typename E::T* __restrict__ value,
                                                          const unsigned long long* __restrict__ rng, DcPtrs<E> S, float* __restrict__ x_out,
                                                          typename E::T* __restrict__ xc_out, float* __restrict__ reg_out,
@@ -560,7 +561,7 @@
   typedef typename E::T T;
   typedef typename E::V4 V4;
   typedef DcLds<E> L;
-  constexpr int BM = E::BM, RPW = E::BM / 4;
+  constexpr int BM = E::BM, RPW = E::BM / E::NW;
   extern __shared__ __attribute__((aligned(16))) unsigned char lds[];
   T* A0 = (T*)(lds + L::A0);
   T* A1 = (T*)(lds + L::A1);
@@ -569,7 +570,8 @@
   float* G = (float*)(lds + L::G);
   float* misc = (float*)(lds + L::MISC);
   const int tid = threadIdx.x, lane = tid & 63, wave = dc_wave_id();
-  const int wv = (wave + (int)(blockIdx.x >> 3)) & 3;
+  constexpr int NTW = 16 / E::NW, WC = NTW * 16;
+  const int wv = (wave + (int)(blockIdx.x >> 3)) & (E::NW - 1);
   const int row0 = blockIdx.x * BM, M = dm.m;
   dc_poison_lds<E>(lds, tid);
   DcDrop drop = {dc_rng_load(rng), dc_thresh(dm.p_drop), dc_inv_keep(dm.p_drop), dm.layer};
@@ -592,7 +594,7 @@
     };
   };
   DC_MARK(1);
-  dc_linear<E, 256, 4>(A0, (const T*)P.w[U3D_DL_OUTP], wv * 64, lane, add_to_F(P.b[U3D_DL_OUTP], 0));
+  dc_linear<E, 256, NTW>(A0, (const T*)P.w[U3D_DL_OUTP], wv * WC, lane, add_to_F(P.b[U3D_DL_OUTP], 0));
   __syncthreads();
   DC_MARK(2);
   {
@@ -651,17 +653,19 @@
   }
   DC_MARK(4);
   {
-    const int col = tid;
+    constexpr int PR = BM / (E::NW / 4);
+    const int col = E::NW > 4 ? tid & 255 : tid, prow0 = E::NW > 4 ? (wave >> 2) * PR : 0;
     const float w0 = E::round(P.pe0_w[col * 3 + 0]), w1 = E::round(P.pe0_w[col * 3 + 1]), w2 = E::round(P.pe0_w[col * 3 + 2]);
     const float b = P.pe0_b[col];
-    for (int row = 0; row < BM; ++row) {
+    for (int pr = 0; pr < PR; ++pr) {
+      const int row = prow0 + pr;
       const float* r3 = misc + row * DC_MISC_LD;
       G[row * DC_TS + col] = E::round(E::round(r3[0]) * w0 + E::round(r3[1]) * w1 + E::round(r3[2]) * w2 + b);
     }
   }
   __syncthreads();
   DC_MARK(5);
-  dc_linear<E, 256, 4>(A1, (const T*)P.w[U3D_DL_OPROJ], wv * 64, lane, add_to_F(P.b[U3D_DL_OPROJ], 1));
+  dc_linear<E, 256, NTW>(A1, (const T*)P.w[U3D_DL_OPROJ], wv * WC, lane, add_to_F(P.b[U3D_DL_OPROJ], 1));
   {
     DcLnOut<E> o = {nullptr, A0, DC_C, nullptr, S.peh0, S.mr, U3D_DLN_PE0, false, nullptr, nullptr};
     dc_layernorm<E>(G, P.ln_g[U3D_DLN_PE0], P.ln_b[U3D_DLN_PE0], dm.ln_eps, true, o, row0, wave, lane);
@@ -670,7 +674,7 @@
   DC_MARK(6);
   {
     const float* bias = P.b[U3D_DL_PE1];
-    dc_linear<E, 256, 4>(A0, (const T*)P.w[U3D_DL_PE1], wv * 64, lane, [=](int row, int col, f32x4 v) {
+    dc_linear<E, 256, NTW>(A0, (const T*)P.w[U3D_DL_PE1], wv * WC, lane, [=](int row, int col, f32x4 v) {
       *(f32x4*)(G + row * DC_TS + col) = E::round4(v + dc_bias4(bias, col));
     });
   }
@@ -700,13 +704,13 @@
       const V4 hb = E::pack4(drop.apply(v, 2, (unsigned)((row0 + row) * DC_FF + col)));
       *(V4*)(A1 + dc_aoff<E>(row, col, DC_FF)) = hb;
     };
-    dc_linear<E, 256, 4>(A0, (const T*)P.w[U3D_DL_FFN0], wv * 64, lane, ffh);
-    dc_linear<E, 256, 4>(A0, (const T*)P.w[U3D_DL_FFN0], 256 + wv * 64, lane, ffh);
+    dc_linear<E, 256, NTW>(A0, (const T*)P.w[U3D_DL_FFN0], wv * WC, lane, ffh);
+    dc_linear<E, 256, NTW>(A0, (const T*)P.w[U3D_DL_FFN0], 256 + wv * WC, lane, ffh);
   }
   __syncthreads();
   DC_MARK(10);
   dc_store_a<E, 512>(A1, S.ffh, DC_FF, row0, tid);
-  dc_linear<E, 512, 4>(A1, (const T*)P.w[U3D_DL_FFN1], wv * 64, lane, add_to_F(P.b[U3D_DL_FFN1], 3));
+  dc_linear<E, 512, NTW>(A1, (const T*)P.w[U3D_DL_FFN1], wv * WC, lane, add_to_F(P.b[U3D_DL_FFN1], 3));
   __syncthreads();
   DC_MARK(11);
   {
@@ -731,58 +735,59 @@
 #ifdef DC_PHASE_TIMING
   {
     DC_MARK(20);
-    f32x4 acc[E::MT][4];
+    f32x4 acc[E::MT][NTW];
 #pragma unroll
     for (int mt = 0; mt < E::MT; ++mt)
 #pragma unroll
-      for (int nt = 0; nt < 4; ++nt) acc[mt][nt] = (f32x4){0.f, 0.f, 0.f, 0.f};
-    dc_gemm<E, 256, 4>(A2, (const T*)P.w[U3D_DL_REG0] + (size_t)(wv * 64) * 256, acc, lane);
+      for (int nt = 0; nt < NTW; ++nt) acc[mt][nt] = (f32x4){0.f, 0.f, 0.f, 0.f};
+    dc_gemm<E, 256, NTW>(A2, (const T*)P.w[U3D_DL_REG0] + (size_t)(wv * WC) * 256, acc, lane);
     __builtin_amdgcn_sched_barrier(0);
     DC_MARK(21);
     auto epi = relu_to(A0, P.b[U3D_DL_REG0]);
 #pragma unroll
     for (int mt = 0; mt < E::MT; ++mt)
 #pragma unroll
-      for (int nt = 0; nt < 4; ++nt) epi(mt * 16 + (lane & 15), wv * 64 + nt * 16 + (lane >> 4) * 4, acc[mt][nt]);
+      for (int nt = 0; nt < NTW; ++nt) epi(mt * 16 + (lane & 15), wv * WC + nt * 16 + (lane >> 4) * 4, acc[mt][nt]);
     __builtin_amdgcn_sched_barrier(0);
     DC_MARK(22);
     __syncthreads();
     DC_MARK(23);
   }
 #else
-  dc_linear<E, 256, 4>(A2, (const T*)P.w[U3D_DL_REG0], wv * 64, lane, relu_to(A0, P.b[U3D_DL_REG0]));
+  dc_linear<E, 256, NTW>(A2, (const T*)P.w[U3D_DL_REG0], wv * WC, lane, relu_to(A0, P.b[U3D_DL_REG0]));
   __syncthreads();
 #endif
   dc_store_a<E, 256>(A0, S.r1, DC_C, row0, tid);
-  dc_linear<E, 256, 4>(A0, (const T*)P.w[U3D_DL_REG1], wv * 64, lane, relu_to(A1, P.b[U3D_DL_REG1]));
+  dc_linear<E, 256, NTW>(A0, (const T*)P.w[U3D_DL_REG1], wv * WC, lane, relu_to(A1, P.b[U3D_DL_REG1]));
   __syncthreads();
   dc_store_a<E, 256>(A1, S.r2, DC_C, row0, tid);
-  dc_linear<E, 256, 1>(A1, (const T*)P.w[U3D_DL_REG2], wv * 16, lane, narrow_out(reg_out, dm.code, P.b[U3D_DL_REG2]));
-  dc_linear<E, 256, 4>(A2, (const T*)P.w[U3D_DL_IOU0], wv * 64, lane, relu_to(A0, P.b[U3D_DL_IOU0]));
+  if (wv < 4) dc_linear<E, 256, 1>(A1, (const T*)P.w[U3D_DL_REG2], wv * 16, lane, narrow_out(reg_out, dm.code, P.b[U3D_DL_REG2]));
+  dc_linear<E, 256, NTW>(A2, (const T*)P.w[U3D_DL_IOU0], wv * WC, lane, relu_to(A0, P.b[U3D_DL_IOU0]));
   __syncthreads();
   dc_store_a<E, 256>(A0, S.i1, DC_C, row0, tid);
-  dc_linear<E, 256, 4>(A0, (const T*)P.w[U3D_DL_IOU1], wv * 64, lane, relu_to(A1b, P.b[U3D_DL_IOU1]));
+  dc_linear<E, 256, NTW>(A0, (const T*)P.w[U3D_DL_IOU1], wv * WC, lane, relu_to(A1b, P.b[U3D_DL_IOU1]));
   __syncthreads();
   dc_store_a<E, 256>(A1b, S.i2, DC_C, row0, tid);
-  dc_linear<E, 256, 1>(A1b, (const T*)P.w[U3D_DL_IOU2], wv * 16, lane, narrow_out(iou_out, 1, P.b[U3D_DL_IOU2]));
+  if (wv < 4) dc_linear<E, 256, 1>(A1b, (const T*)P.w[U3D_DL_IOU2], wv * 16, lane, narrow_out(iou_out, 1, P.b[U3D_DL_IOU2]));
+  DC_MARK(13);
   auto to_G = [&](const float* bias) {
     return [=](int row, int col, f32x4 v) { *(f32x4*)(G + row * DC_TS + col) = E::round4(v + dc_bias4(bias, col)); };
   };
-  dc_linear<E, 256, 4>(A2, (const T*)P.w[U3D_DL_CLS0], wv * 64, lane, to_G(P.b[U3D_DL_CLS0]));
+  dc_linear<E, 256, NTW>(A2, (const T*)P.w[U3D_DL_CLS0], wv * WC, lane, to_G(P.b[U3D_DL_CLS0]));
   __syncthreads();
   {
     DcLnOut<E> o = {nullptr, A0, DC_C, nullptr, S.c1, S.mr, U3D_DLN_C1, false, nullptr, S.uc1};
     dc_layernorm<E>(G, P.ln_g[U3D_DLN_C1], P.ln_b[U3D_DLN_C1], dm.ln_eps, true, o, row0, wave, lane);
   }
   __syncthreads();
-  dc_linear<E, 256, 4>(A0, (const T*)P.w[U3D_DL_CLS1], wv * 64, lane, to_G(P.b[U3D_DL_CLS1]));
+  dc_linear<E, 256, NTW>(A0, (const T*)P.w[U3D_DL_CLS1], wv * WC, lane, to_G(P.b[U3D_DL_CLS1]));
   __syncthreads();
   {
     DcLnOut<E> o = {nullptr, A1, DC_C, nullptr, S.c2, S.mr, U3D_DLN_C2, false, nullptr, S.uc2};
     dc_layernorm<E>(G, P.ln_g[U3D_DLN_C2], P.ln_b[U3D_DLN_C2], dm.ln_eps, true, o, row0, wave, lane);
   }
   __syncthreads();
-  dc_linear<E, 256, 1>(A1, (const T*)P.w[U3D_DL_CLS2], wv * 16, lane, narrow_out(cls_out, dm.ncls, P.b[U3D_DL_CLS2]));
+  if (wv < 4) dc_linear<E, 256, 1>(A1, (const T*)P.w[U3D_DL_CLS2], wv * 16, lane, narrow_out(cls_out, dm.ncls, P.b[U3D_DL_CLS2]));
   DC_MARK(14);
 }
 
@@ -812,7 +817,7 @@
   U3D_ALLOW_LDS(k_dec_pre<E>, DcLds<E>::BYTES);
   U3D_ALLOW_LDS(k_dec_post<E>, DcLds<E>::BYTES);
   const bool fused = mha_fused_inproj(E::DT, d->nq);
-  hipLaunchKernelGGL(k_dec_pre<E>, dim3(nb), dim3(DC_THREADS), DcLds<E>::BYTES, s, *p, *d, (const T*)xc, ref, S, fused ? 1 : 0);
+  hipLaunchKernelGGL(k_dec_pre<E>, dim3(nb), dim3(E::NW * 64), DcLds<E>::BYTES, s, *p, *d, (const T*)xc, ref, S, fused ? 1 : 0);
   if (fused) {
     U3D_ALLOW_LDS(k_mha_proj_fwd, MhaProjLds::BYTES);
     const float scale_log2 = 1.4426950408889634f / sqrtf((float)DC_HD);
@@ -824,22 +829,31 @@
     int32_t rc = u3d_mha_fwd_dt(S.qk, S.v, d->m, d->nq, d->p_attn, d->layer, rng, S.o, S.lse, E::DT, s);
     if (rc != U3D_OK) return rc;
   }
-  hipLaunchKernelGGL(k_dec_post<E>, dim3(nb), dim3(DC_THREADS), DcLds<E>::BYTES, s, *p, *d, x, ref, (const T*)value,
+  hipLaunchKernelGGL(k_dec_post<E>, dim3(nb), dim3(E::NW * 64), DcLds<E>::BYTES, s, *p, *d, x, ref, (const T*)value,
                      (const unsigned long long*)rng, S, x_out, (T*)xc_out, reg_out, cls_out, iou_out);
   U3D_CHECK_LAUNCH();
   return U3D_OK;
 }
 
-extern "C" int32_t u3d_decoder_layer_fwd(const u3d_declayer_params* p, const u3d_declayer_dims* d, const float* x, const void* xc,
-                                         const float* ref, const void* value, const uint64_t* rng, float* x_out, void* xc_out,
-                                         float* reg_out, float* cls_out, float* iou_out, void* save, int64_t save_bytes, u3d_stream s) {
+extern "C" int32_t u3d_decoder_layer_fwd_nw(const u3d_declayer_params* p, const u3d_declayer_dims* d, const float* x, const void* xc,
+                                            const float* ref, const void* value, const uint64_t* rng, float* x_out, void* xc_out,
+                                            float* reg_out, float* cls_out, float* iou_out, void* save, int64_t save_bytes,
+                                            int32_t row_waves, u3d_stream s) {
   int32_t rc = dc_check(p, d);
   if (rc != U3D_OK) return rc;
   U3D_REQUIRE(x && xc && ref && value && x_out && xc_out && reg_out && cls_out && iou_out && save, U3D_ERR_ARG);
   U3D_REQUIRE((d->p_attn == 0.f && d->p_drop == 0.f) || rng, U3D_ERR_ARG);
+  U3D_REQUIRE(row_waves == 0 || row_waves == 4 || (row_waves == 8 && d->dtype == U3D_BF16), U3D_ERR_ARG);
   int64_t off[U3D_DS_COUNT + 1];
   u3d_decoder_layer_slots_dt(d->m, d->ncls, d->code, d->dtype, off, nullptr);
   U3D_REQUIRE(save_bytes >= off[U3D_DS_COUNT], U3D_ERR_WORKSPACE);
+  if (d->dtype == U3D_BF16 && row_waves == 4)
+    return dc_layer_fwd<EB4>(p, d, x, xc, ref, value, rng, x_out, xc_out, reg_out, cls_out, iou_out, save, s);
   if (d->dtype == U3D_BF16) return dc_layer_fwd<EB>(p, d, x, xc, ref, value, rng, x_out, xc_out, reg_out, cls_out, iou_out, save, s);
   return dc_layer_fwd<EF>(p, d, x, xc, ref, value, rng, x_out, xc_out, reg_out, cls_out, iou_out, save, s);
 }
+extern "C" int32_t u3d_decoder_layer_fwd(const u3d_declayer_params* p, const u3d_declayer_dims* d, const float* x, const void* xc,
+                                         const float* ref, const void* value, const uint64_t* rng, float* x_out, void* xc_out,
+                                         float* reg_out, float* cls_out, float* iou_out, void* save, int64_t save_bytes, u3d_stream s) {
+  return u3d_decoder_layer_fwd_nw(p, d, x, xc, ref, value, rng, x_out, xc_out, reg_out, cls_out, iou_out, save, save_bytes, 0, s);
+}
diff --git a/uni3detr_amd/csrc/decoder_bwd.hip b/uni3detr_amd/csrc/decoder_bwd.hip
--- a/uni3detr_amd/csrc/decoder_bwd.hip
+++ b/uni3detr_amd/csrc/decoder_bwd.hip
@@ -87,10 +87,12 @@
                                                  const DcLnBwdOut<E>& o, float* __restrict__ lnp, int ln, int nb, float* red ,
                                                  int row0, int wave, int lane, int tid) {
   typedef typename E::V4 V4;
-  constexpr int RPW = E::BM / 4;
+  constexpr int RPW = E::BM / E::NW, CHAIN = E::NW / 4;
   const f32x4 ga = *(const f32x4*)(gamma + lane * 4), be = *(const f32x4*)(beta + lane * 4);
   f32x4 dg = {0.f, 0.f, 0.f, 0.f}, db = {0.f, 0.f, 0.f, 0.f};
-#pragma unroll 2
+  constexpr int KEEP = CHAIN > 1 ? RPW : 1, UNROLL = CHAIN > 1 ? RPW : 2;
+  f32x4 kdy[KEEP], kxh[KEEP];
+#pragma unroll UNROLL
   for (int rr = 0; rr < RPW; ++rr) {
     const int row = wave * RPW + rr;
     const int gr = row0 + row;
@@ -106,8 +108,14 @@
       dxh[j] = dy[j] * ga[j];
       s1 += dxh[j];
       s2 += dxh[j] * xh[j];
-      dg[j] += dy[j] * xh[j];
-      db[j] += dy[j];
+      if constexpr (CHAIN == 1) {
+        dg[j] += dy[j] * xh[j];
+        db[j] += dy[j];
+      }
+    }
+    if constexpr (CHAIN > 1) {
+      kdy[rr] = dy;
+      kxh[rr] = xh;
     }
     s1 = dc_wave_sum(s1) * (1.f / DC_C);
     s2 = dc_wave_sum(s2) * (1.f / DC_C);
@@ -119,9 +127,32 @@
     if (o.a) *(V4*)(o.a + dc_aoff<E>(row, lane * 4, DC_C)) = dub;
     if (o.g16) *(V4*)(o.g16 + (size_t)gr * DC_C + lane * 4) = dub;
   }
-  *(f32x4*)(red + (wave * 2 + 0) * DC_C + lane * 4) = dg;
-  *(f32x4*)(red + (wave * 2 + 1) * DC_C + lane * 4) = db;
-  __syncthreads();
+  float* rq = red + (wave / CHAIN) * 2 * DC_C + lane * 4;
+  if constexpr (CHAIN == 1) {
+    *(f32x4*)rq = dg;
+    *(f32x4*)(rq + DC_C) = db;
+    __syncthreads();
+  } else {
+#pragma unroll
+    for (int t = 0; t < CHAIN; ++t) {
+      if (wave % CHAIN == t) {
+        if (t > 0) {
+          dg = *(const f32x4*)rq;
+          db = *(const f32x4*)(rq + DC_C);
+        }
+#pragma unroll
+        for (int rr = 0; rr < RPW; ++rr)
+#pragma unroll
+          for (int j = 0; j < 4; ++j) {
+            dg[j] += kdy[rr][j] * kxh[rr][j];
+            db[j] += kdy[rr][j];
+          }
+        *(f32x4*)rq = dg;
+        *(f32x4*)(rq + DC_C) = db;
+      }
+      __syncthreads();
+    }
+  }
   DC_FOR_TID(i, 2 * DC_C) {
     const int which = i >> 8, col = i & 255;
     const float v = red[(0 * 2 + which) * DC_C + col] + red[(1 * 2 + which) * DC_C + col] + red[(2 * 2 + which) * DC_C + col] +
@@ -132,7 +163,7 @@
 }
 
 template <typename E>
-__global__ __launch_bounds__(DC_THREADS) void k_dec_post_bwd(u3d_declayer_params P, u3d_declayer_dims dm, const float* __restrict__ ref,
+__global__ __launch_bounds__(E::NW * 64) void k_dec_post_bwd(u3d_declayer_params P, u3d_declayer_dims dm, const float* __restrict__ ref,
                                                              const typename E::T* __restrict__ value,
                                                              const unsigned long long* __restrict__ rng, DcSave<E> S, DcGrad<E> Gd,
                                                              const float* __restrict__ dx_out, const float* __restrict__ dreg,
@@ -144,7 +175,7 @@
   typedef typename E::T T;
   typedef typename E::V4 V4;
   typedef DcLds<E> L;
-  constexpr int BM = E::BM, RPW = E::BM / 4;
+  constexpr int BM = E::BM, RPW = E::BM / E::NW;
   extern __shared__ __attribute__((aligned(16))) unsigned char lds[];
   T* A0 = (T*)(lds + L::A0);
   T* A1 = (T*)(lds + L::A1);
@@ -158,7 +189,8 @@
   T* Dn = A2;
   static_assert(BM * NLD <= BM * DC_C, "narrow-gradient tile must fit the A2 region");
   const int tid = threadIdx.x, lane = tid & 63, wave = dc_wave_id();
-  const int wv = (wave + (int)(blockIdx.x >> 3)) & 3;
+  constexpr int NTW = 16 / E::NW, WC = NTW * 16;
+  const int wv = (wave + (int)(blockIdx.x >> 3)) & (E::NW - 1);
   const int row0 = blockIdx.x * BM, M = dm.m, nb = Gd.nb;
   dc_poison_lds<E>(lds, tid);
   DcDrop drop = {dc_rng_load(rng), dc_thresh(dm.p_drop), dc_inv_keep(dm.p_drop), dm.layer};
@@ -182,19 +214,19 @@
     typedef typename E::VC VC;
     constexpr int KSN = 32 / E::KSTEP, WBLK = 64 * E::CH;
     const int r16 = lane & 15, kq = lane >> 4;
-    f32x4 acc[E::MT][4];
+    f32x4 acc[E::MT][NTW];
 #pragma unroll
     for (int mt = 0; mt < E::MT; ++mt)
 #pragma unroll
-      for (int nt = 0; nt < 4; ++nt) acc[mt][nt] = (f32x4){0.f, 0.f, 0.f, 0.f};
+      for (int nt = 0; nt < NTW; ++nt) acc[mt][nt] = (f32x4){0.f, 0.f, 0.f, 0.f};
 #pragma unroll
     for (int ks = 0; ks < KSN; ++ks) {
       VC a[E::MT];
 #pragma unroll
       for (int mt = 0; mt < E::MT; ++mt) a[mt] = *(const VC*)(Dn + (mt * 16 + r16) * NLD + (ks * 4 + kq) * E::CH);
 #pragma unroll
-      for (int nt = 0; nt < 4; ++nt) {
-        const VC wf = *(const VC*)(wt + (size_t)((wv * 4 + nt) * KSN + ks) * WBLK + lane * E::CH);
+      for (int nt = 0; nt < NTW; ++nt) {
+        const VC wf = *(const VC*)(wt + (size_t)((wv * NTW + nt) * KSN + ks) * WBLK + lane * E::CH);
 #pragma unroll
         for (int mt = 0; mt < E::MT; ++mt) E::mma(wf, a[mt], acc[mt][nt]);
       }
@@ -202,8 +234,8 @@
 #pragma unroll
     for (int mt = 0; mt < E::MT; ++mt)
 #pragma unroll
-      for (int nt = 0; nt < 4; ++nt) {
-        const int row = mt * 16 + r16, col = wv * 64 + nt * 16 + kq * 4;
+      for (int nt = 0; nt < NTW; ++nt) {
+        const int row = mt * 16 + r16, col = wv * WC + nt * 16 + kq * 4;
         f32x4 v = acc[mt][nt];
         if (mask_src) {
           const V4 y = *(const V4*)(mask_src + (size_t)(row0 + row) * DC_C + col);
@@ -248,14 +280,14 @@
     dc_layernorm_bwd<E>(G, u_elem(S.uc2), S.mr, U3D_DLN_C2, P.ln_g[U3D_DLN_C2], P.ln_b[U3D_DLN_C2], true, o, Gd.lnp, U3D_DLN_C2, nb, red, row0,
                         wave, lane, tid);
   }
-  dc_linear<E, 256, 4>(A0, (const T*)P.wt[U3D_DL_CLS1], wv * 64, lane, to_G());
+  dc_linear<E, 256, NTW>(A0, (const T*)P.wt[U3D_DL_CLS1], wv * WC, lane, to_G());
   __syncthreads();
   {
     DcLnBwdOut<E> o = {nullptr, A0, Gd.c1u};
     dc_layernorm_bwd<E>(G, u_elem(S.uc1), S.mr, U3D_DLN_C1, P.ln_g[U3D_DLN_C1], P.ln_b[U3D_DLN_C1], true, o, Gd.lnp, U3D_DLN_C1, nb, red, row0,
                         wave, lane, tid);
   }
-  dc_linear<E, 256, 4>(A0, (const T*)P.wt[U3D_DL_CLS0], wv * 64, lane, acc_to_F());
+  dc_linear<E, 256, NTW>(A0, (const T*)P.wt[U3D_DL_CLS0], wv * WC, lane, acc_to_F());
   __syncthreads();
   DC_MARK(2);
   load_narrow(diou, 1, Gd.iouo);
@@ -263,10 +295,10 @@
   narrow_dgrad((const T*)P.wt[U3D_DL_IOU2], S.i2, A0);
   __syncthreads();
   dc_store_a<E, 256>(A0, Gd.i2, DC_C, row0, tid);
-  dc_linear<E, 256, 4>(A0, (const T*)P.wt[U3D_DL_IOU1], wv * 64, lane, masked_to(A1, S.i1));
+  dc_linear<E, 256, NTW>(A0, (const T*)P.wt[U3D_DL_IOU1], wv * WC, lane, masked_to(A1, S.i1));
   __syncthreads();
   dc_store_a<E, 256>(A1, Gd.i1, DC_C, row0, tid);
-  dc_linear<E, 256, 4>(A1, (const T*)P.wt[U3D_DL_IOU0], wv * 64, lane, acc_to_F());
+  dc_linear<E, 256, NTW>(A1, (const T*)P.wt[U3D_DL_IOU0], wv * WC, lane, acc_to_F());
   __syncthreads();
   DC_MARK(3);
   load_narrow(dreg, dm.code, Gd.rego);
@@ -274,10 +306,10 @@
   narrow_dgrad((const T*)P.wt[U3D_DL_REG2], S.r2, A0);
   __syncthreads();
   dc_store_a<E, 256>(A0, Gd.r2, DC_C, row0, tid);
-  dc_linear<E, 256, 4>(A0, (const T*)P.wt[U3D_DL_REG1], wv * 64, lane, masked_to(A1, S.r1));
+  dc_linear<E, 256, NTW>(A0, (const T*)P.wt[U3D_DL_REG1], wv * WC, lane, masked_to(A1, S.r1));
   __syncthreads();
   dc_store_a<E, 256>(A1, Gd.r1, DC_C, row0, tid);
-  dc_linear<E, 256, 4>(A1, (const T*)P.wt[U3D_DL_REG0], wv * 64, lane, acc_to_F());
+  dc_linear<E, 256, NTW>(A1, (const T*)P.wt[U3D_DL_REG0], wv * WC, lane, acc_to_F());
   __syncthreads();
   DC_MARK(4);
   {
@@ -307,12 +339,12 @@
       const V4 o = E::pack4(v);
       *(V4*)(A1 + dc_aoff<E>(row, col, DC_FF)) = o;
     };
-    dc_linear<E, 256, 4>(A0, (const T*)P.wt[U3D_DL_FFN1], wv * 64, lane, dh);
-    dc_linear<E, 256, 4>(A0, (const T*)P.wt[U3D_DL_FFN1], 256 + wv * 64, lane, dh);
+    dc_linear<E, 256, NTW>(A0, (const T*)P.wt[U3D_DL_FFN1], wv * WC, lane, dh);
+    dc_linear<E, 256, NTW>(A0, (const T*)P.wt[U3D_DL_FFN1], 256 + wv * WC, lane, dh);
   }
   __syncthreads();
   dc_store_a<E, 512>(A1, Gd.ffh, DC_FF, row0, tid);
-  dc_linear<E, 512, 4>(A1, (const T*)P.wt[U3D_DL_FFN0], wv * 64, lane, acc_to_F());
+  dc_linear<E, 512, NTW>(A1, (const T*)P.wt[U3D_DL_FFN0], wv * WC, lane, acc_to_F());
   __syncthreads();
   DC_MARK(6);
   {
@@ -331,7 +363,7 @@
     dc_layernorm_bwd<E>(G, u_elem(S.upe1), S.mr, U3D_DLN_PE1, P.ln_g[U3D_DLN_PE1], P.ln_b[U3D_DLN_PE1], true, o, Gd.lnp, U3D_DLN_PE1, nb, red,
                         row0, wave, lane, tid);
   }
-  dc_linear<E, 256, 4>(A0, (const T*)P.wt[U3D_DL_PE1], wv * 64, lane, to_G());
+  dc_linear<E, 256, NTW>(A0, (const T*)P.wt[U3D_DL_PE1], wv * WC, lane, to_G());
   __syncthreads();
   {
     const f32x4 b4 = *(const f32x4*)(P.pe0_b + lane * 4);
@@ -366,7 +398,7 @@
   DC_MARK(8);
   branch_grad(1, A0, Gd.out);
   __syncthreads();
-  dc_linear<E, 256, 4>(A0, (const T*)P.wt[U3D_DL_OPROJ], wv * 64, lane, to_G());
+  dc_linear<E, 256, NTW>(A0, (const T*)P.wt[U3D_DL_OPROJ], wv * WC, lane, to_G());
   __syncthreads();
   DC_MARK(9);
   {
@@ -440,7 +472,7 @@
   dc_store_f<E>(F, Gd.du1, row0, tid);
   branch_grad(0, A0, Gd.o2);
   __syncthreads();
-  dc_linear<E, 256, 4>(A0, (const T*)P.wt[U3D_DL_OUTP], wv * 64, lane, [=](int row, int col, f32x4 v) {
+  dc_linear<E, 256, NTW>(A0, (const T*)P.wt[U3D_DL_OUTP], wv * WC, lane, [=](int row, int col, f32x4 v) {
     *(V4*)(A1 + dc_aoff<E>(row, col, DC_C)) = E::pack4(v);
   });
   __syncthreads();
@@ -578,7 +610,7 @@
         __syncthreads();
         H::stage(qk + h * DC_HD, 512, base, qc0, nq, Qs, Qt, tid);
         H::stage(d_o + h * DC_HD, 256, base, qc0, nq, Os, Ot, tid);
-        DC_FOR_TID(c, KC * NP) {
+        MHA_FOR_TID(c, KC * NP) {
           const int qq = c / NP, part = c % NP;
           float d = 0.f;
           if (qc0 + qq < nq) {
@@ -596,7 +628,7 @@
         }
         if constexpr (H::TR) {
           if (amask) {
-            DC_FOR_TID(c, KC * MW) Ms[c] = c < nq * MW ? amask[(size_t)bh * nq * MW + c] : 0u;
+            MHA_FOR_TID(c, KC * MW) Ms[c] = c < nq * MW ? amask[(size_t)bh * nq * MW + c] : 0u;
           }
         }
         __syncthreads();
@@ -669,7 +701,7 @@
 }
 
 template <typename E>
-__global__ __launch_bounds__(DC_THREADS) void k_dec_pre_bwd(u3d_declayer_params P, u3d_declayer_dims dm, DcSave<E> S, DcGrad<E> Gd,
+__global__ __launch_bounds__(E::NW * 64) void k_dec_pre_bwd(u3d_declayer_params P, u3d_declayer_dims dm, DcSave<E> S, DcGrad<E> Gd,
                                                             float* __restrict__ dx) {
   typedef typename E::T T;
   typedef typename E::V4 V4;
@@ -682,7 +714,8 @@
   float* F = (float*)(lds + L::F);
   float* G = (float*)(lds + L::G);
   const int tid = threadIdx.x, lane = tid & 63, wave = dc_wave_id();
-  const int wv = (wave + (int)(blockIdx.x >> 3)) & 3;
+  constexpr int NTW = 16 / E::NW, WC = NTW * 16;
+  const int wv = (wave + (int)(blockIdx.x >> 3)) & (E::NW - 1);
   const int row0 = blockIdx.x * BM, M = dm.m;
   dc_poison_lds<E>(lds, tid);
 
@@ -704,9 +737,9 @@
       *(V4*)(dst + dc_aoff<E>(row, col, DC_C)) = E::pack4(v);
     };
   };
-  dc_linear<E, 512, 4>(A1, (const T*)P.wt[U3D_DL_INQK], wv * 64, lane,
+  dc_linear<E, 512, NTW>(A1, (const T*)P.wt[U3D_DL_INQK], wv * WC, lane,
                        [=](int row, int col, f32x4 v) { *(f32x4*)(G + row * DC_TS + col) = E::round4(v); });
-  dc_linear<E, 256, 4>(A0, (const T*)P.wt[U3D_DL_INV], wv * 64, lane, acc_to_F());
+  dc_linear<E, 256, NTW>(A0, (const T*)P.wt[U3D_DL_INV], wv * WC, lane, acc_to_F());
   __syncthreads();
   DC_FOR_TID(c, BM * 64) {
     const int row = c >> 6, col = (c & 63) * 4;
@@ -732,25 +765,25 @@
   __syncthreads();
   T* A1b = A1 + BM * DC_C;
   if (dm.has_qs) {
-    dc_linear<E, 256, 4>(A0, (const T*)P.wt[U3D_DL_QS2], wv * 64, lane, masked_to(A1, S.qs2));
+    dc_linear<E, 256, NTW>(A0, (const T*)P.wt[U3D_DL_QS2], wv * WC, lane, masked_to(A1, S.qs2));
     __syncthreads();
     dc_store_a<E, 256>(A1, Gd.qs2, DC_C, row0, tid);
-    dc_linear<E, 256, 4>(A1, (const T*)P.wt[U3D_DL_QS1], wv * 64, lane, masked_to(A1b, S.qs1));
+    dc_linear<E, 256, NTW>(A1, (const T*)P.wt[U3D_DL_QS1], wv * WC, lane, masked_to(A1b, S.qs1));
     __syncthreads();
     dc_store_a<E, 256>(A1b, Gd.qs1, DC_C, row0, tid);
-    dc_linear<E, 256, 4>(A1b, (const T*)P.wt[U3D_DL_QS0], wv * 64, lane, acc_to_F());
+    dc_linear<E, 256, NTW>(A1b, (const T*)P.wt[U3D_DL_QS0], wv * WC, lane, acc_to_F());
     __syncthreads();
   }
-  dc_linear<E, 256, 4>(A2, (const T*)P.wt[U3D_DL_RPH2], wv * 64, lane, masked_to(A0, S.rph2));
+  dc_linear<E, 256, NTW>(A2, (const T*)P.wt[U3D_DL_RPH2], wv * WC, lane, masked_to(A0, S.rph2));
   __syncthreads();
   dc_store_a<E, 256>(A0, Gd.rph2, DC_C, row0, tid);
-  dc_linear<E, 256, 4>(A0, (const T*)P.wt[U3D_DL_RPH1], wv * 64, lane, masked_to(A1, S.rph1));
+  dc_linear<E, 256, NTW>(A0, (const T*)P.wt[U3D_DL_RPH1], wv * WC, lane, masked_to(A1, S.rph1));
   __syncthreads();
   dc_store_a<E, 256>(A1, Gd.rph1, DC_C, row0, tid);
   if (dm.need_dref) {
     auto to_sine = [=](int row, int col, f32x4 v) { *(V4*)(Gd.sine + (size_t)(row0 + row) * 384 + col) = E::pack4(v); };
-    dc_linear<E, 256, 4>(A1, (const T*)P.wt[U3D_DL_RPH0], wv * 64, lane, to_sine);
-    dc_linear<E, 256, 2>(A1, (const T*)P.wt[U3D_DL_RPH0], 256 + wv * 32, lane, to_sine);
+    dc_linear<E, 256, NTW>(A1, (const T*)P.wt[U3D_DL_RPH0], wv * WC, lane, to_sine);
+    dc_linear<E, 256, NTW / 2>(A1, (const T*)P.wt[U3D_DL_RPH0], 256 + wv * (WC / 2), lane, to_sine);
   }
   dc_store_f<E>(F, dx, row0, tid);
 }
@@ -781,24 +814,24 @@
   const DcSave<E> S = dcb_resolve_save<E>(save, d->m);
   U3D_ALLOW_LDS(k_dec_post_bwd<E>, DcLds<E>::BYTES);
   U3D_ALLOW_LDS(k_dec_pre_bwd<E>, DcLds<E>::BYTES);
-  hipLaunchKernelGGL(k_dec_post_bwd<E>, dim3(G.nb), dim3(DC_THREADS), DcLds<E>::BYTES, s, *p, *d, ref, (const T*)value,
+  hipLaunchKernelGGL(k_dec_post_bwd<E>, dim3(G.nb), dim3(E::NW * 64), DcLds<E>::BYTES, s, *p, *d, ref, (const T*)value,
                      (const unsigned long long*)rng, S, G, dx_out, dreg, dcls, diou, dvalue, dref);
   if (mha_fused_inproj(E::DT, d->nq) && d->p_attn > 0.f) {
     U3D_REQUIRE((long long)(d->m / d->nq) * DC_NHEAD * d->nq * (d->nq + 1) < (1ll << 32), U3D_ERR_UNSUPPORTED);
-    mha_bwd_launch<E>(S.qk, S.v, S.o, G.d_o, S.lse, d->m, d->nq, d->p_attn, d->layer, rng, G.dqk, G.dv, s, S.amask);
+    mha_bwd_launch<typename E::ME>(S.qk, S.v, S.o, G.d_o, S.lse, d->m, d->nq, d->p_attn, d->layer, rng, G.dqk, G.dv, s, S.amask);
   } else {
     int32_t rc = u3d_mha_bwd_dt(S.qk, S.v, S.o, G.d_o, S.lse, d->m, d->nq, d->p_attn, d->layer, rng, G.dqk, G.dv, E::DT, s);
     if (rc != U3D_OK) return rc;
   }
-  hipLaunchKernelGGL(k_dec_pre_bwd<E>, dim3(G.nb), dim3(DC_THREADS), DcLds<E>::BYTES, s, *p, *d, S, G, dx);
+  hipLaunchKernelGGL(k_dec_pre_bwd<E>, dim3(G.nb), dim3(E::NW * 64), DcLds<E>::BYTES, s, *p, *d, S, G, dx);
   U3D_CHECK_LAUNCH();
   return U3D_OK;
 }
 
-extern "C" int32_t u3d_decoder_layer_bwd(const u3d_declayer_params* p, const u3d_declayer_dims* d, const float* x, const void* xc,
-                                         const float* ref, const void* value, const uint64_t* rng, const void* xc_out, const void* save,
-                                         const float* dx_out, const float* dreg, const float* dcls, const float* diou, float* dx,
-                                         void* dvalue, float* dref, void* grad, int64_t grad_bytes, u3d_stream s) {
+extern "C" int32_t u3d_decoder_layer_bwd_nw(const u3d_declayer_params* p, const u3d_declayer_dims* d, const float* x, const void* xc,
+                                            const float* ref, const void* value, const uint64_t* rng, const void* xc_out, const void* save,
+                                            const float* dx_out, const float* dreg, const float* dcls, const float* diou, float* dx,
+                                            void* dvalue, float* dref, void* grad, int64_t grad_bytes, int32_t row_waves, u3d_stream s) {
   (void)x; (void)xc; (void)xc_out;
   int32_t rc = dcb_check(p, d);
   if (rc != U3D_OK) return rc;
@@ -806,9 +839,19 @@
   U3D_REQUIRE(d->reserved == 0, U3D_ERR_ARG);
   U3D_REQUIRE(!d->need_dref || dref, U3D_ERR_ARG);
   U3D_REQUIRE((d->p_attn == 0.f && d->p_drop == 0.f) || rng, U3D_ERR_ARG);
+  U3D_REQUIRE(row_waves == 0 || row_waves == 4 || (row_waves == 8 && d->dtype == U3D_BF16), U3D_ERR_ARG);
+  if (d->dtype == U3D_BF16 && row_waves == 4)
+    return dcb_layer_bwd<EB4>(p, d, ref, value, rng, save, dx_out, dreg, dcls, diou, dx, dvalue, dref, grad, grad_bytes, s);
   if (d->dtype == U3D_BF16)
     return dcb_layer_bwd<EB>(p, d, ref, value, rng, save, dx_out, dreg, dcls, diou, dx, dvalue, dref, grad, grad_bytes, s);
   return dcb_layer_bwd<EF>(p, d, ref, value, rng, save, dx_out, dreg, dcls, diou, dx, dvalue, dref, grad, grad_bytes, s);
+}
+extern "C" int32_t u3d_decoder_layer_bwd(const u3d_declayer_params* p, const u3d_declayer_dims* d, const float* x, const void* xc,
+                                         const float* ref, const void* value, const uint64_t* rng, const void* xc_out, const void* save,
+                                         const float* dx_out, const float* dreg, const float* dcls, const float* diou, float* dx,
+                                         void* dvalue, float* dref, void* grad, int64_t grad_bytes, u3d_stream s) {
+  return u3d_decoder_layer_bwd_nw(p, d, x, xc, ref, value, rng, xc_out, save, dx_out, dreg, dcls, diou, dx, dvalue, dref, grad, grad_bytes,
+                                  0, s);
 }
 
 #define VS_K 64
diff --git a/uni3detr_amd/csrc/decoder_common.h b/uni3detr_amd/csrc/decoder_common.h
--- a/uni3detr_amd/csrc/decoder_common.h
+++ b/uni3detr_amd/csrc/decoder_common.h
@@ -8,7 +8,7 @@
 typedef unsigned short u16x4 __attribute__((ext_vector_type(4)));
 typedef unsigned short u16x8 __attribute__((ext_vector_type(8)));
 
-#define DC_THREADS 256
+#define MHA_THREADS 256
 #define DC_C 256
 #define DC_FF 512
 #define DC_TS 260
@@ -41,9 +41,11 @@
   typedef u16 T;
   typedef u16x4 V4;
   typedef u16x8 VC;
+  typedef EB ME;
   static constexpr int CH = 8;
   static constexpr int BM = 32;
   static constexpr int MT = 2;
+  static constexpr int NW = 8;
   static constexpr int KSTEP = 32;
   static constexpr int DT = U3D_BF16;
   static constexpr int MHA_KC = 320;
@@ -65,13 +67,16 @@
     acc = __builtin_amdgcn_mfma_f32_16x16x32_bf16(__builtin_bit_cast(bf16x8, w), __builtin_bit_cast(bf16x8, a), acc, 0, 0, 0);
   }
 };
+struct EB4 : EB { static constexpr int NW = 4; };
 struct EF {
   typedef float T;
   typedef f32x4 V4;
   typedef f32x4 VC;
+  typedef EF ME;
   static constexpr int CH = 4;
   static constexpr int BM = 16;
   static constexpr int MT = 1;
+  static constexpr int NW = 4;
   static constexpr int KSTEP = 16;
   static constexpr int DT = U3D_F32;
   static constexpr int MHA_KC = 64;
@@ -150,6 +155,9 @@
 #ifndef DC_PF
 #define DC_PF 8
 #endif
+#ifndef DC_PF_NW8
+#define DC_PF_NW8 DC_PF
+#endif
 constexpr int dc_burst(int ks, int want) {
   int b = 1;
   for (int d = 1; d <= want && d <= ks; ++d)
@@ -161,7 +169,7 @@
   typedef typename E::T T;
   typedef typename E::VC VC;
   constexpr int KS = K / E::KSTEP;
-  constexpr int PF = dc_burst(KS, DC_PF);
+  constexpr int PF = dc_burst(KS, E::NW == 8 ? DC_PF_NW8 : DC_PF);
   static_assert((K / E::CH) % 16 == 0, "the chunk swizzle permutes aligned groups of 16 chunks");
 #ifdef DC_ABL_NOGEMM
   return;
@@ -232,14 +240,15 @@
   return r;
 }
 
-#define DC_FOR_TID(c, N) _Pragma("unroll") for (int it_ = 0, c = tid; it_ < (N) / DC_THREADS; ++it_, c += DC_THREADS)
+#define DC_FOR_TID(c, N) _Pragma("unroll") for (int it_ = 0, c = tid; it_ < (N) / (E::NW * 64); ++it_, c += E::NW * 64)
+#define MHA_FOR_TID(c, N) _Pragma("unroll") for (int it_ = 0, c = tid; it_ < (N) / MHA_THREADS; ++it_, c += MHA_THREADS)
 __device__ __forceinline__ int dc_wave_id() { return __builtin_amdgcn_readfirstlane((int)(threadIdx.x >> 6)); }
 
 template <typename E, int K, bool CLAMP>
 __device__ __forceinline__ void dc_load_a(typename E::T* A, const typename E::T* __restrict__ src, int ld, int row0, int M, int tid) {
   typedef typename E::VC VC;
   constexpr int CPR = K / E::CH;
-  static_assert((E::BM * CPR) % DC_THREADS == 0, "tile chunks must split evenly over the workgroup");
+  static_assert((E::BM * CPR) % (E::NW * 64) == 0, "tile chunks must split evenly over the workgroup");
   DC_FOR_TID(c, E::BM * CPR) {
     const int row = c / CPR, ch = c % CPR;
     const int gr = CLAMP ? min(row0 + row, M - 1) : row0 + row;
@@ -296,7 +305,7 @@
 __device__ __forceinline__ void dc_layernorm(const float* T, const float* __restrict__ gamma, const float* __restrict__ beta, float eps,
                                              bool relu, const DcLnOut<E>& o, int row0, int wave, int lane) {
   typedef typename E::V4 V4;
-  constexpr int RPW = E::BM / 4;
+  constexpr int RPW = E::BM / E::NW;
   const f32x4 ga = *(const f32x4*)(gamma + lane * 4), be = *(const f32x4*)(beta + lane * 4);
 #pragma unroll 2
   for (int rr = 0; rr < RPW; ++rr) {
@@ -355,12 +364,12 @@
 template <typename E>
 __device__ __forceinline__ void dc_poison_lds(unsigned char* lds, int tid) {
 #if DC_POISON_LDS == 1
-  for (int i = tid; i < DcLds<E>::BYTES / 4; i += DC_THREADS) ((unsigned*)lds)[i] = 0xFFFFFFFFu;
+  for (int i = tid; i < DcLds<E>::BYTES / 4; i += E::NW * 64) ((unsigned*)lds)[i] = 0xFFFFFFFFu;
   __syncthreads();
 #elif DC_POISON_LDS == 2
   __syncthreads();
 #elif DC_POISON_LDS == 3
-  for (int i = tid; i < DcLds<E>::BYTES / 4; i += DC_THREADS) ((unsigned*)lds)[i] = 0xFFFFFFFFu;
+  for (int i = tid; i < DcLds<E>::BYTES / 4; i += E::NW * 64) ((unsigned*)lds)[i] = 0xFFFFFFFFu;
 #endif
 }
 
@@ -392,7 +401,7 @@
   }
   __device__ static __forceinline__ void stage(const T* __restrict__ src, int ld, long long base_row, int first, int nvalid, T* rowmajor,
                                                T* transposed, int tid) {
-    DC_FOR_TID(c, KC * NP) {
+    MHA_FOR_TID(c, KC * NP) {
       const int key = c / NP, part = c % NP;
       VC v = E::zero_chunk();
       if (first + key < nvalid) v = *(const VC*)(src + (base_row + first + key) * ld + part * E::CH);
diff --git a/uni3detr_amd/native.py b/uni3detr_amd/native.py
--- a/uni3detr_amd/native.py
+++ b/uni3detr_amd/native.py
@@ -1627,7 +1627,7 @@
     return decoder_blocks(m, dtype) * (32 if dtype == torch.bfloat16 else 16)
 
 
-def decoder_layer_fwd(params, dims, x, xc, ref, value_rows, rng, save):
+def decoder_layer_fwd(params, dims, x, xc, ref, value_rows, rng, save, row_waves=0):
     m, code, ncls = dims.m, dims.code, dims.ncls
     et = torch.bfloat16 if dims.dtype == DT_BF16 else torch.float32
     assert xc.dtype == et and value_rows.dtype == et and x.dtype == torch.float32
@@ -1638,13 +1638,13 @@
     reg = torch.empty((mp, code), dtype=torch.float32, device=dev)
     cls = torch.empty((mp, ncls), dtype=torch.float32, device=dev)
     iou = torch.empty((mp,), dtype=torch.float32, device=dev)
-    _check(lib().u3d_decoder_layer_fwd(C.byref(params), C.byref(dims), _ptr(x), _ptr(xc), _ptr(ref), _ptr(value_rows), _ptr(rng),
-                                       _ptr(x_out), _ptr(xc_out), _ptr(reg), _ptr(cls), _ptr(iou), _ptr(save), save.numel(), _stream()),
-           "decoder_layer_fwd")
+    _check(lib().u3d_decoder_layer_fwd_nw(C.byref(params), C.byref(dims), _ptr(x), _ptr(xc), _ptr(ref), _ptr(value_rows), _ptr(rng),
+                                          _ptr(x_out), _ptr(xc_out), _ptr(reg), _ptr(cls), _ptr(iou), _ptr(save), save.numel(),
+                                          int(row_waves), _stream()), "decoder_layer_fwd")
     return x_out[:m], xc_out[:m], reg[:m], cls[:m], iou[:m]
 
 
-def decoder_layer_bwd(params, dims, x, xc, ref, value_rows, rng, xc_out, save, dx_out, dreg, dcls, diou, dvalue, grad):
+def decoder_layer_bwd(params, dims, x, xc, ref, value_rows, rng, xc_out, save, dx_out, dreg, dcls, diou, dvalue, grad, row_waves=0):
     m = dims.m
     dims.reserved = 0
     assert dvalue.dtype == torch.float32 or dims.dtype == DT_BF16
@@ -1652,9 +1652,10 @@
     mp = decoder_rows(m, torch.bfloat16 if dims.dtype == DT_BF16 else torch.float32)
     dx = torch.empty((mp, 256), dtype=torch.float32, device=ref.device)
     dref = torch.empty((mp, 3), dtype=torch.float32, device=ref.device) if dims.need_dref else None
-    _check(lib().u3d_decoder_layer_bwd(C.byref(params), C.byref(dims), _ptr(x), _ptr(xc), _ptr(ref), _ptr(value_rows), _ptr(rng),
-                                       _ptr(xc_out), _ptr(save), _ptr(dx_out), _ptr(dreg), _ptr(dcls), _ptr(diou), _ptr(dx),
-                                       _ptr(rec), _ptr(dref), _ptr(grad), grad.numel(), _stream()), "decoder_layer_bwd")
+    _check(lib().u3d_decoder_layer_bwd_nw(C.byref(params), C.byref(dims), _ptr(x), _ptr(xc), _ptr(ref), _ptr(value_rows), _ptr(rng),
+                                          _ptr(xc_out), _ptr(save), _ptr(dx_out), _ptr(dreg), _ptr(dcls), _ptr(diou), _ptr(dx),
+                                          _ptr(rec), _ptr(dref), _ptr(grad), grad.numel(), int(row_waves), _stream()),
+           "decoder_layer_bwd")
     value_scatter(rec, m, dvalue)
     return dx[:m], (None if dref is None else dref[:m])
 
diff --git a/uni3detr_amd/plugin/fused_decoder.py b/uni3detr_amd/plugin/fused_decoder.py
--- a/uni3detr_amd/plugin/fused_decoder.py
+++ b/uni3detr_amd/plugin/fused_decoder.py
@@ -10,6 +10,7 @@
 PK_SCATTER = os.environ.get("U3D_PK_SCATTER", "0") == "1"
 POISON = os.environ.get("U3D_DEC_POISON", "0") == "1"
 DEBUG_KEEP = None
+ROW_WAVES = 8
 
 _WIDE = [nv.DL_RPH0, nv.DL_RPH1, nv.DL_RPH2, nv.DL_QS0, nv.DL_QS1, nv.DL_QS2, nv.DL_INQK, nv.DL_INV, nv.DL_OUTP, nv.DL_OPROJ, nv.DL_PE1,
          nv.DL_FFN0, nv.DL_FFN1, nv.DL_REG0, nv.DL_REG1, nv.DL_CLS0, nv.DL_CLS1, nv.DL_IOU0, nv.DL_IOU1]
@@ -218,7 +219,8 @@
         if POISON:
             save.fill_(255)
         params = fd._states[et].params[lid]
-        x_out, xc_out, reg, cls, iou = nv.decoder_layer_fwd(params, d, x, xc, ref, rows, fd.rng, save)
+        ctx.row_waves = ROW_WAVES if et == torch.bfloat16 else 4
+        x_out, xc_out, reg, cls, iou = nv.decoder_layer_fwd(params, d, x, xc, ref, rows, fd.rng, save, ctx.row_waves)
         ctx.save_for_backward(x, xc, ref, rows, xc_out, save)
         ctx.meta, ctx.dims, ctx.et, ctx.params = meta, d, et, params
         ctx.wids = []
@@ -261,7 +263,8 @@
             dvalue = accum.buf
         else:
             dvalue = torch.zeros(rows.shape, dtype=acc_dt, device=dev)
-        dx, dref = nv.decoder_layer_bwd(ctx.params, d, x, xc, ref, rows, fd.rng, xc_out, save, dx_out, dreg, dcls, diou, dvalue, grad)
+        dx, dref = nv.decoder_layer_bwd(ctx.params, d, x, xc, ref, rows, fd.rng, xc_out, save, dx_out, dreg, dcls, diou, dvalue, grad,
+                                        ctx.row_waves)
         if DEBUG_KEEP is not None:
             DEBUG_KEEP.append(grad)
         drows = None
```

Result: faster. 442.1 (median of 6 runs) (+1.5%).
